# GuoYi0/alphaFive

Hardware: AMD Instinct MI355X
Metric: self-play moves/sec (11x11, 500 sims/move) (higher is better)
Workload: dtype f32 (fp16x2 split operands: 3 fp16 MFMA products per MAC, fp32 accumulate)

## Files before the change

### alphafive_amd/arena.py

```python
import ctypes

import numpy as np

from . import engine as _eng
from . import utils


def play_matches(cfg, pv0, pv1, n_games, device=0, seed0=0, seed1=1, node_cap=0, max_plies=None):
    import torch
    S, G = cfg.board_size, n_games
    C = S * S
    dev = torch.device("cuda", device)
    engines = [_eng.Engine(cfg, G, device=device, mode=_eng.MODE_EXTERNAL, training=False, seed=s, node_cap=node_cap)
               for s in (seed0, seed1)]
    pvs = [pv0, pv1]
    planes = torch.zeros((G, 3, S, S), dtype=torch.float32, device=dev)
    policy = [torch.zeros((G, C), dtype=torch.float32, device=dev) for _ in range(2)]
    value = [torch.zeros((G,), dtype=torch.float32, device=dev) for _ in range(2)]
    stream = torch.cuda.current_stream(dev).cuda_stream
    boards = [np.zeros((S, S), np.int8) for _ in range(G)]
    last = [None] * G
    over = [False] * G
    moves = [[] for _ in range(G)]
    wins, draws = [0, 0], 0
    ply = 0
    limit = max_plies or C
    while not all(over) and ply < limit:
        for p in (0, 1):
            active = [i for i in range(G) if not over[i] and (i + ply) % 2 == p]
            if not active:
                continue
            e = engines[p]
            keys = np.stack([_eng.state_to_key(utils.board_to_state(boards[i]), S) for i in active])
            lcs = [-1 if last[i] is None else last[i][0] * S + last[i][1] for i in active]
            e.set_roots(active, keys, lcs, random_a=True, reset_tree=(ply < 2), stream=stream)
            while True:
                e.tick(policy[p].data_ptr(), value[p].data_ptr(), planes.data_ptr(), stream)
                st = e.status(stream)
                if all(st[i] == _eng.STATUS_MOVE_DONE for i in active):
                    break
                pr, va = pvs[p](planes)
                policy[p].copy_(pr.reshape(G, C))
                value[p].copy_(va.reshape(G))
            cells = e.move_results(active, stream=stream)[0]
            for i, cell in zip(active, cells):
                cell = int(cell)
                a = (cell // S, cell % S)
                moves[i].append(cell)
                boards[i] = utils.step(boards[i], a)
                last[i] = a
                done, v = utils.is_game_over(boards[i], cfg.goal)
                if done:
                    over[i] = True
                    if v == 0.0:
                        draws += 1
                    else:
                        wins[p] += 1
        ply += 1
    for e in engines:
        e.close()
    return dict(wins=wins, draws=draws, moves=moves, lengths=[len(m) for m in moves])


MATCH_WIN0, MATCH_WIN1, MATCH_DRAW, MATCH_UNFINISHED = 0, 1, 2, -1
TICK_SLACK = 64


class DeviceArena:

    def __init__(self, cfg, pv0, pv1, num_games, device=0, seed0=0, seed1=1, node_cap=0, weights_versions=(None, None)):
        import torch
        if not torch.cuda.is_available():
            raise _eng.EngineError("DeviceArena needs a HIP device (torch.cuda.is_available() is False)")
        self.torch = torch
        self.cfg = cfg
        S, G = cfg.board_size, num_games
        self.S, self.C, self.G = S, S * S, G
        self.dev = torch.device("cuda", device)
        torch.cuda.set_device(self.dev)
        self.engines, self._match = [], None
        for s in (seed0, seed1):
            self.engines.append(_eng.Engine(cfg, G, device=device, mode=_eng.MODE_EXTERNAL, training=False, seed=s, node_cap=node_cap))
        h = ctypes.c_void_p()
        _eng._check(_eng.lib().af_match_create(self.engines[0]._h, self.engines[1]._h, ctypes.byref(h)), "af_match_create")
        self._match = h
        self.pvs = [pv0, pv1]
        self.planes = [torch.zeros((G, 3, S, S), dtype=torch.float32, device=self.dev) for _ in range(2)]
        self.policy = [torch.zeros((G, self.C), dtype=torch.float32, device=self.dev) for _ in range(2)]
        self.value = [torch.zeros((G,), dtype=torch.float32, device=self.dev) for _ in range(2)]
        self._versions, self._version_missing = [], False
        for p, pv in enumerate(self.pvs):
            ver, missing = _eng.resolve_weights_version(pv, weights_versions[p])
            self._versions.append(ver)
            self._version_missing = self._version_missing or missing
            if hasattr(pv, "bind_outputs"):
                pv.bind_outputs(self.policy[p], self.value[p])
        self._graph = None
        self._prog_host = torch.zeros(3, dtype=torch.int64, pin_memory=True)
        self._prog_events = [torch.cuda.Event(), torch.cuda.Event()]
        self.rounds = self.replays = self.eager_rounds = 0

    def _stream(self):
        return self.torch.cuda.current_stream(self.dev).cuda_stream

    def round(self):
        stream = self._stream()
        L = _eng.lib()
        for p in (0, 1):
            self.engines[p].tick(self.policy[p].data_ptr(), self.value[p].data_ptr(), self.planes[p].data_ptr(), stream)
            pr, va = self.pvs[p](self.planes[p])
            if pr.data_ptr() != self.policy[p].data_ptr():
                self.policy[p].copy_(pr.reshape(self.G, self.C))
            if va.data_ptr() != self.value[p].data_ptr():
                self.value[p].copy_(va.reshape(self.G))
            _eng._check(L.af_match_step(self._match, stream), "af_match_step")
        self.rounds += 1

    def _post_progress(self):
        _eng._check(_eng.lib().af_match_progress_async(self._match, self._stream(), self._prog_host.data_ptr()), "af_match_progress_async")

    def _graph_key(self, rounds_per_replay):
        return (int(rounds_per_replay), self.engines[0].params_key(), self.engines[1].params_key(),
                tuple(v() if v is not None else None for v in self._versions))

    def _raise_first_error(self, code):
        raise _eng.EngineError("device arena: a game failed: %s (code %d)" % (_eng.lib().af_strerror(code).decode(), code))

    def run(self, n_games=None, max_plies=None, rounds_per_replay=8, graph=True):
        torch = self.torch
        n_games = self.G if n_games is None else int(n_games)
        limit = int(max_plies or self.C)
        if graph and self._version_missing:
            raise _eng.EngineError("DeviceArena.run(graph=True): an evaluator takes bind_outputs but exposes no weights_version (a "
                                   "replayed graph would keep evaluating with stale weights); pass weights_versions=")
        stream = self._stream()
        _eng._check(_eng.lib().af_match_start(self._match, stream, n_games, limit), "af_match_start")
        self.rounds = self.replays = self.eager_rounds = 0
        self._prog_host.zero_()
        bound = limit * (2 * int(self.cfg.upper_simulation_per_step) + TICK_SLACK)
        n = int(rounds_per_replay)
        turn, posted = 0, 0
        if graph and (self._graph is None or self._graph[0] != self._graph_key(n)):
            self._graph = None
            self.round()
            self.eager_rounds += 1
            torch.cuda.synchronize(self.dev)
            g = torch.cuda.CUDAGraph()
            with torch.cuda.graph(g, capture_error_mode="thread_local"):
                for _ in range(n):
                    self.round()
                self._post_progress()
            self.rounds -= n
            self._graph = (self._graph_key(n), g)
        while True:
            if self.rounds > bound:
                raise _eng.EngineError("device arena: %d games not finished after %d rounds (bound %d)" % (n_games, self.rounds, bound))
            if graph:
                self._graph[1].replay()
                self.rounds += n
                self.replays += 1
            else:
                for _ in range(n):
                    self.round()
                self.eager_rounds += n
                self._post_progress()
            turn ^= 1
            self._prog_events[turn].record(torch.cuda.current_stream(self.dev))
            posted += 1
            if posted < 2:
                continue
            self._prog_events[turn ^ 1].synchronize()
            done, _, err = (int(x) for x in self._prog_host)
            if err:
                torch.cuda.synchronize(self.dev)
                self._raise_first_error(err)
            if done >= n_games:
                break
        return self.results(n_games)

    def results(self, n_games=None):
        n_games = self.G if n_games is None else int(n_games)
        res, lens = np.zeros(self.G, np.int32), np.zeros(self.G, np.int32)
        mv = np.zeros((self.G, self.C), np.int32)
        rc = _eng.lib().af_match_results(self._match, self._stream(), _eng._p(res, ctypes.c_int32), _eng._p(lens, ctypes.c_int32),
                                         _eng._p(mv, ctypes.c_int32))
        if rc < 0:
            self._raise_first_error(rc)
        res, lens = res[:n_games], lens[:n_games]
        return dict(wins=[int((res == MATCH_WIN0).sum()), int((res == MATCH_WIN1).sum())], draws=int((res == MATCH_DRAW).sum()),
                    moves=[[int(c) for c in mv[i, :lens[i]]] for i in range(n_games)], lengths=[int(x) for x in lens])

    def close(self):
        if getattr(self, "_match", None):
            _eng.lib().af_match_destroy(self._match)
            self._match = None
        for e in getattr(self, "engines", []):
            e.close()

    __del__ = close


def play_matches_device(cfg, pv0, pv1, n_games, device=0, seed0=0, seed1=1, node_cap=0, max_plies=None, **run_kw):
    a = DeviceArena(cfg, pv0, pv1, n_games, device=device, seed0=seed0, seed1=seed1, node_cap=node_cap)
    try:
        return a.run(n_games, max_plies=max_plies, **run_kw)
    finally:
        a.close()


def ladder(cfg, ckpt_paths, games, match_fn=None, result_path=None, log=print):
    paths = list(ckpt_paths)
    own = None
    if match_fn is None:
        own = match_fn = _arena_match_fn(cfg, games)
    out = []
    low, high = 0, len(paths) - 1
    try:
        while low < high:
            c0, c1 = paths[low], paths[high]
            w0, w1, draws = match_fn(c0, c1, games)
            line = "%s: %s = %d: %d" % (c0, c1, w0, w1)
            if log is not None:
                log(line)
            if result_path is not None:
                with open(result_path, "a") as f:
                    f.write(line + "\n")
            out.append((c0, c1, int(w0), int(w1), int(draws)))
            if w0 < w1:
                low += 1
            else:
                high -= 1
    finally:
        if own is not None:
            own.close()
    return out


def _arena_match_fn(cfg, games, device=0):
    state = {}

    def load(net, path):
        if str(path).endswith(".npz"):
            net.load_npz(path)
        else:
            net.restore(path)

    def match(path0, path1, n):
        from .network import ResNet
        if not state:
            state["nets"] = [ResNet(cfg.board_size, device="cuda:%d" % device) for _ in range(2)]
            state["loaded"] = [None, None]
            state["arena"] = DeviceArena(cfg, state["nets"][0].select_backend("hip"), state["nets"][1].select_backend("hip"), n,
                                         device=device)
        for p, path in enumerate((path0, path1)):
            if state["loaded"][p] != path:
                load(state["nets"][p], path)
                state["loaded"][p] = path
        r = state["arena"].run(n)
        return r["wins"][0], r["wins"][1], r["draws"]

    def close():
        if state:
            state["arena"].close()
# ... 7 lines not shown
```

### alphafive_amd/csrc/af_conv_f16s.h

```cpp
#ifndef AF_CONV_F16S_H
#define AF_CONV_F16S_H

#include <hip/hip_runtime.h>

#include <map>
#include <string>

struct f16s_net;

int f16s_supported(int board_size);
int f16s_create(f16s_net** out, int board_size, int max_batch, int device);
void f16s_destroy(f16s_net* n);
enum F16sBits : int {
    kF16sProfilingBits = 1 | 2 | 4 | 8 | 4096,
    kF16sValuStem = 16,
    kF16sOneWgPerCu = 32,
    kF16sTwoHalves15 = 64,
    kF16sWgPerPosition = 128,
    kF16sTwoLaunchBlocks = 256,
    kF16sBranchLaunchesSmall = 512,
    kF16sBranchLaunchesBig = 1024,
    kF16sLaunchSequence = 2048,
};
enum F16sForm {
    kF16sRoles,
    kF16sPaired,
    kF16sBranches,
};
struct F16sPlan {
    int batch, bits;
    bool heads;
    F16sForm form;
    bool valu_stem, two_wg_per_cu, half_classes, tile_split, fused_blocks;
};
F16sPlan f16s_plan(const f16s_net* n, int batch, int bits, bool heads);
int f16s_forward(f16s_net* n, const F16sPlan& p, hipStream_t st, const float* planes_dev, float* value, float* policy);
int f16s_trunk(f16s_net* n, const F16sPlan& p, hipStream_t st, const float* planes_dev);
int f16s_value_branch(f16s_net* n, const F16sPlan& p, hipStream_t st, float* o3_dev, int WP, int PP, float* value);
int f16s_policy_branch(f16s_net* n, const F16sPlan& p, hipStream_t st, float* o5_dev, int WP, int PP, float* policy);
int f16s_small_forward_error(f16s_net* n);
int f16s_read_activation(f16s_net* n, int which, int batch, float* host);

typedef std::map<std::string, const float*> f16s_dev_vars;
constexpr int kF16sScaleGroups = 20;
int f16s_update_absmax(f16s_net* n, hipStream_t st, const f16s_dev_vars& D, float* max_dev);
int f16s_update_pack(f16s_net* n, hipStream_t st, const f16s_dev_vars& D, const float* max_host);
int f16s_weight_buffer(const f16s_net* n, int index, const void** ptr, size_t* bytes);
int f16s_scales(const f16s_net* n, float* out, int cap);
struct UpdCopy { float* dst; const float* a; const float* b; int n_dst, n_src, sum; };
int upd_launch_copies(hipStream_t st, const UpdCopy* d, int count);

#endif
```

### alphafive_amd/csrc/af_conv_f16s.hip

```cpp
#include <hip/hip_runtime.h>
#include <stdint.h>
#include <stdio.h>
#include <stdlib.h>
#include <string.h>

#include <algorithm>
#include <atomic>
#include <cmath>
#include <map>
#include <string>
#include <vector>

#include "af_conv_f16s.h"

typedef _Float16 h8 __attribute__((ext_vector_type(8)));
typedef float f32x16 __attribute__((ext_vector_type(16)));
typedef float f32x4 __attribute__((ext_vector_type(4)));

#define FS_HIP_OK(x) do { hipError_t e_ = (x); if (e_ != hipSuccess) { fprintf(stderr, "[af_conv_f16s] %s failed: %s\n", #x, hipGetErrorString(e_)); return -2; } } while (0)

namespace {

template <int S_> struct Geo;
template <> struct Geo<11> {
// ... 12 lines not shown
    __host__ __device__ static constexpr uint32_t seg_unit(int seg) { return seg == 0 ? 0u : (seg == 1 ? 64u : 96u); }
    __host__ __device__ static constexpr uint32_t wbase(int h) { return h ? 96u : 0u; }
};
template <class G> struct Lay {
    static constexpr uint32_t kRowH = G::ROWU * 16u, kHalfH = 4u * kRowH, kSlabH = 2u * kHalfH;
    static constexpr uint32_t kRowL = G::WINU * 16u, kHalfL = 4u * kRowL, kSlotL = 2u * kHalfL;
};
constexpr uint32_t kLds0 = 256u;
#ifndef AF_F16S_DIST
#define AF_F16S_DIST 3
#endif
constexpr int kDist = AF_F16S_DIST;
template <class G, int DIST = kDist> struct Lds {
    static constexpr uint32_t kZoff = kLds0 + (DIST + 2) * Lay<G>::kSlotL;
    static constexpr uint32_t kBiasOff = kZoff + Lay<G>::kSlotL;
    static constexpr uint32_t kScrOff = kBiasOff + 512u;
};
template <class G> struct Hx {
    static constexpr int HXP = 128 * G::HALVES;
    static constexpr uint32_t kValPos = HXP * 16u, kValLo = HXP * 8u;
    static constexpr uint32_t kPolPos = HXP * 64u, kPolLo = HXP * 32u;
    static constexpr int VSTEPS = (G::NPIX + 3) / 4;
    static constexpr int NLT = (G::NPIX + 31) / 32;
};

constexpr int kS = 11, kPIX = 144, kNPIX = kS * kS;
constexpr uint32_t kRowB = kPIX * 16u, kHalfB = 4u * kRowB, kSlabB = 2u * kHalfB;

#ifndef AF_F16S_APIN
#define AF_F16S_APIN 1
#endif
#ifndef AF_F16S_VW
#define AF_F16S_VW 128
#endif
#ifndef AF_F16S_ZPAD
#define AF_F16S_ZPAD 1
#endif

__device__ __forceinline__ void st16(void* gdst, const h8& v) { *reinterpret_cast<h8*>(gdst) = v; }

template <class V16>
__device__ __forceinline__ void st16_sc1(void* gdst, const V16& v) {
    static_assert(sizeof(V16) == 16, "16-byte store");
    asm volatile("global_store_dwordx4 %0, %1, off sc1\n\ts_nop 1" : : "v"(gdst), "v"(v) : "memory");
}
template <class V8>
__device__ __forceinline__ void st8_sc1(void* gdst, const V8& v) {
    static_assert(sizeof(V8) == 8, "8-byte store");
    asm volatile("global_store_dwordx2 %0, %1, off sc1" : : "v"(gdst), "v"(v) : "memory");
}

__device__ __forceinline__ void wait_vmcnt(int n) {
#define AF_VM(k) case k: asm volatile("s_waitcnt vmcnt(" #k ")" ::: "memory"); break;
    switch (n) {
        AF_VM(0) AF_VM(1) AF_VM(2) AF_VM(3) AF_VM(4) AF_VM(5) AF_VM(6) AF_VM(7) AF_VM(8) AF_VM(9) AF_VM(10) AF_VM(11) AF_VM(12) AF_VM(13)
        AF_VM(14) AF_VM(15) AF_VM(16) AF_VM(17) AF_VM(18) AF_VM(19) AF_VM(20) AF_VM(21) AF_VM(22) AF_VM(23) AF_VM(24) AF_VM(25) AF_VM(26)
        AF_VM(27) AF_VM(28) AF_VM(29) AF_VM(30) AF_VM(31) AF_VM(32) AF_VM(33) AF_VM(34) AF_VM(35) AF_VM(36) AF_VM(37) AF_VM(38) AF_VM(39)
        AF_VM(40) AF_VM(41) AF_VM(42) AF_VM(43) AF_VM(44) AF_VM(45) AF_VM(46) AF_VM(47) AF_VM(48) AF_VM(49) AF_VM(50) AF_VM(51) AF_VM(52)
        AF_VM(53) AF_VM(54) AF_VM(55) AF_VM(56) AF_VM(57) AF_VM(58) AF_VM(59) AF_VM(60) AF_VM(61) AF_VM(62) AF_VM(63)
        default: asm volatile("s_waitcnt vmcnt(0)" ::: "memory"); break;
    }
#undef AF_VM
}

__device__ __forceinline__ void glds16(const void* gsrc, uint32_t lds_dst) {
    unsigned keep;
    asm volatile("s_mov_b32 %0, m0\n\ts_mov_b32 m0, %2\n\ts_nop 0\n\tglobal_load_lds_dwordx4 %1, off nt\n\ts_mov_b32 m0, %0"
                 : "=&s"(keep) : "v"(gsrc), "s"(lds_dst) : "memory");
}

__device__ __forceinline__ void glds16_sc1(const void* gsrc, uint32_t lds_dst) {
    unsigned keep;
    asm volatile("s_mov_b32 %0, m0\n\ts_mov_b32 m0, %2\n\ts_nop 0\n\tglobal_load_lds_dwordx4 %1, off sc1\n\ts_mov_b32 m0, %0"
                 : "=&s"(keep) : "v"(gsrc), "s"(lds_dst) : "memory");
}

typedef float f32x2 __attribute__((ext_vector_type(2)));
__device__ __forceinline__ float elu1(float x) {
    const float e = __builtin_amdgcn_exp2f(x * 1.44269504088896341f);
    return fmaxf(x, fminf(fmaxf(e, 0.0f), 1.0f) - 1.0f);
}
__device__ __forceinline__ f32x2 elu2(f32x2 x) {
    const f32x2 t = x * 1.44269504088896341f;
    f32x2 e;
    e.x = fminf(fmaxf(__builtin_amdgcn_exp2f(t.x), 0.0f), 1.0f);
    e.y = fminf(fmaxf(__builtin_amdgcn_exp2f(t.y), 0.0f), 1.0f);
    const f32x2 em1 = e - 1.0f;
    return f32x2{fmaxf(x.x, em1.x), fmaxf(x.y, em1.y)};
}

#ifndef AF_F16S_XCD_SWIZZLE
#define AF_F16S_XCD_SWIZZLE 1
#endif
#ifdef AF_F16S_TIMING
__device__ unsigned long long g_f16s_cycles[10][512][4][9];
__device__ unsigned long long g_f16s_wall[10][512][2];
#define AF_T(var) const unsigned long long var = __builtin_readcyclecounter()
#define AF_TACC(slot, a, b) tacc[slot] += (b) - (a)
#else
#define AF_T(var)
#define AF_TACC(slot, a, b)
#endif

#ifdef AF_DF_TIMING
__device__ unsigned long long g_df_wall[256][5];
#define DF_T(i) if (threadIdx.x == 0 && blockIdx.x < 256) g_df_wall[blockIdx.x][i] = wall_clock64()
#else
#define DF_T(i)
#endif
__device__ __forceinline__ void df_signal(int* ctr) {
    DF_T(2);
    asm volatile("s_waitcnt vmcnt(0)" ::: "memory");
    __syncthreads();
    if (threadIdx.x == 0) __hip_atomic_fetch_add(ctr, 1, __ATOMIC_RELAXED, __HIP_MEMORY_SCOPE_AGENT);
    DF_T(3);
}
__device__ __forceinline__ void df_poll(const int* ctr, int need, int* err) {
    int it = 0;
    while (__hip_atomic_load(ctr, __ATOMIC_RELAXED, __HIP_MEMORY_SCOPE_AGENT) < need) {
        __builtin_amdgcn_s_sleep(2);
        if (++it > (1 << 22)) { __hip_atomic_store(err, 1, __ATOMIC_RELAXED, __HIP_MEMORY_SCOPE_AGENT); break; }
    }
}
__device__ __forceinline__ void df_wait_one(const int* ctr, int need, int* err) {
    if (threadIdx.x == 0) df_poll(ctr, need, err);
    DF_T(1);
    __syncthreads();
}
__device__ __forceinline__ void df_wait_inv(const int* ctr, int need, int* err) {
    if (threadIdx.x == 0) {
        df_poll(ctr, need, err);
        __builtin_amdgcn_fence(__ATOMIC_ACQUIRE, "agent");
    }
    DF_T(1);
    __syncthreads();
}

struct F16sArgs {
    const char* in;
    const char* in2;
    const uint4* w;
    const float* bias;
    char* out;
    float* out32;
    float inv_scale;
    const uint4* pw;
    float* pbuf;
    float inv_scale_p;
    const uint4* hw;
    const float* hbias;
    char* hx;
    float inv_scale_h;
    int batch, WP, PP;
    const uint4* w2;
    const float* bias2;
    float inv_scale2;
    int gx0;
    char* stash;
    const int* df_wait;
    int df_need;
    int* df_done;
    int* df_err;
    int abl;
};

template <class G, int NSM, int NSP, int CT, int KS, int PS, bool OUT32, bool XACC, int PJ, int HD, int DIST, int WPE, int NTW, int HSEL, int FU = 0, int DF = 0>
__device__ __forceinline__ void f16s_body(const F16sArgs& A, char* smem, const int bx, const int gxw, const int tb = 0,
                                          const int by = (int)blockIdx.y, const int gy = (int)gridDim.y) {
    using L = Lay<G>;
    constexpr uint32_t kRowH = L::kRowH, kHalfH = L::kHalfH, kSlabH = L::kSlabH, kRowL = L::kRowL, kHalfL = L::kHalfL, kSlotL = L::kSlotL;
    constexpr uint32_t kZoff = Lds<G, DIST>::kZoff, kBiasOff = Lds<G, DIST>::kBiasOff, kScrOff = Lds<G, DIST>::kScrOff;
    constexpr int kDist = DIST, kRing = DIST + 2;
    constexpr int NPC = G::NPC, HV = G::HALVES;
    static_assert(FU == 0 || (G::HALVES == 1 && PJ == 1 && HD == 0 && !OUT32 && NSP == 0 && CT == 1 && HSEL < 0 &&
                              ((KS == 1 && NTW == 1) || (KS == 2 && NTW == 2))), "fused block: see above");
    constexpr uint32_t kScrBytes = KS == 2 ? (uint32_t)(CT * PS * NTW) * 4096u * (PJ == 1 ? 2u : 1u) : 0u;
    constexpr uint32_t kGOff = Lds<G, DIST>::kScrOff;
    constexpr uint32_t kW2Off = kGOff + (kScrBytes > Lay<G>::kSlotL ? kScrBytes : Lay<G>::kSlotL);
    constexpr int NT = NTW;
    static_assert(HSEL < 0 || (HV == 2 && PJ == 0 && HD == 0 && !OUT32), "half classes: plain 15x15 layers only");
    static_assert(NT % KS == 0 || PJ == 0, "an odd tile count under a k-split has no projection exchange");
    constexpr int C16 = 2 / KS;
    constexpr int ITP = C16, ITM = 9 * C16;
    constexpr int NIT = NSP * ITP + NSM * ITM;
    constexpr int SPP = NSP + NSM;
    constexpr int NFIN = NT / KS;
    static_assert(CT * KS * PS == 4 && NT >= KS, "4 waves");
    static_assert(PJ == 0 || NSP == 0, "a producer / consumer of the separate projection has no projection slabs");
    constexpr int NPW = PJ == 1 ? NSM * C16 : 0;
    static_assert(NPC * (DIST > 1 ? DIST - 1 : 1) < 64, "vmcnt is a 6-bit field");
    static_assert(DIST >= 2 || (NSP == 0 && ITM - 1 >= NPC), "distance 1: a slab's pieces must all be issued before its predecessor's last item");
    const int lane = threadIdx.x & 63, kg = lane >> 5, nn = lane & 31;
    const int wv = __builtin_amdgcn_readfirstlane((int)(threadIdx.x >> 6));
    const int ct = wv % CT, ks = (wv / CT) % KS, ps = wv / (CT * KS);
    const int rot = KS == 2 ? ks * ((NT + 1) / 2) : 0;
#define AF_OWN(jj) (KS == 1 || (jj) < NT / 2 || ((jj) < (NT + 1) / 2 && ks == 0))
    const int ctg = by * CT + ct, nso = gy * CT;
    const uint32_t lds = (uint32_t)(uintptr_t)smem;

    const int nq = HSEL >= 0 ? A.batch : A.batch * HV;
    int qpos = bx;
    if (AF_F16S_XCD_SWIZZLE && (gxw & (8 * (HSEL >= 0 ? 1 : HV) - 1)) == 0) qpos = (bx >> 3) + (gxw >> 3) * (bx & 7);
    if (qpos >= nq) return;
    const int hv = HSEL >= 0 ? HSEL : (HV == 1 ? 0 : qpos % HV);
    const uint32_t wsrc = G::wbase(hv) * 16u;
    AF_T(t_entry);
#ifdef AF_F16S_TIMING
    const unsigned long long wall_entry = wall_clock64();
#endif

    auto slab_src = [&](int qq, int j) -> const char* {
        const int p_ = (HV == 1 || HSEL >= 0) ? qq : qq / HV;
        const int p = (A.abl & 0x1000) ? (p_ & 127) : p_;
        return (j < NSM ? A.in + ((size_t)p * NSM + j) * kSlabH : A.in2 + ((size_t)p * NSP + (j - NSM)) * kSlabH) + wsrc;
    };
    auto dma_piece = [&](const char* src, uint32_t slot_off, int k) {
        const int piece = wv + 4 * k, row = piece / G::PR;
        const uint32_t su = G::seg_unit(piece % G::PR) * 16u;
        const uint32_t offh = (uint32_t)(row >> 2) * kHalfH + (uint32_t)(row & 3) * kRowH + su;
        const uint32_t offl = (uint32_t)(row >> 2) * kHalfL + (uint32_t)(row & 3) * kRowL + su;
        if (DF != 0) glds16_sc1(src + offh + lane * 16, (uint32_t)__builtin_amdgcn_readfirstlane((int)(lds + kLds0 + slot_off + offl)));
        else glds16(src + offh + lane * 16, (uint32_t)__builtin_amdgcn_readfirstlane((int)(lds + kLds0 + slot_off + offl)));
    };
    const int q0 = qpos;
    auto stream_src = [&](uint32_t idx) -> const char* {
        const int p = q0 + (int)(idx / SPP) * gxw, j = (int)(idx % SPP);
        return slab_src(p, j);
    };
    const uint32_t nslabs = (uint32_t)((nq - q0 + gxw - 1) / gxw) * SPP;

    if (DF == 0) {
#pragma unroll
        for (int d = 0; d < kDist; ++d) {
            if ((uint32_t)d < nslabs) {
#pragma unroll
                for (int k = 0; k < NPC; ++k) dma_piece(stream_src(d), (uint32_t)d * kSlotL, k);
            }
        }
    }

    h8 W[2 * NIT];
    {
        const uint4* wp = A.w + ((size_t)(ctg * KS + ks) * (2 * NIT)) * 64 + lane;
#pragma unroll
        for (int f = 0; f < 2 * NIT; ++f) {
            const uint4 v = wp[f * 64];
            __builtin_memcpy(&W[f], &v, 16);
        }
    }
    h8 PW[PJ == 1 ? 2 * NPW : 1];
    if (PJ == 1) {
        const uint4* wp = A.pw + ((size_t)(ctg * KS + ks) * (2 * NPW)) * 64 + lane;
#pragma unroll
        for (int f = 0; f < 2 * NPW; ++f) {
            const uint4 v = wp[f * 64];
            __builtin_memcpy(&PW[f], &v, 16);
        }
    }
    constexpr int HDS = HD > 0 ? HD : FU;
    h8 HA[HDS > 0 ? 4 : 1];
    float hb[HDS > 0 ? 8 : 1];
    if (FU > 0) {
        const uint4* w2 = A.w2;
#pragma unroll
        for (int i = 0; i < 9; ++i) *reinterpret_cast<uint4*>(smem + kW2Off + (uint32_t)(i * 256 + (int)threadIdx.x) * 16u) = w2[i * 256 + threadIdx.x];
        if (threadIdx.x < 32) reinterpret_cast<float*>(smem + kBiasOff + 256u)[threadIdx.x] = A.bias2[threadIdx.x];
        if (KS == 1) {
            for (uint32_t u = threadIdx.x; u < kSlotL / 16; u += 256) *reinterpret_cast<uint4*>(smem + kGOff + u * 16) = uint4{0, 0, 0, 0};
        }
    }
    if (HDS > 0) {
#pragma unroll
        for (int f = 0; f < 4; ++f) {
            const uint4 v = A.hw[f * 64 + lane];
            __builtin_memcpy(&HA[f], &v, 16);
        }
#pragma unroll
        for (int r = 0; r < 8; ++r) hb[r] = A.hbias[8 * kg + r];
    }
    if (threadIdx.x < kLds0 / 16) *reinterpret_cast<uint4*>(smem + threadIdx.x * 16) = uint4{0, 0, 0, 0};
    if (G::PADL + G::PADR > 0) {
        static_assert(G::PADL + G::PADR == 0 || (G::PADL == 8 && G::PADR == 8), "pad zeroing is written for 8 + 8 units");
        for (uint32_t u = threadIdx.x; u < (uint32_t)kRing * 128u; u += 256) {
            const uint32_t off = kLds0 + (u >> 7) * kSlotL + ((u >> 4) & 7u) * kRowL + (((u >> 3) & 1u) ? (G::WINU - 8u) * 16u : 0u) + (u & 7u) * 16u;
            *reinterpret_cast<uint4*>(smem + off) = uint4{0, 0, 0, 0};
        }
    }
    for (uint32_t u = threadIdx.x; u < kSlotL / 16; u += 256) *reinterpret_cast<uint4*>(smem + kZoff + u * 16) = uint4{0, 0, 0, 0};
    if (threadIdx.x < CT * 32) reinterpret_cast<float*>(smem + kBiasOff)[threadIdx.x] = A.bias[by * CT * 32 + threadIdx.x];
    uint32_t lb[NT], zb[NT];
    int pix[NT];
    bool ok[NT], edgeL[NT], edgeR[NT];
#pragma unroll
    for (int jj = 0; jj < NT; ++jj) {
        const int n = 128 * hv + 32 * (tb + ps * NT + ((jj + rot) % NT)) + nn;
        ok[jj] = n < G::NPIX;
        const int nc = ok[jj] ? n : 128 * hv;
        pix[jj] = nc;
        const int x = nc % G::S;
        edgeL[jj] = x == 0; edgeR[jj] = x == G::S - 1;
        lb[jj] = kLds0 + (uint32_t)((KS == 2 ? 2 * ks : 0) + kg) * kRowL + (uint32_t)((nc + G::POFF - G::S - 1 - (int)G::wbase(hv)) * 16);
        zb[jj] = kZoff + (lb[jj] & 255u);
    }
    constexpr int kAccRegs = 16 * NT * (1 + (XACC ? 1 : 0) + (PJ == 1 ? 1 : 0));
    constexpr int kWRegs = 4 * (2 * NIT + (PJ == 1 ? 2 * NPW : 0) + (HDS > 0 ? 4 : 0));
    constexpr int kNAmax = (256 - kAccRegs - 16) / 4, kNAwant = (kWRegs - AF_F16S_VW + 3) / 4;
    constexpr int NA = (AF_F16S_APIN && WPE == 1 && kNAwant > 0) ? (kNAwant < kNAmax ? kNAwant : kNAmax) : 0;
#pragma unroll
    for (int f = 0; f < 2 * NIT; ++f) {
        if (f < 2 * NIT - NA) asm volatile("" : "+v"(W[f]));
        else asm volatile("" : "+a"(W[f]));
    }
    if (PJ == 1) {
#pragma unroll
        for (int f = 0; f < 2 * NPW; ++f) asm volatile("" : "+v"(PW[f]));
    }
    if (HDS > 0) {
#pragma unroll
        for (int f = 0; f < 4; ++f) asm volatile("" : "+v"(HA[f]));
    }
    if (DF != 0) {
        df_wait_one(A.df_wait + qpos, A.df_need, A.df_err);
#pragma unroll
        for (int d = 0; d < kDist; ++d) {
            if ((uint32_t)d < nslabs) {
#pragma unroll
                for (int k = 0; k < NPC; ++k) dma_piece(stream_src(d), (uint32_t)d * kSlotL, k);
            }
        }
    }
    asm volatile("s_waitcnt vmcnt(0) lgkmcnt(0)" ::: "memory");
    __builtin_amdgcn_s_barrier();
    AF_T(t_ready);

    auto rd = [](const char* sm, bool proj, int it, int p, uint32_t c_, uint32_t l_, uint32_t r_) -> h8 {
        const int c = proj ? it : it / 9, tap = proj ? 4 : it % 9, ky = tap / 3, kx = tap % 3;
        const uint32_t base = kx == 0 ? l_ : (kx == 2 ? r_ : c_);
        const uint32_t imm = (uint32_t)p * kHalfL + (KS == 1 ? 2u * c * kRowL : 0u) + (uint32_t)(ky * G::S + kx) * 16u;
        return *reinterpret_cast<const h8*>(sm + base + imm);
    };

    auto head_tile = [&](const float (&v)[16], const int jj, const int pos) {
      if constexpr (HDS > 0) {
        h8 bh[2], bl[2];
#pragma unroll
        for (int st_ = 0; st_ < 2; ++st_)
#pragma unroll
            for (int e = 0; e < 8; ++e) {
                const float f = v[8 * st_ + e];
                const _Float16 h = (_Float16)f;
                bh[st_][e] = h;
                bl[st_][e] = (_Float16)(f - (float)h);
            }
// ... 427 lines not shown
    const int tile = (int)blockIdx.y * 4 + (int)(threadIdx.x >> 6);
    if (tile >= A.NCT) return;
    const int p = 32 * (int)blockIdx.x + nn;
    const bool valid = p < A.batch;
    const size_t pc = (size_t)(valid ? p : A.batch - 1);
    f32x16 acc[KS], acx[XACC ? KS : 1];
#pragma unroll
    for (int h = 0; h < KS; ++h)
#pragma unroll
        for (int r = 0; r < 16; ++r) { acc[h][r] = 0.0f; if (XACC) acx[h][r] = 0.0f; }
    const uint4* const wbase = A.w + (size_t)tile * KS * NIT * 2 * 64 + lane;
    constexpr int SPP = NSM + NSP;
    const char* const st0 = A.stash + (pc * SPP * 32 + (uint32_t)kg * 4u) * 16;
    struct Ops { uint4 a0, a1, b0, b1; };
    auto half_of = [](int t) constexpr -> int {
        const int k16 = t < NSM * 8 ? (t >> 2) & 1 : (t - NSM * 8) & 1;
        return KS == 2 ? k16 : 0;
    };
    auto fetch = [&](int t) -> Ops {
        int k16, item;
        const char* bsrc;
        if (t < NSM * 8) {
            const int s_ = t >> 3, tq = t & 3, ky = tq >> 1, kx = tq & 1;
            k16 = (t >> 2) & 1;
            item = NSP * C16 + s_ * 9 * C16 + (KS == 2 ? 0 : k16) * 9 + 3 * ky + kx;
            bsrc = st0 + (uint32_t)((s_ * 32 + 2 * k16 * 4 + tq) * 16);
        } else {
            const int u = t - NSM * 8, s_ = u >> 1;
            k16 = u & 1;
            item = s_ * C16 + (KS == 2 ? 0 : k16);
            bsrc = st0 + (uint32_t)(((NSM + s_) * 32 + 2 * k16 * 4 + 3) * 16);
        }
        const uint4* wp = wbase + ((size_t)((KS == 2 ? k16 : 0) * NIT + item) * 2) * 64;
        Ops o;
        o.a0 = wp[0]; o.a1 = wp[64];
        o.b0 = *reinterpret_cast<const uint4*>(bsrc); o.b1 = *reinterpret_cast<const uint4*>(bsrc + 256);
        return o;
    };
    Ops ring[D];
#pragma unroll
    for (int t = 0; t < D; ++t) ring[t] = fetch(t);
    __builtin_amdgcn_sched_barrier(0);
#pragma unroll
    for (int t = 0; t < NST; ++t) {
        const Ops o = ring[t % D];
        if (t + D < NST) ring[t % D] = fetch(t + D);
        const int h = half_of(t);
        h8 wh, wl, bh, bl;
        __builtin_memcpy(&wh, &o.a0, 16); __builtin_memcpy(&wl, &o.a1, 16); __builtin_memcpy(&bh, &o.b0, 16); __builtin_memcpy(&bl, &o.b1, 16);
        acc[h] = __builtin_amdgcn_mfma_f32_32x32x16_f16(wh, bh, acc[h], 0, 0, 0);
        if (XACC) {
            acx[h] = __builtin_amdgcn_mfma_f32_32x32x16_f16(wh, bl, acx[h], 0, 0, 0);
            acx[h] = __builtin_amdgcn_mfma_f32_32x32x16_f16(wl, bh, acx[h], 0, 0, 0);
        } else {
            acc[h] = __builtin_amdgcn_mfma_f32_32x32x16_f16(wh, bl, acc[h], 0, 0, 0);
            acc[h] = __builtin_amdgcn_mfma_f32_32x32x16_f16(wl, bh, acc[h], 0, 0, 0);
        }
        __builtin_amdgcn_sched_group_barrier(0x008, 3, 0);
        __builtin_amdgcn_sched_group_barrier(0x020, 4, 0);
    }
    if (XACC) {
#pragma unroll
        for (int h = 0; h < KS; ++h)
#pragma unroll
            for (int r = 0; r < 16; ++r) acc[h][r] += acx[h][r];
    }
    if (KS == 2) {
#pragma unroll
        for (int r = 0; r < 16; ++r) acc[0][r] = acc[KS - 1][r] + acc[0][r];
    }
    if (!valid) return;
    float v[16];
#pragma unroll
    for (int r = 0; r < 16; r += 2) {
        const f32x2 pre = f32x2{acc[0][r], acc[0][r + 1]} * A.inv_scale + f32x2{A.bias[32 * tile + 16 * kg + r], A.bias[32 * tile + 16 * kg + r + 1]};
        const f32x2 y = elu2(pre);
        v[r] = y.x; v[r + 1] = y.y;
    }
    char* o = A.out + ((size_t)p * A.NCT + tile) * L::kSlabH + (uint32_t)(2 * kg) * L::kRowH + (uint32_t)(CPIX + G::POFF) * 16u;
#pragma unroll
    for (int hf = 0; hf < 2; ++hf) {
        h8 hi, lo;
#pragma unroll
        for (int e = 0; e < 8; ++e) {
            const float f = v[8 * hf + e];
            const _Float16 h = (_Float16)f;
            hi[e] = h;
            lo[e] = (_Float16)(f - (float)h);
        }
        st16(o + hf * L::kRowH, hi);
        st16(o + hf * L::kRowH + L::kHalfH, lo);
    }
}

template <class G>
__global__ __launch_bounds__(256) void af_stem_f16s(const float* __restrict__ planes, const float* __restrict__ w,
                                                    const float* __restrict__ bias, char* __restrict__ out, int batch) {
    constexpr int S = G::S, NPIX = G::NPIX, SP = S + 4;
    constexpr uint32_t kRowH = Lay<G>::kRowH, kHalfH = Lay<G>::kHalfH, kSlabH = Lay<G>::kSlabH;
    __shared__ float sx[3 * SP * SP];
    __shared__ float sw[75 * 32];
    __shared__ float sb[32];
    const int t = threadIdx.x;
    for (int i = t; i < 75 * 32; i += 256) sw[i] = w[i];
    if (t < 32) sb[t] = bias[t];
    for (int i = t; i < 3 * SP * SP; i += 256) sx[i] = 0.0f;
    for (int b = blockIdx.x; b < batch; b += gridDim.x) {
        __syncthreads();
        for (int i = t; i < 3 * NPIX; i += 256) {
            const int c = i / NPIX, p = i - c * NPIX, y = p / S, x = p - y * S;
            sx[c * SP * SP + (y + 2) * SP + x + 2] = planes[(size_t)b * 3 * NPIX + i];
        }
        __syncthreads();
        if (t < NPIX) {
            const int y = t / S, x = t - y * S;
            float acc[32];
#pragma unroll
            for (int co = 0; co < 32; ++co) acc[co] = sb[co];
            for (int ky = 0; ky < 5; ++ky)
                for (int kx = 0; kx < 5; ++kx)
#pragma unroll
                    for (int c = 0; c < 3; ++c) {
                        const float xv = sx[c * SP * SP + (y + ky) * SP + x + kx];
                        const float* wr = sw + ((ky * 5 + kx) * 3 + c) * 32;
#pragma unroll
                        for (int co = 0; co < 32; ++co) acc[co] = fmaf(xv, wr[co], acc[co]);
                    }
            char* o = out + (size_t)b * kSlabH + (uint32_t)(t + G::POFF) * 16u;
#pragma unroll
            for (int u = 0; u < 4; ++u) {
                h8 hi, lo;
#pragma unroll
                for (int e = 0; e < 8; ++e) {
                    const float f = elu1(acc[8 * u + e]);
                    const _Float16 h = (_Float16)f;
                    hi[e] = h;
                    lo[e] = (_Float16)(f - (float)h);
                }
                *reinterpret_cast<h8*>(o + u * kRowH) = hi;
                *reinterpret_cast<h8*>(o + u * kRowH + kHalfH) = lo;
            }
        }
    }
}

template <class G> struct StemLds {
    static constexpr int SR = G::S + 4, IW = G::S + 5;
    static constexpr int kEnt = 3 * SR * G::S + 1, kImg = 3 * SR * IW;
    static constexpr uint32_t kImgOff = (uint32_t)((kEnt * 16 + 255) / 256 * 256), kBytes = kImgOff + (uint32_t)kImg * 2u;
};
template <class G, bool SC1 = false>
__device__ __forceinline__ void f16s_stem_body(const float* __restrict__ planes, const uint4* __restrict__ w ,
                                               const float* __restrict__ bias, float inv_scale, char* __restrict__ out, int batch,
                                               const int bx, const int gx, uint4* ent, _Float16* img) {
    constexpr int S = G::S, NPIX = G::NPIX, SR = S + 4, IW = S + 5;
    constexpr int NPL = 3 * NPIX, NLD = (NPL + 255) / 256;
    constexpr int NTL = (NPIX + 31) / 32, NRND = (NTL + 3) / 4;
    constexpr uint32_t kRowH = Lay<G>::kRowH, kHalfH = Lay<G>::kHalfH, kSlabH = Lay<G>::kSlabH;
    const int lane = threadIdx.x & 63, kg = lane >> 5, nn = lane & 31;
    const int wv = __builtin_amdgcn_readfirstlane((int)(threadIdx.x >> 6));
    h8 W[16];
#pragma unroll
    for (int f = 0; f < 16; ++f) {
        const uint4 v = w[f * 64 + lane];
        __builtin_memcpy(&W[f], &v, 16);
    }
    float bs[16];
#pragma unroll
    for (int r = 0; r < 16; ++r) bs[r] = bias[16 * kg + r];
    for (int i = threadIdx.x; i < 3 * SR * IW; i += 256) img[i] = (_Float16)0.0f;
    auto img_at = [](int i) -> int { const int c = i / NPIX, p = i - c * NPIX, y = p / S, x = p - y * S; return (c * SR + y + 2) * IW + x + 2; };
    int at[NLD];
    float nx[NLD];
#pragma unroll
    for (int q = 0; q < NLD; ++q) {
        const int i = (int)threadIdx.x + 256 * q;
        at[q] = img_at(i < NPL ? i : 0);
        nx[q] = 0.0f;
        if (i < NPL && bx < batch) nx[q] = planes[(size_t)bx * NPL + i];
    }
    for (int pos = bx; pos < batch; pos += gx) {
        __syncthreads();
#pragma unroll
        for (int q = 0; q < NLD; ++q)
            if ((int)threadIdx.x + 256 * q < NPL) img[at[q]] = (_Float16)nx[q];
        if (pos + gx < batch) {
            const float* pl = planes + (size_t)(pos + gx) * NPL;
#pragma unroll
            for (int q = 0; q < NLD; ++q)
                if ((int)threadIdx.x + 256 * q < NPL) nx[q] = pl[threadIdx.x + 256 * q];
        }
        __syncthreads();
        for (int en = threadIdx.x; en < 3 * SR * S; en += 256) {
            const int cin = en / (SR * S), rem = en - cin * SR * S, yy = rem / S, x = rem - yy * S;
            const _Float16* src = img + (cin * SR + yy) * IW + x;
            const h8 v = {src[0], src[1], src[2], src[3], src[4], 0, 0, 0};
            __builtin_memcpy(&ent[en], &v, 16);
        }
        __syncthreads();
#pragma unroll
        for (int rd_ = 0; rd_ < NRND; ++rd_) {
            const int n = 32 * (wv + 4 * rd_) + nn;
            const bool ok = n < NPIX;
            const int nc = ok ? n : 0;
            if (32 * (wv + 4 * rd_) >= NPIX) continue;
            f32x16 acc;
#pragma unroll
            for (int r = 0; r < 16; ++r) acc[r] = 0.0f;
#pragma unroll
            for (int s_ = 0; s_ < 8; ++s_) {
                const int ga = 2 * s_, gb = 2 * s_ + 1 < 15 ? 2 * s_ + 1 : 0;
                const uint32_t offa = (uint32_t)((ga / 5) * SR + ga % 5) * S, offb = (uint32_t)((gb / 5) * SR + gb % 5) * S;
                h8 b;
                __builtin_memcpy(&b, &ent[(uint32_t)nc + (kg ? offb : offa)], 16);
                acc = __builtin_amdgcn_mfma_f32_32x32x16_f16(W[2 * s_], b, acc, 0, 0, 0);
                acc = __builtin_amdgcn_mfma_f32_32x32x16_f16(W[2 * s_ + 1], b, acc, 0, 0, 0);
            }
            char* o = out + (size_t)pos * kSlabH + (uint32_t)(2 * kg) * kRowH + (uint32_t)(nc + G::POFF) * 16u;
#pragma unroll
            for (int hf = 0; hf < 2; ++hf) {
                h8 hi, lo;
#pragma unroll
                for (int e = 0; e < 8; ++e) {
                    const float f = elu1(acc[8 * hf + e] * inv_scale + bs[8 * hf + e]);
                    const _Float16 h = (_Float16)f;
                    hi[e] = h;
                    lo[e] = (_Float16)(f - (float)h);
                }
                if (ok) {
                    if (SC1) { st16_sc1(o + hf * kRowH, hi); st16_sc1(o + hf * kRowH + kHalfH, lo); }
                    else {
                        *reinterpret_cast<h8*>(o + hf * kRowH) = hi;
                        *reinterpret_cast<h8*>(o + hf * kRowH + kHalfH) = lo;
                    }
                }
            }
        }
    }
}

template <class G>
__global__ __launch_bounds__(256) void af_stem_mfma_f16s(const float* __restrict__ planes, const uint4* __restrict__ w, const float* __restrict__ bias,
                                                         float inv_scale, char* __restrict__ out, int batch) {
    __shared__ __attribute__((aligned(16))) uint4 ent[StemLds<G>::kEnt];
    __shared__ _Float16 img[StemLds<G>::kImg];
    f16s_stem_body<G>(planes, w, bias, inv_scale, out, batch, (int)blockIdx.x, (int)gridDim.x, ent, img);
}

template <class G>
__device__ __forceinline__ void f16s_vfc_body(const char* __restrict__ xv, const uint4* __restrict__ a, const float* __restrict__ b1,
                                              const float* __restrict__ w2, const float* __restrict__ b2, float inv_scale,
                                              float* __restrict__ value, int batch, const int bx) {
    __shared__ float red[2][32];
    constexpr int NS = Hx<G>::VSTEPS;
    const bool act = threadIdx.x < 128;
    const int lane = threadIdx.x & 63, mt = (threadIdx.x >> 6) & 1, n = lane & 31, kg = lane >> 5;
    const int pos = bx * 32 + n, posc = pos < batch ? pos : batch - 1;
    const char* xb = xv + (size_t)posc * Hx<G>::kValPos + (uint32_t)kg * 16u;
    const uint4* ap = a + (size_t)mt * 128 + lane;
    f32x16 acc;
#pragma unroll
    for (int r = 0; r < 16; ++r) acc[r] = 0.0f;
#pragma unroll
    for (int half = 0; half < (NS + 15) / 16; ++half) {
        uint4 bh[16], bl[16], ah[16], al[16];
#pragma unroll
        for (int q = 0; q < 16; ++q) {
            const int s_ = 16 * half + q;
            if (s_ < NS) {
                bh[q] = *reinterpret_cast<const uint4*>(xb + s_ * 32);
                bl[q] = *reinterpret_cast<const uint4*>(xb + Hx<G>::kValLo + s_ * 32);
                ah[q] = ap[(size_t)s_ * 256];
                al[q] = ap[(size_t)s_ * 256 + 64];
            }
        }
        typedef uint32_t u32x4 __attribute__((ext_vector_type(4)));
#pragma unroll
        for (int q = 0; q < 16; ++q) {
            if (16 * half + q < NS) {
                u32x4 t0, t1, t2, t3;
                __builtin_memcpy(&t0, &bh[q], 16); __builtin_memcpy(&t1, &bl[q], 16); __builtin_memcpy(&t2, &ah[q], 16); __builtin_memcpy(&t3, &al[q], 16);
                asm volatile("" : "+v"(t0), "+v"(t1), "+v"(t2), "+v"(t3));
                __builtin_memcpy(&bh[q], &t0, 16); __builtin_memcpy(&bl[q], &t1, 16); __builtin_memcpy(&ah[q], &t2, 16); __builtin_memcpy(&al[q], &t3, 16);
            }
        }
#pragma unroll
        for (int q = 0; q < 16; ++q) {
            if (16 * half + q < NS) {
                h8 xh, xl, wh, wl;
                __builtin_memcpy(&xh, &bh[q], 16); __builtin_memcpy(&xl, &bl[q], 16);
                __builtin_memcpy(&wh, &ah[q], 16); __builtin_memcpy(&wl, &al[q], 16);
                acc = __builtin_amdgcn_mfma_f32_32x32x16_f16(wh, xh, acc, 0, 0, 0);
                acc = __builtin_amdgcn_mfma_f32_32x32x16_f16(wh, xl, acc, 0, 0, 0);
                acc = __builtin_amdgcn_mfma_f32_32x32x16_f16(wl, xh, acc, 0, 0, 0);
            }
        }
    }
    float part = 0.0f;
#pragma unroll
    for (int r = 0; r < 16; ++r) {
        const int j = 32 * mt + 16 * kg + r;
        part += elu1(acc[r] * inv_scale + b1[j]) * w2[j];
    }
    part += __shfl_xor(part, 32);
    if (act && kg == 0) red[mt][n] = part;
    __syncthreads();
    if (act && mt == 0 && kg == 0 && pos < batch) value[pos] = tanhf((red[0][n] + red[1][n] + b2[0]) * 0.5f);
}
template <class G>
__global__ __launch_bounds__(128) __attribute__((amdgpu_waves_per_eu(1, 2))) void af_value_fc_f16s(
    const char* __restrict__ xv, const uint4* __restrict__ a , const float* __restrict__ b1, const float* __restrict__ w2,
    const float* __restrict__ b2, float inv_scale, float* __restrict__ value, int batch) {
    f16s_vfc_body<G>(xv, a, b1, w2, b2, inv_scale, value, batch, (int)blockIdx.x);
}
struct VfcArgs { const char* xv; const uint4* a; const float *b1, *w2, *b2; float inv_scale; float* value; };
template <class G>
__global__ __launch_bounds__(256, 1) __attribute__((amdgpu_waves_per_eu(1, 1))) void af_small_l7v_f16s(F16sArgs P, VfcArgs V) {
    extern __shared__ __attribute__((aligned(16))) char smem[];
    const int nb = P.batch, id = (int)blockIdx.x;
    if (id < 2 * nb) f16s_body<G, 2, 4, 2, 2, 1, false, true, 0, 0, kDist, 1, 2, -1>(P, smem, id % nb, nb, (id / nb) * 2);
    else f16s_vfc_body<G>(V.xv, V.a, V.b1, V.w2, V.b2, V.inv_scale, V.value, nb, id - 2 * nb);
}
template <class G>
__global__ __launch_bounds__(256, 1) __attribute__((amdgpu_waves_per_eu(1, 1))) void af_big_l7v_f16s(F16sArgs P, VfcArgs V) {
    extern __shared__ __attribute__((aligned(16))) char smem[];
    const int gp = P.gx0, id = (int)blockIdx.x;
    if (id < gp) f16s_body<G, 2, 4, 2, 2, 1, false, true, 0, 0, kDist, 1, 4, -1>(P, smem, id, gp);
    else f16s_vfc_body<G>(V.xv, V.a, V.b1, V.w2, V.b2, V.inv_scale, V.value, P.batch, id - gp);
}

constexpr int kDfStem = 0, kDfL0 = 8, kDfL1 = 16, kDfL2 = 24, kDfL3 = 32, kDfP = 40, kDfV = 48, kDfQ = 56, kDfB5 = 64, kDfPF = 72, kDfFin = 73, kDfErr = 74, kDfWords = 75;
struct SmallFwdArgs {
    const float* planes; const uint4* stem_w; const float* stem_b; float stem_inv; char* f0;
    F16sArgs L0, L1, L2, L3, P, V, Q, B5;
    VfcArgs F;
    const char* xp; const uint4* pfa; const float* pfb; float pf_inv; float* policy; float* pfx;
    int* df;
    int batch;
};

template <class G>
__device__ __forceinline__ void f16s_pfc_role(const SmallFwdArgs& S, const int kh, char* smem) {
    constexpr int NPIX = G::NPIX, HXP = Hx<G>::HXP, NLT = Hx<G>::NLT, LW = 32 * NLT, LWP = LW + 1, NS = HXP / 2, RD = 32;
    static_assert(NLT == 4 && NS == 64, "the role form of the policy head is written for 11x11 (one logit tile per wave)");
    const int nb = S.batch, lane = threadIdx.x & 63, n = lane & 31, kg = lane >> 5;
    const int mt = __builtin_amdgcn_readfirstlane((int)(threadIdx.x >> 6));
    int* const df = S.df;
    const int step0 = NS * kh, nstep = NPIX - step0 < NS ? NPIX - step0 : NS;
    const uint4* ap = S.pfa + ((size_t)step0 * NLT + mt) * 128 + lane;
    uint4 ring[RD][2];
#pragma unroll
    for (int q = 0; q < RD; ++q) {
        const int st_ = q < nstep ? q : nstep - 1;
        ring[q][0] = ap[(size_t)st_ * NLT * 128];
        ring[q][1] = ap[(size_t)st_ * NLT * 128 + 64];
    }
    float bj[16];
#pragma unroll
    for (int r = 0; r < 16; ++r) { const int j = 32 * mt + 16 * kg + r; bj[r] = S.pfb[j < NPIX ? j : 0]; }
    {
        unsigned sink = 0;
#pragma unroll
        for (int q = RD; q < NS; ++q) {
            const int st_ = q < nstep ? q : nstep - 1;
            sink ^= reinterpret_cast<const unsigned*>(ap + (size_t)st_ * NLT * 128)[0] ^ reinterpret_cast<const unsigned*>(ap + (size_t)st_ * NLT * 128 + 64)[0];
        }
        asm volatile("" : : "v"(sink));
    }
    if (threadIdx.x == 0) {
        for (int p = 0; p < nb; ++p) df_poll(df + kDfB5 + p, 1, df + kDfErr);
    }
    DF_T(1);
    __syncthreads();
    constexpr uint32_t kXS = 2u * NS * 32u + 16u;
    for (int c = mt; c < nb * 4; c += 4) {
        const int pp = c >> 2, hl = (c >> 1) & 1, part = c & 1;
        glds16_sc1(S.xp + (size_t)pp * Hx<G>::kPolPos + (uint32_t)hl * Hx<G>::kPolLo + (uint32_t)step0 * 32u + (uint32_t)part * 1024u + (uint32_t)lane * 16u,
                   (uint32_t)__builtin_amdgcn_readfirstlane((int)((uint32_t)(uintptr_t)smem + (uint32_t)pp * kXS + (uint32_t)hl * (NS * 32u) + (uint32_t)part * 1024u)));
    }
    asm volatile("s_waitcnt vmcnt(0)" ::: "memory");
    __syncthreads();
    const int pq = n < nb ? n : nb - 1;
    const char* xb = smem + (uint32_t)pq * kXS + (uint32_t)kg * 16u;
    f32x16 acc;
#pragma unroll
    for (int r = 0; r < 16; ++r) acc[r] = 0.0f;
    h8 bh = *reinterpret_cast<const h8*>(xb), bl = *reinterpret_cast<const h8*>(xb + NS * 32);
#pragma unroll
    for (int st_ = 0; st_ < NS; ++st_) {
        h8 ah, al, nbh = bh, nbl = bl;
        __builtin_memcpy(&ah, &ring[st_ % RD][0], 16); __builtin_memcpy(&al, &ring[st_ % RD][1], 16);
        if (st_ + 1 < NS) {
            nbh = *reinterpret_cast<const h8*>(xb + (st_ + 1) * 32);
            nbl = *reinterpret_cast<const h8*>(xb + NS * 32 + (st_ + 1) * 32);
        }
        if (st_ + RD < NS) {
            const int pf = st_ + RD < nstep ? st_ + RD : nstep - 1;
            ring[st_ % RD][0] = ap[(size_t)pf * NLT * 128];
            ring[st_ % RD][1] = ap[(size_t)pf * NLT * 128 + 64];
        }
        acc = __builtin_amdgcn_mfma_f32_32x32x16_f16(ah, bh, acc, 0, 0, 0);
        acc = __builtin_amdgcn_mfma_f32_32x32x16_f16(ah, bl, acc, 0, 0, 0);
        acc = __builtin_amdgcn_mfma_f32_32x32x16_f16(al, bh, acc, 0, 0, 0);
        if (st_ + 1 < NS) __builtin_amdgcn_sched_group_barrier(0x100, 2, 0);
        if (st_ + RD < NS) __builtin_amdgcn_sched_group_barrier(0x020, 2, 0);
        __builtin_amdgcn_sched_group_barrier(0x008, 3, 0);
        bh = nbh; bl = nbl;
    }
    __syncthreads();
    f32x4* const px = reinterpret_cast<f32x4*>(S.pfx) + (size_t)mt * 4 * 64 + lane;
    if (kh == 1) {
#pragma unroll
        for (int q = 0; q < 4; ++q) st16_sc1(px + q * 64, f32x4{acc[4 * q], acc[4 * q + 1], acc[4 * q + 2], acc[4 * q + 3]});
        df_signal(df + kDfPF);
        return;
    }
    df_wait_inv(df + kDfPF, 1, df + kDfErr);
    float* Lg = reinterpret_cast<float*>(smem);
#pragma unroll
    for (int q = 0; q < 4; ++q) {
        const f32x4 o = px[q * 64];
#pragma unroll
        for (int e = 0; e < 4; ++e) {
            const int r = 4 * q + e, j = 32 * mt + 16 * kg + r;
            Lg[n * LWP + j] = j < NPIX ? (acc[r] + o[e]) * S.pf_inv + bj[r] : -3.0e38f;
        }
    }
    __syncthreads();
    const int p = (int)threadIdx.x >> 4, sub = (int)threadIdx.x & 15;
    constexpr int NV = LW / 16;
    float v[NV], mx = -3.0e38f;
#pragma unroll
    for (int q = 0; q < NV; ++q) { v[q] = Lg[p * LWP + sub + 16 * q]; mx = fmaxf(mx, v[q]); }
#pragma unroll
    for (int off = 8; off >= 1; off >>= 1) mx = fmaxf(mx, __shfl_xor(mx, off));
    float sum = 0.0f;
#pragma unroll
    for (int q = 0; q < NV; ++q) { v[q] = (sub + 16 * q) < NPIX ? expf(v[q] - mx) : 0.0f; sum += v[q]; }
#pragma unroll
    for (int off = 8; off >= 1; off >>= 1) sum += __shfl_xor(sum, off);
    if (p < nb) {
#pragma unroll
        for (int q = 0; q < NV; ++q) {
            const int j = sub + 16 * q;
            if (j < NPIX) S.policy[(size_t)p * NPIX + j] = v[q] / sum;
        }
    }
}

template <class G>
__global__ __launch_bounds__(256, 1) __attribute__((amdgpu_waves_per_eu(1, 1))) void af_small_forward_f16s(SmallFwdArgs S) {
    extern __shared__ __attribute__((aligned(16))) char smem[];
    const int nb = S.batch;
    int id = (int)blockIdx.x;
    int* const df = S.df;
    DF_T(0);
    if (id < nb) {
        DF_T(1);
        f16s_stem_body<G, true>(S.planes, S.stem_w, S.stem_b, S.stem_inv, S.f0, nb, id, nb, reinterpret_cast<uint4*>(smem),
                          reinterpret_cast<_Float16*>(smem + StemLds<G>::kImgOff));
        df_signal(df + kDfStem + id);
    } else if ((id -= nb) < 2 * nb) {
        f16s_body<G, 1, 0, 2, 1, 2, false, false, 0, 0, 1, 1, 1, -1, 0, 1>(S.L0, smem, id % nb, nb, (id / nb) * 2, 0, 1);
    } else if ((id -= 2 * nb) < 2 * nb) {
        f16s_body<G, 2, 1, 2, 1, 2, false, true, 0, 0, kDist, 1, 1, -1, 0, 1>(S.L1, smem, id % nb, nb, (id / nb) * 2, 0, 1);
    } else if ((id -= 2 * nb) < 4 * nb) {
        f16s_body<G, 2, 0, 4, 1, 1, false, false, 0, 0, kDist, 1, 1, -1, 0, 1>(S.L2, smem, id % nb, nb, id / nb, 0, 1);
    } else if ((id -= 4 * nb) < 4 * nb) {
        const int r = id / nb;
        f16s_body<G, 4, 2, 2, 2, 1, false, false, 0, 0, kDist, 1, 2, -1, 0, 1>(S.L3, smem, id % nb, nb, (r >> 1) * 2, r & 1, 2);
    } else if ((id -= 4 * nb) < 3 * nb) {
        if (id < 2 * nb) f16s_body<G, 4, 0, 2, 2, 1, false, false, 0, 0, kDist, 1, 2, -1, 0, 1>(S.P, smem, id % nb, nb, (id / nb) * 2, 0, 1);
        else f16s_body<G, 4, 0, 1, 2, 2, false, false, 1, 0, 2, 1, 2, -1, 1, 1>(S.V, smem, id - 2 * nb, nb, 0, 0, 1);
    } else if ((id -= 3 * nb) < 2 * nb + 1) {
        if (id < 2 * nb) {
            f16s_body<G, 2, 4, 2, 2, 1, false, true, 0, 0, kDist, 1, 2, -1, 0, 1>(S.Q, smem, id % nb, nb, (id / nb) * 2, 0, 1);
        } else {
            if (threadIdx.x == 0) {
                for (int p = 0; p < nb; ++p) df_poll(df + kDfV + p, 1, df + kDfErr);
                __builtin_amdgcn_fence(__ATOMIC_ACQUIRE, "agent");
            }
            DF_T(1);
            __syncthreads();
            f16s_vfc_body<G>(S.F.xv, S.F.a, S.F.b1, S.F.w2, S.F.b2, S.F.inv_scale, S.F.value, nb, 0);
        }
    } else if ((id -= 2 * nb + 1) < nb) {
        f16s_body<G, 2, 0, 1, 1, 4, false, true, 1, 0, 2, 1, 1, -1, 2, 1>(S.B5, smem, id, nb, 0, 0, 1);
    } else {
        f16s_pfc_role<G>(S, id - nb == 0 ? 1 : 0, smem);
    }
    __syncthreads();
    DF_T(4);
    if (threadIdx.x == 0) {
        if (__hip_atomic_fetch_add(df + kDfFin, 1, __ATOMIC_RELAXED, __HIP_MEMORY_SCOPE_AGENT) == (int)gridDim.x - 1) {
            for (int i = 0; i <= kDfFin; ++i) __hip_atomic_store(df + i, 0, __ATOMIC_RELAXED, __HIP_MEMORY_SCOPE_AGENT);
        }
    }
}

constexpr uint32_t kPfRow = 528u, kPfBuf = 64u * kPfRow;
#ifndef AF_PFC_POS
#define AF_PFC_POS 32
#endif
constexpr int kPfPos = AF_PFC_POS;
constexpr uint32_t kPfLds = 4u * kPfBuf;
#ifdef AF_PFC_TIMING
__device__ unsigned long long g_pfc_wall[256][8][5];
#define PF_T(i) if ((threadIdx.x & 63) == 0 && blockIdx.x < 256) g_pfc_wall[blockIdx.x][threadIdx.x >> 6][i] = wall_clock64()
#else
#define PF_T(i)
#endif
template <class G>
__global__ __launch_bounds__(512, 1) void af_policy_fc_f16s(const char* __restrict__ xp, const uint4* __restrict__ a ,
                                                            const float* __restrict__ bf, float inv_scale, float* __restrict__ policy, int batch) {
    extern __shared__ __attribute__((aligned(16))) char psm[];
    constexpr int NPIX = G::NPIX, HXP = Hx<G>::HXP, NLT = Hx<G>::NLT, MT = NLT / 4, RD = 16 / MT, NCH = HXP / 32, LW = 32 * NLT;
    constexpr int LWP = LW + 1;
    static_assert(NLT % 4 == 0 && LWP * 32 * 4 <= (int)kPfLds, "logit tiles");
    const int t = threadIdx.x & 255, lane = t & 63, n = lane & 31, kg = lane >> 5;
    const int kh = __builtin_amdgcn_readfirstlane((int)(threadIdx.x >> 8)), mt = __builtin_amdgcn_readfirstlane(t >> 6);
    PF_T(0);
    const int b0 = (int)blockIdx.x * kPfPos;
    char* const sm = psm + (uint32_t)kh * 2u * kPfBuf;
    const char* src[8];
    uint32_t dst[8];
#pragma unroll
    for (int i = 0; i < 8; ++i) {
        const int u = 256 * i + t, seg = u >> 5, pl = seg >> 1, hl = seg & 1, wi = u & 31, px = wi >> 1, oc = wi & 1;
        const int pq = b0 + (pl & (kPfPos - 1));
        const int p = pq < batch ? pq : batch - 1;
        src[i] = xp + (size_t)p * Hx<G>::kPolPos + (uint32_t)hl * Hx<G>::kPolLo + (uint32_t)((HXP / 2) * kh + px) * 32u + (uint32_t)oc * 16u;
        dst[i] = (uint32_t)((hl * 16 + px) * 2 + oc) * kPfRow + (uint32_t)pl * 16u;
    }
    uint4 stg[8];
#pragma unroll
    for (int i = 0; i < 8; ++i) stg[i] = *reinterpret_cast<const uint4*>(src[i]);
    uint4 ring[RD][MT][2];
    const int step0 = (HXP / 2) * kh, nstep = NPIX - step0 < HXP / 2 ? NPIX - step0 : HXP / 2;
    const uint4* ap = a + ((size_t)step0 * NLT + mt) * 128 + lane;
#pragma unroll
    for (int q = 0; q < RD; ++q)
#pragma unroll
        for (int m = 0; m < MT; ++m) {
            ring[q][m][0] = ap[((size_t)q * NLT + 4 * m) * 128];
            ring[q][m][1] = ap[((size_t)q * NLT + 4 * m) * 128 + 64];
        }
#pragma unroll
    for (int i = 0; i < 8; ++i) *reinterpret_cast<uint4*>(sm + dst[i]) = stg[i];
    f32x16 acc[MT];
#pragma unroll
    for (int m = 0; m < MT; ++m)
#pragma unroll
        for (int r = 0; r < 16; ++r) acc[m][r] = 0.0f;
    __syncthreads();
    PF_T(1);
    for (int c = 0; c < NCH; ++c) {
        const uint32_t cur = (uint32_t)(c & 1) * kPfBuf, nxt = kPfBuf - cur;
        if (c < NCH - 1) {
#pragma unroll
            for (int i = 0; i < 8; ++i) stg[i] = *reinterpret_cast<const uint4*>(src[i] + (size_t)(c + 1) * 512u);
        }
        const char* bb = sm + cur + (uint32_t)kg * kPfRow + (uint32_t)n * 16u;
#pragma unroll
        for (int q = 0; q < 16; ++q) {
            const int step = 16 * c + q;
            {
                const h8 bh = *reinterpret_cast<const h8*>(bb + (uint32_t)(2 * q) * kPfRow);
                const h8 bl = *reinterpret_cast<const h8*>(bb + (uint32_t)(2 * (16 + q)) * kPfRow);
#pragma unroll
                for (int m = 0; m < MT; ++m) {
                    h8 ah, al;
                    __builtin_memcpy(&ah, &ring[q % RD][m][0], 16);
                    __builtin_memcpy(&al, &ring[q % RD][m][1], 16);
                    {
                        const int pf = step + RD < nstep ? step + RD : nstep - 1;
                        ring[q % RD][m][0] = ap[((size_t)pf * NLT + 4 * m) * 128];
                        ring[q % RD][m][1] = ap[((size_t)pf * NLT + 4 * m) * 128 + 64];
                    }
                    acc[m] = __builtin_amdgcn_mfma_f32_32x32x16_f16(ah, bh, acc[m], 0, 0, 0);
                    acc[m] = __builtin_amdgcn_mfma_f32_32x32x16_f16(ah, bl, acc[m], 0, 0, 0);
                    acc[m] = __builtin_amdgcn_mfma_f32_32x32x16_f16(al, bh, acc[m], 0, 0, 0);
                }
            }
        }
        if (c < NCH - 1) {
#pragma unroll
            for (int i = 0; i < 8; ++i) *reinterpret_cast<uint4*>(sm + nxt + dst[i]) = stg[i];
        }
        __syncthreads();
    }
    PF_T(2);
    float* Lg = reinterpret_cast<float*>(psm);
    if (kh == 1) {
#pragma unroll
        for (int m = 0; m < MT; ++m)
#pragma unroll
            for (int r = 0; r < 16; ++r) Lg[n * LWP + 32 * (mt + 4 * m) + 16 * kg + r] = acc[m][r];
    }
    __syncthreads();
    if (kh == 0) {
#pragma unroll
        for (int m = 0; m < MT; ++m)
#pragma unroll
            for (int r = 0; r < 16; ++r) {
                const int j = 32 * (mt + 4 * m) + 16 * kg + r;
                Lg[n * LWP + j] = j < NPIX ? (acc[m][r] + Lg[n * LWP + j]) * inv_scale + bf[j] : -3.0e38f;
            }
    }
    __syncthreads();
    PF_T(3);
    const int p = (int)threadIdx.x >> 4, sub = (int)threadIdx.x & 15;
    constexpr int NV = LW / 16;
    float v[NV], mx = -3.0e38f;
#pragma unroll
    for (int q = 0; q < NV; ++q) { v[q] = Lg[p * LWP + sub + 16 * q]; mx = fmaxf(mx, v[q]); }
#pragma unroll
    for (int off = 8; off >= 1; off >>= 1) mx = fmaxf(mx, __shfl_xor(mx, off));
    float sum = 0.0f;
#pragma unroll
    for (int q = 0; q < NV; ++q) { v[q] = (sub + 16 * q) < NPIX ? expf(v[q] - mx) : 0.0f; sum += v[q]; }
#pragma unroll
    for (int off = 8; off >= 1; off >>= 1) sum += __shfl_xor(sum, off);
    if (p < kPfPos && b0 + p < batch) {
#pragma unroll
        for (int q = 0; q < NV; ++q) {
            const int j = sub + 16 * q;
            if (j < NPIX) policy[(size_t)(b0 + p) * NPIX + j] = v[q] / sum;
        }
    }
    PF_T(4);
}
#ifdef AF_PFC_TIMING
extern "C" int af_pfc_debug_wall(unsigned long long* host) {
    FS_HIP_OK(hipDeviceSynchronize());
    FS_HIP_OK(hipMemcpyFromSymbol(host, HIP_SYMBOL(g_pfc_wall), sizeof(unsigned long long) * 256 * 8 * 5));
    return 0;
}
#endif

struct LayerCfg { int cin, cout, pcin, CT, KS, PS, gy, pj; bool xacc; };
constexpr LayerCfg kLayers[10] = {
    {32, 64, 0, 2, 1, 2, 1, 0, true},    {64, 64, 32, 2, 1, 2, 1, 0, true},
    {64, 128, 0, 4, 1, 1, 1, 0, false},  {128, 128, 64, 2, 2, 1, 2, 0, false},
    {128, 32, 0, 1, 2, 2, 1, 1, false},  {32, 32, 0, 1, 1, 4, 1, 2, true},
    {128, 64, 0, 2, 2, 1, 1, 0, false},  {64, 64, 128, 2, 2, 1, 1, 0, true},
    {64, 32, 0, 1, 1, 4, 1, 1, true},    {32, 32, 0, 1, 1, 4, 1, 2, true},
};
const char* const kBlockNames[5] = {"bone/block1", "bone/block2", "value/block3", "policy/block4", "policy/block5"};
template <int LI> constexpr int kHeadOf = LI == 4 || LI == 5 ? 1 : LI == 8 || LI == 9 ? 2 : 0;

int device_bit(uint64_t* bit) {
    int dev = 0;
    FS_HIP_OK(hipGetDevice(&dev));
    *bit = 1ull << (dev & 63);
    return 0;
}
template <auto K>
int dyn_lds(uint64_t bit, int bytes) {
    static std::atomic<uint64_t> devs{0};
    if (!(devs.load(std::memory_order_relaxed) & bit)) {
        FS_HIP_OK(hipFuncSetAttribute(reinterpret_cast<const void*>(K), hipFuncAttributeMaxDynamicSharedMemorySize, bytes));
        devs.fetch_or(bit, std::memory_order_relaxed);
    }
    return 0;
}

template <class G, int NSM, int NSP, int CT, int KS, int PS, bool OUT32, bool XACC, int PJ = 0, int HD = 0, int DIST = kDist, int WPE = 1>
int launch_cfg(hipStream_t st, const F16sArgs& a, int gy, int ncu, bool tile_split) {
    constexpr int NT = 4 / PS;
    constexpr size_t lds = Lds<G, DIST>::kScrOff + (KS == 2 ? (size_t)CT * PS * NT * 4096 * (PJ == 1 ? 2 : 1) : 0);
    static_assert(WPE * lds <= 160 * 1024, "LDS budget of the workgroups sharing a CU");
#ifndef AF_F16S_NO_LDS_ASSERT
    static_assert(lds <= 160 * 1024, "LDS budget");
#endif
    uint64_t bit;
    if (device_bit(&bit) || dyn_lds<af_conv_f16s<G, NSM, NSP, CT, KS, PS, OUT32, XACC, PJ, HD, DIST, WPE>>(bit, 160 * 1024)) return -2;
    constexpr int NTS = KS == 2 ? 2 : 1;
    if constexpr (NTS < NT && HD == 0) {
        if (tile_split) {
            if (dyn_lds<af_conv_f16s_sb<G, NSM, NSP, CT, KS, PS, OUT32, XACC, PJ, HD, DIST, WPE, NTS>>(bit, 160 * 1024)) return -2;
            hipLaunchKernelGGL((af_conv_f16s_sb<G, NSM, NSP, CT, KS, PS, OUT32, XACC, PJ, HD, DIST, WPE, NTS>),
                               dim3(a.batch * G::HALVES, gy, NT / NTS), dim3(256), lds, st, a);
            FS_HIP_OK(hipGetLastError());
            return 0;
        }
    }
    int gx = std::max(1, std::min(a.batch * G::HALVES, WPE * ncu / gy));
    gx = std::max(G::HALVES, gx / G::HALVES * G::HALVES);
    hipLaunchKernelGGL((af_conv_f16s<G, NSM, NSP, CT, KS, PS, OUT32, XACC, PJ, HD, DIST, WPE>), dim3(gx, gy), dim3(256), lds, st, a);
    FS_HIP_OK(hipGetLastError());
    return 0;
}

template <class G, int LI>
int launch_block(hipStream_t st, const F16sArgs& a, int ncu) {
    constexpr LayerCfg L = kLayers[LI];
    constexpr int NSM = L.cin / 32, KS = L.KS, PS = L.PS, FU = kHeadOf<LI>;
    constexpr int DIST = 2;
    constexpr size_t scr = KS == 2 ? (size_t)PS * (4 / PS) * 4096 * 2 : 0;
    constexpr size_t lds = Lds<G, DIST>::kScrOff + (scr > Lay<G>::kSlotL ? scr : Lay<G>::kSlotL) + 36864;
    static_assert(lds <= 160 * 1024, "LDS budget of the fused block");
    uint64_t bit;
    if (device_bit(&bit) || dyn_lds<af_block_f16s<G, NSM, KS, PS, L.xacc, FU, DIST>>(bit, 160 * 1024)) return -2;
    const int gx = std::max(1, std::min(a.batch, ncu));
    hipLaunchKernelGGL((af_block_f16s<G, NSM, KS, PS, L.xacc, FU, DIST>), dim3(gx), dim3(256), lds, st, a);
    FS_HIP_OK(hipGetLastError());
    return 0;
}

template <class G, int NSM, int NSP, int CT, int KS, bool XACC>
int launch_h15(hipStream_t st, F16sArgs a, int gy, int ncu) {
    constexpr size_t lds = Lds<G, kDist>::kScrOff + (KS == 2 ? (size_t)CT * 4 * 4096 : 0);
    static_assert(lds <= 160 * 1024, "LDS budget");
    uint64_t bit;
    if (device_bit(&bit) || dyn_lds<af_conv_f16s_h15<G, NSM, NSP, CT, KS, XACC>>(bit, 160 * 1024)) return -2;
    const int gx = std::max(16, ncu / gy / 16 * 16);
    static const int num1 = [] { const char* e = getenv("AF_F16S_H15_NUM1"); const int v = e ? atoi(e) : 0; return v > 0 && v < 32 ? v : 18; }();
    static const int num2 = [] { const char* e = getenv("AF_F16S_H15_NUM2"); const int v = e ? atoi(e) : 0; return v > 0 && v < 32 ? v : 17; }();
    static const int rnd = [] { const char* e = getenv("AF_F16S_H15_ROUND"); return e ? atoi(e) : 1; }();
    const int num = KS == 1 ? num1 : num2;
    a.gx0 = rnd ? std::max(8, (gx * num / 32 + 4) / 8 * 8) : std::max(1, gx * num / 32);
    if (a.gx0 >= gx) a.gx0 = gx - 8;
    hipLaunchKernelGGL((af_conv_f16s_h15<G, NSM, NSP, CT, KS, XACC>), dim3(gx, gy), dim3(256), lds, st, a);
    FS_HIP_OK(hipGetLastError());
    CornerArgs c;
    c.stash = a.stash; c.w = a.w; c.bias = a.bias; c.out = a.out; c.inv_scale = a.inv_scale;
    c.batch = a.batch; c.NCT = gy * CT;
    hipLaunchKernelGGL((af_corner_f16s<G, KS, XACC, NSM, NSP>), dim3((a.batch + 31) / 32, (c.NCT + 3) / 4), dim3(256), 0, st, c);
    FS_HIP_OK(hipGetLastError());
    return 0;
}

}

struct f16s_net {
    int S = 11;
    int max_batch = 0, device = 0, ncu = 256;
    std::vector<void*> allocs;
    float *stem_w = nullptr, *stem_b = nullptr;
    uint4* stem_wm = nullptr;
    float stem_inv_scale = 1.0f;
    uint4* w[10] = {};
    uint4* pw[10] = {};
    float* pbuf[5] = {};
    float* bias[10] = {};
    float inv_scale[10] = {}, inv_scale_p[10] = {};
    char *f0 = nullptr, *g[5] = {}, *o[5] = {};
    uint4 *hcw[2] = {}, *hfw[2] = {};
    float *hcb[2] = {}, *hfb[2] = {}, *v2w = nullptr, *v2b = nullptr;
    float hc_inv[2] = {}, hf_inv[2] = {};
    char* hx[2] = {};
    int* df = nullptr;
    float* pfx = nullptr;
    char* stash = nullptr;
    std::vector<std::pair<const void*, size_t>> wreg;
};

static int layer_frags(const LayerCfg& L) { return (L.cout / 32) * L.KS * ((L.pcin / 32) * (2 / L.KS) + (L.cin / 32) * 9 * (2 / L.KS)); }
static int proj_frags(const LayerCfg& L, int cout) { return (cout / 32) * L.KS * (L.cin / 32) * (2 / L.KS); }
constexpr int kStemFrags = 8, kHconvFrags = 2;
static int vfc_frags(int npix) { return (npix + 3) / 4 * 2; }
static int pfc_frags(int npix) { return npix * ((npix + 31) / 32); }
constexpr size_t kFragBytes = 2 * 64 * 16;

int f16s_supported(int board_size) { return board_size == 11 || board_size == 15; }

template <class T>
static int dev_alloc(f16s_net* n, T** dst, size_t bytes, bool zero) {
    void* q = nullptr;
    FS_HIP_OK(hipMalloc(&q, bytes));
    n->allocs.push_back(q);
    if (zero) FS_HIP_OK(hipMemset(q, 0, bytes));
    *dst = (T*)q;
    return 0;
}

int f16s_create(f16s_net** out, int board_size, int max_batch, int device) {
    if (!f16s_supported(board_size)) return -1;
    FS_HIP_OK(hipSetDevice(device));
    f16s_net* n = new f16s_net();
// ... 122 lines not shown
            return j < D.npix ? D.w3[(size_t)(c16 * D.npix + px) * D.npix + j] * D.scale : 0.0f;
        }
    }
}

constexpr int kFragBlocks = 64;
__global__ __launch_bounds__(256) void af_update_frags(FragTable T) {
#pragma clang fp contract(off)
    const FragDesc& D = T.d[blockIdx.y];
    for (int row = blockIdx.x * 256 + threadIdx.x; row < D.frags * 64; row += kFragBlocks * 256) {
        const int f = row >> 6, lane = row & 63;
        h8 hi, lo;
#pragma unroll
        for (int e = 0; e < 8; ++e) {
            const float v = frag_value(D, f, lane, e);
            const _Float16 h = (_Float16)v;
            hi[e] = h;
            lo[e] = (_Float16)(v - (float)h);
        }
        h8* dst = reinterpret_cast<h8*>(D.dst);
        dst[(size_t)(2 * f) * 64 + lane] = hi;
        dst[(size_t)(2 * f + 1) * 64 + lane] = lo;
    }
}

constexpr int kMaxCopies = 48, kCopyBlocks = 32;
struct CopyTable { UpdCopy d[kMaxCopies]; };
__global__ __launch_bounds__(256) void af_update_copy(CopyTable T) {
    const UpdCopy& D = T.d[blockIdx.y];
    for (int i = blockIdx.x * 256 + threadIdx.x; i < D.n_dst; i += kCopyBlocks * 256) {
        float v = 0.0f;
        if (i < D.n_src) v = D.sum ? D.a[i] + (D.b ? D.b[i] : 0.0f) : D.a[i];
        D.dst[i] = v;
    }
}

}

int upd_launch_copies(hipStream_t st, const UpdCopy* d, int count) {
    if (count < 1 || count > kMaxCopies) return -1;
    CopyTable T = {};
    for (int i = 0; i < count; ++i) T.d[i] = d[i];
    hipLaunchKernelGGL(af_update_copy, dim3(kCopyBlocks, count), dim3(256), 0, st, T);
    FS_HIP_OK(hipGetLastError());
    return 0;
}

int f16s_update_absmax(f16s_net* n, hipStream_t st, const f16s_dev_vars& D, float* max_dev) {
    const int npix = n->S * n->S;
    MaxTable T = {};
    T.g[0] = {D.at("bone/conv1/kernel"), nullptr, 75 * 32, 0};
    for (int b = 0; b < 5; ++b) {
        const std::string s = kBlockNames[b];
        const LayerCfg &L1 = kLayers[2 * b], &L2 = kLayers[2 * b + 1];
        const float* kr = D.at(s + "_res/kernel");
        const int nr = L1.cin * L2.cout;
        T.g[1 + 3 * b] = {D.at(s + "_conv1/kernel"), nullptr, 9 * L1.cin * L1.cout, 0};
        T.g[2 + 3 * b] = {D.at(s + "_conv2/kernel"), kr, 9 * L2.cin * L2.cout, L1.pj == 1 ? 0 : nr};
        T.g[3 + 3 * b] = {kr, nullptr, nr, 0};
    }
    T.g[16] = {D.at("value/conv/kernel"), nullptr, 32 * 4, 0};
    T.g[17] = {D.at("policy/conv/kernel"), nullptr, 32 * 16, 0};
    T.g[18] = {D.at("value/fc1/kernel"), nullptr, 4 * npix * 64, 0};
    T.g[19] = {D.at("policy/fc/kernel"), nullptr, 16 * npix * npix, 0};
    FS_HIP_OK(hipMemsetAsync(max_dev, 0, kF16sScaleGroups * sizeof(float), st));
    hipLaunchKernelGGL(af_update_absmax, dim3(kMaxBlocks, kF16sScaleGroups), dim3(256), 0, st, T, max_dev);
    FS_HIP_OK(hipGetLastError());
    return 0;
}

int f16s_update_pack(f16s_net* n, hipStream_t st, const f16s_dev_vars& D, const float* max_host) {
    const int npix = n->S * n->S;
    float sc[kF16sScaleGroups];
    for (int g = 0; g < kF16sScaleGroups; ++g) sc[g] = pick_scale(max_host[g]);
    FragTable T = {};
    int nb = 0;
    auto frag = [&](uint4* dst, const float* w3, const float* w1, float scale, int kind, int frags, int cin, int cout, int pcin, int KS, int nc) {
        T.d[nb++] = FragDesc{dst, w3, w1, scale, kind, frags, cin, cout, pcin, KS, nc, npix};
    };
    UpdCopy C[kMaxCopies];
    int ncp = 0;
    auto copy = [&](float* dst, const float* a, const float* b, int n_dst, int n_src, int sum) { C[ncp++] = UpdCopy{dst, a, b, n_dst, n_src, sum}; };
    frag(n->stem_wm, D.at("bone/conv1/kernel"), nullptr, sc[0], FK_STEM, kStemFrags, 0, 0, 0, 1, 0);
    copy(n->stem_w, D.at("bone/conv1/kernel"), nullptr, 75 * 32, 75 * 32, 0);
    copy(n->stem_b, D.at("bone/conv1/bias"), nullptr, 32, 32, 0);
    for (int b = 0; b < 5; ++b) {
        const std::string s = kBlockNames[b];
        const LayerCfg &L1 = kLayers[2 * b], &L2 = kLayers[2 * b + 1];
        const float *k1 = D.at(s + "_conv1/kernel"), *k2 = D.at(s + "_conv2/kernel"), *kr = D.at(s + "_res/kernel");
        frag(n->w[2 * b], k1, nullptr, sc[1 + 3 * b], FK_LAYER, layer_frags(L1), L1.cin, L1.cout, L1.pcin, L1.KS, 0);
        frag(n->w[2 * b + 1], k2, kr, sc[2 + 3 * b], FK_LAYER, layer_frags(L2), L2.cin, L2.cout, L2.pcin, L2.KS, 0);
        if (L1.pj == 1) frag(n->pw[2 * b], nullptr, kr, sc[3 + 3 * b], FK_LAYER, proj_frags(L1, L2.cout), 0, L2.cout, L1.cin, L1.KS, 0);
        copy(n->bias[2 * b], D.at(s + "_conv1/bias"), nullptr, L1.cout, L1.cout, 0);
        copy(n->bias[2 * b + 1], D.at(s + "_conv2/bias"), D.at(s + "_res/bias"), L2.cout, L2.cout, 1);
    }
    frag(n->hcw[0], D.at("value/conv/kernel"), nullptr, sc[16], FK_HCONV, kHconvFrags, 0, 0, 0, 1, 4);
    frag(n->hcw[1], D.at("policy/conv/kernel"), nullptr, sc[17], FK_HCONV, kHconvFrags, 0, 0, 0, 1, 16);
    frag(n->hfw[0], D.at("value/fc1/kernel"), nullptr, sc[18], FK_VFC, vfc_frags(npix), 0, 0, 0, 1, 0);
    frag(n->hfw[1], D.at("policy/fc/kernel"), nullptr, sc[19], FK_PFC, pfc_frags(npix), 0, 0, 0, 1, 0);
    copy(n->hcb[0], D.at("value/conv/bias"), nullptr, 16, 4, 0);
    copy(n->hcb[1], D.at("policy/conv/bias"), nullptr, 16, 16, 0);
    copy(n->hfb[0], D.at("value/fc1/bias"), nullptr, 64, 64, 0);
    copy(n->hfb[1], D.at("policy/fc/bias"), nullptr, npix, npix, 0);
    copy(n->v2w, D.at("value/fc2/kernel"), nullptr, 64, 64, 0);
    copy(n->v2b, D.at("value/fc2/bias"), nullptr, 1, 1, 0);
    hipLaunchKernelGGL(af_update_frags, dim3(kFragBlocks, nb), dim3(256), 0, st, T);
    FS_HIP_OK(hipGetLastError());
    if (upd_launch_copies(st, C, ncp)) return -2;
    n->stem_inv_scale = 1.0f / sc[0];
    for (int b = 0; b < 5; ++b) {
        n->inv_scale[2 * b] = 1.0f / sc[1 + 3 * b]; n->inv_scale[2 * b + 1] = 1.0f / sc[2 + 3 * b];
        if (kLayers[2 * b].pj == 1) n->inv_scale_p[2 * b] = 1.0f / sc[3 + 3 * b];
    }
    n->hc_inv[0] = 1.0f / sc[16]; n->hc_inv[1] = 1.0f / sc[17];
    n->hf_inv[0] = 1.0f / sc[18]; n->hf_inv[1] = 1.0f / sc[19];
    return 0;
}

int f16s_weight_buffer(const f16s_net* n, int index, const void** ptr, size_t* bytes) {
    if (!n || index < 0 || index >= (int)n->wreg.size()) return -1;
    *ptr = n->wreg[index].first; *bytes = n->wreg[index].second;
    return 0;
}

int f16s_scales(const f16s_net* n, float* out, int cap) {
    float v[25];
    v[0] = n->stem_inv_scale;
    for (int i = 0; i < 10; ++i) { v[1 + i] = n->inv_scale[i]; v[11 + i] = n->inv_scale_p[i]; }
    v[21] = n->hc_inv[0]; v[22] = n->hc_inv[1]; v[23] = n->hf_inv[0]; v[24] = n->hf_inv[1];
    for (int i = 0; i < 25 && i < cap; ++i) out[i] = v[i];
    return 25;
}

constexpr int kSmallBatch = 8;

F16sPlan f16s_plan(const f16s_net* n, int batch, int bits, bool heads) {
    const bool s11 = n->S == 11, small = batch <= kSmallBatch;
    F16sPlan p = {};
    p.batch = batch; p.bits = bits; p.heads = heads;
    p.valu_stem = bits & kF16sValuStem;
    p.two_wg_per_cu = s11 && !(bits & kF16sOneWgPerCu);
    p.half_classes = !s11 && batch >= 128 && !(bits & kF16sTwoHalves15);
    p.tile_split = small && !(bits & kF16sWgPerPosition);
    p.fused_blocks = s11 && heads && !(bits & kF16sTwoLaunchBlocks);
    if (p.fused_blocks && p.tile_split && p.two_wg_per_cu && !p.valu_stem && !(bits & (kF16sBranchLaunchesSmall | kF16sLaunchSequence)))
        p.form = kF16sRoles;
    else if (p.fused_blocks && (small ? p.tile_split && !(bits & kF16sBranchLaunchesSmall) : !(bits & kF16sBranchLaunchesBig)))
        p.form = kF16sPaired;
    else
        p.form = kF16sBranches;
    return p;
}

static F16sArgs layer_args(const f16s_net* n, const F16sPlan& p, int li, const char* in, const char* in2, char* out) {
    F16sArgs a = {};
    a.in = in; a.in2 = in2; a.out = out;
    a.w = n->w[li]; a.bias = n->bias[li]; a.inv_scale = n->inv_scale[li];
    a.pw = n->pw[li]; a.pbuf = n->pbuf[li / 2]; a.inv_scale_p = n->inv_scale_p[li];
    a.inv_scale2 = a.inv_scale_h = 1.0f;
    a.batch = p.batch; a.stash = n->stash;
    a.abl = (p.bits & 0xf0ff) | (li << 8);
    static const int mask = [] { const char* e = getenv("AF_F16S_ABL_LAYERS"); return e ? (int)strtol(e, nullptr, 0) : 0x3ff; }();
    if (!((mask >> li) & 1)) a.abl &= ~kF16sProfilingBits;
    return a;
}
static void add_conv2(F16sArgs& a, const f16s_net* n, int li) { a.w2 = n->w[li]; a.bias2 = n->bias[li]; a.inv_scale2 = n->inv_scale[li]; }
static void add_head(F16sArgs& a, const f16s_net* n, int h) { a.hw = n->hcw[h]; a.hbias = n->hcb[h]; a.hx = n->hx[h]; a.inv_scale_h = n->hc_inv[h]; }
template <int LI>
static F16sArgs block_args(const f16s_net* n, const F16sPlan& p, const char* in) {
    F16sArgs a = layer_args(n, p, LI, in, nullptr, nullptr);
    add_conv2(a, n, LI + 1);
    add_head(a, n, kHeadOf<LI> - 1);
    return a;
}

template <class F>
static int with_geo(const f16s_net* n, F&& f) { return n->S == 11 ? f(Geo<11>{}) : f(Geo<15>{}); }

template <class G, int LI>
static int launch_one(const f16s_net* n, const F16sPlan& p, hipStream_t st, const F16sArgs& a) {
    constexpr LayerCfg L = kLayers[LI];
    constexpr int NSM = L.cin / 32, NSP = L.pcin / 32, CT = L.CT, KS = L.KS, PS = L.PS, PJ = L.pj, HD = kHeadOf<LI>;
    constexpr bool OUT32 = PJ == 2, XACC = L.xacc;
    const bool head = OUT32 && p.heads;
    if constexpr (G::S == 11 && (LI == 0 || LI == 5 || LI == 9)) {
        if (p.two_wg_per_cu && (head || !OUT32))
            return launch_cfg<G, NSM, NSP, CT, KS, PS, OUT32, XACC && LI != 0, PJ, HD, 1, 2>(st, a, L.gy, n->ncu, p.tile_split);
    }
    if constexpr (G::S == 15 && (LI == 2 || LI == 3 || LI == 6 || LI == 7)) {
        if (p.half_classes) return launch_h15<G, NSM, NSP, CT, KS, XACC>(st, a, L.gy, n->ncu);
    }
    if constexpr (OUT32) {
        if (head) return launch_cfg<G, NSM, NSP, CT, KS, PS, OUT32, XACC, PJ, HD>(st, a, L.gy, n->ncu, p.tile_split);
    }
    return launch_cfg<G, NSM, NSP, CT, KS, PS, OUT32, XACC, PJ>(st, a, L.gy, n->ncu, p.tile_split);
}
template <int LI>
static int launch_layer(const f16s_net* n, const F16sPlan& p, hipStream_t st, const char* in, const char* in2, char* out,
                        float* out32 = nullptr, int WP = 0, int PP = 0) {
    F16sArgs a = layer_args(n, p, LI, in, in2, out);
    a.out32 = out32; a.WP = WP; a.PP = PP;
    if constexpr (kLayers[LI].pj == 2) {
        if (p.heads) add_head(a, n, kHeadOf<LI> - 1);
    }
    return with_geo(n, [&](auto g) { return launch_one<decltype(g), LI>(n, p, st, a); });
}
static int launch_policy_fc(const f16s_net* n, hipStream_t st, int batch, float* policy) {
    return with_geo(n, [&](auto g) {
        hipLaunchKernelGGL(af_policy_fc_f16s<decltype(g)>, dim3((batch + kPfPos - 1) / kPfPos), dim3(512), kPfLds, st, n->hx[1], n->hfw[1], n->hfb[1],
                           n->hf_inv[1], policy, batch);
        return 0;
    });
}

int f16s_trunk(f16s_net* n, const F16sPlan& p, hipStream_t st, const float* planes) {
    const int batch = p.batch;
    if (!n || batch < 1 || batch > n->max_batch) return -1;
    with_geo(n, [&](auto g) {
        using G = decltype(g);
        if (p.valu_stem) hipLaunchKernelGGL(af_stem_f16s<G>, dim3(std::min(batch, 2048)), dim3(256), 0, st, planes, n->stem_w, n->stem_b, n->f0, batch);
        else hipLaunchKernelGGL(af_stem_mfma_f16s<G>, dim3(std::min(batch, 1024)), dim3(256), 0, st, planes, n->stem_wm, n->stem_b, n->stem_inv_scale, n->f0, batch);
        return 0;
    });
    int rc = launch_layer<0>(n, p, st, n->f0, nullptr, n->g[0]);
    if (!rc) rc = launch_layer<1>(n, p, st, n->g[0], n->f0, n->o[0]);
    if (!rc) rc = launch_layer<2>(n, p, st, n->o[0], nullptr, n->g[1]);
    if (!rc) rc = launch_layer<3>(n, p, st, n->g[1], n->o[0], n->o[1]);
    return rc;
}

int f16s_value_branch(f16s_net* n, const F16sPlan& p, hipStream_t st, float* o3, int WP, int PP, float* value) {
    int rc;
    if (p.fused_blocks) {
        rc = launch_block<Geo<11>, 4>(st, block_args<4>(n, p, n->o[1]), n->ncu);
    } else {
        rc = launch_layer<4>(n, p, st, n->o[1], nullptr, n->g[2]);
        if (!rc) rc = launch_layer<5>(n, p, st, n->g[2], n->o[1], nullptr, o3, WP, PP);
    }
    if (!rc && p.heads)
        with_geo(n, [&](auto g) {
            hipLaunchKernelGGL(af_value_fc_f16s<decltype(g)>, dim3((p.batch + 31) / 32), dim3(128), 0, st, n->hx[0], n->hfw[0], n->hfb[0], n->v2w, n->v2b,
                               n->hf_inv[0], value, p.batch);
            return 0;
        });
    return rc;
}

int f16s_policy_branch(f16s_net* n, const F16sPlan& p, hipStream_t st, float* o5, int WP, int PP, float* policy) {
    int rc = launch_layer<6>(n, p, st, n->o[1], nullptr, n->g[3]);
    if (!rc) rc = launch_layer<7>(n, p, st, n->g[3], n->o[1], n->o[3]);
    if (!rc && p.fused_blocks) {
        rc = launch_block<Geo<11>, 8>(st, block_args<8>(n, p, n->o[3]), n->ncu);
    } else {
        if (!rc) rc = launch_layer<8>(n, p, st, n->o[3], nullptr, n->g[4]);
        if (!rc) rc = launch_layer<9>(n, p, st, n->g[4], n->o[3], nullptr, o5, WP, PP);
    }
    if (!rc && p.heads) launch_policy_fc(n, st, p.batch, policy);
    return rc;
}

static int paired_branches(f16s_net* n, const F16sPlan& p, hipStream_t st, float* value, float* policy) {
    using G = Geo<11>;
    const int batch = p.batch;
    F16sArgs P = layer_args(n, p, 6, n->o[1], nullptr, n->g[3]);
    const F16sArgs V = block_args<4>(n, p, n->o[1]);
    constexpr size_t ldsP = Lds<G, kDist>::kScrOff + (size_t)2 * 1 * 4 * 4096;
    constexpr size_t ldsV = Lds<G, 2>::kScrOff + (size_t)2 * 2 * 4096 * 2 + 36864;
    constexpr size_t lds = ldsP > ldsV ? ldsP : ldsV;
    static_assert(lds <= 160 * 1024, "LDS budget");
    uint64_t bit;
    if (device_bit(&bit)) return -2;
    const int gp = std::max(1, std::min(batch, n->ncu));
    if (p.tile_split) {
        if (dyn_lds<af_small_pair_f16s<G>>(bit, 160 * 1024)) return -2;
        hipLaunchKernelGGL(af_small_pair_f16s<G>, dim3(3 * batch), dim3(256), lds, st, P, V);
    } else {
        if (dyn_lds<af_big_pair_f16s<G>>(bit, 160 * 1024)) return -2;
        P.gx0 = gp;
        hipLaunchKernelGGL(af_big_pair_f16s<G>, dim3(2 * gp), dim3(256), lds, st, P, V);
    }
    FS_HIP_OK(hipGetLastError());
    F16sArgs Q = layer_args(n, p, 7, n->g[3], n->o[1], n->o[3]);
    const VfcArgs F = {n->hx[0], n->hfw[0], n->hfb[0], n->v2w, n->v2b, n->hf_inv[0], value};
    constexpr size_t lds7 = Lds<G, kDist>::kScrOff + (size_t)2 * 1 * 4 * 4096;
    if (p.tile_split) {
        if (dyn_lds<af_small_l7v_f16s<G>>(bit, (int)lds7)) return -2;
        hipLaunchKernelGGL(af_small_l7v_f16s<G>, dim3(2 * batch + 1), dim3(256), lds7, st, Q, F);
    } else {
        if (dyn_lds<af_big_l7v_f16s<G>>(bit, (int)lds7)) return -2;
        Q.gx0 = gp;
        hipLaunchKernelGGL(af_big_l7v_f16s<G>, dim3(gp + (batch + 31) / 32), dim3(256), lds7, st, Q, F);
    }
    FS_HIP_OK(hipGetLastError());
    const int rc = launch_block<G, 8>(st, block_args<8>(n, p, n->o[3]), n->ncu);
    if (!rc) launch_policy_fc(n, st, batch, policy);
    FS_HIP_OK(hipGetLastError());
    return rc;
}

static int roles_forward(f16s_net* n, const F16sPlan& p, hipStream_t st, const float* planes, float* value, float* policy) {
    using G = Geo<11>;
    const int batch = p.batch;
    SmallFwdArgs S = {};
    S.planes = planes; S.stem_w = n->stem_wm; S.stem_b = n->stem_b; S.stem_inv = n->stem_inv_scale; S.f0 = n->f0;
    S.df = n->df; S.batch = batch;
    auto role = [&](F16sArgs a, int wait, int need, int done) { a.df_wait = n->df + wait; a.df_need = need; a.df_done = n->df + done; a.df_err = n->df + kDfErr; return a; };
    S.L0 = role(layer_args(n, p, 0, n->f0, nullptr, n->g[0]), kDfStem, 1, kDfL0);
    S.L1 = role(layer_args(n, p, 1, n->g[0], n->f0, n->o[0]), kDfL0, 2, kDfL1);
    S.L2 = role(layer_args(n, p, 2, n->o[0], nullptr, n->g[1]), kDfL1, 2, kDfL2);
    S.L3 = role(layer_args(n, p, 3, n->g[1], n->o[0], n->o[1]), kDfL2, 4, kDfL3);
    S.P = role(layer_args(n, p, 6, n->o[1], nullptr, n->g[3]), kDfL3, 4, kDfP);
    S.V = role(block_args<4>(n, p, n->o[1]), kDfL3, 4, kDfV);
    S.Q = role(layer_args(n, p, 7, n->g[3], n->o[1], n->o[3]), kDfP, 2, kDfQ);
    S.B5 = role(block_args<8>(n, p, n->o[3]), kDfQ, 2, kDfB5);
    S.F = VfcArgs{n->hx[0], n->hfw[0], n->hfb[0], n->v2w, n->v2b, n->hf_inv[0], value};
    constexpr size_t ldsC = Lds<G, kDist>::kScrOff + (size_t)2 * 1 * 4 * 4096;
    constexpr size_t ldsV = Lds<G, 2>::kScrOff + (size_t)2 * 2 * 4096 * 2 + 36864;
    constexpr size_t ldsB = Lds<G, 2>::kScrOff + Lay<G>::kSlotL + 36864;
    constexpr size_t lds = std::max(std::max(ldsC, ldsV), std::max(ldsB, (size_t)StemLds<G>::kBytes));
    static_assert(lds + 256 <= 160 * 1024, "LDS budget (dynamic + the value head's static reduction buffer)");
    uint64_t bit;
    if (device_bit(&bit) || dyn_lds<af_small_forward_f16s<G>>(bit, (int)lds)) return -2;
    S.xp = n->hx[1]; S.pfa = n->hfw[1]; S.pfb = n->hfb[1]; S.pf_inv = n->hf_inv[1]; S.policy = policy; S.pfx = n->pfx;
    hipLaunchKernelGGL(af_small_forward_f16s<G>, dim3(19 * batch + 3), dim3(256), lds, st, S);
    FS_HIP_OK(hipGetLastError());
    return 0;
}

int f16s_forward(f16s_net* n, const F16sPlan& p, hipStream_t st, const float* planes, float* value, float* policy) {
    if (!n || p.form == kF16sBranches || p.batch < 1 || p.batch > n->max_batch || !planes || !value || !policy) return -1;
    if (p.form == kF16sRoles) return roles_forward(n, p, st, planes, value, policy);
    const int rc = f16s_trunk(n, p, st, planes);
    return rc ? rc : paired_branches(n, p, st, value, policy);
}
int f16s_small_forward_error(f16s_net* n) {
    if (!n || !n->df) return -1;
    int e = 0;
    FS_HIP_OK(hipDeviceSynchronize());
    FS_HIP_OK(hipMemcpy(&e, n->df + kDfErr, sizeof(int), hipMemcpyDeviceToHost));
    return e;
}

int f16s_read_activation(f16s_net* n, int which, int batch, float* host) {
    if (!n || batch < 1 || batch > n->max_batch) return -1;
    const char* bufs[9] = {n->f0, n->g[0], n->o[0], n->g[1], n->o[1], n->g[2], n->g[3], n->o[3], n->g[4]};
    const int chans[9] = {32, 64, 64, 128, 128, 32, 64, 64, 32};
    if (which < 0 || which > 8) return -1;
    const int C = chans[which];
    const bool s11 = n->S == 11;
    const size_t slab_h = (s11 ? Lay<Geo<11>>::kSlabH : Lay<Geo<15>>::kSlabH) / 2, half_h = slab_h / 2;
    const int rowu = s11 ? (int)Geo<11>::ROWU : (int)Geo<15>::ROWU, poff = s11 ? Geo<11>::POFF : Geo<15>::POFF, npix = n->S * n->S;
    std::vector<_Float16> h((size_t)batch * (C / 32) * slab_h);
    FS_HIP_OK(hipDeviceSynchronize());
    FS_HIP_OK(hipMemcpy(h.data(), bufs[which], h.size() * 2, hipMemcpyDeviceToHost));
    for (int b = 0; b < batch; ++b)
        for (int c = 0; c < C; ++c)
            for (int p = 0; p < npix; ++p) {
                const size_t slab = ((size_t)b * (C / 32) + c / 32) * slab_h;
                const size_t idx = slab + ((size_t)((c % 32) / 8) * rowu + p + poff) * 8 + c % 8;
                host[((size_t)b * C + c) * npix + p] = (float)h[idx] + (float)h[idx + half_h];
            }
    return C;
}

#ifdef AF_DF_TIMING
extern "C" int af_df_debug_wall(unsigned long long* host) {
    FS_HIP_OK(hipDeviceSynchronize());
    FS_HIP_OK(hipMemcpyFromSymbol(host, HIP_SYMBOL(g_df_wall), sizeof(unsigned long long) * 256 * 5));
    return 0;
}
#endif
#ifdef AF_F16S_TIMING
extern "C" int af_f16s_debug_cycles(unsigned long long* host) {
    FS_HIP_OK(hipDeviceSynchronize());
    FS_HIP_OK(hipMemcpyFromSymbol(host, HIP_SYMBOL(g_f16s_cycles), sizeof(unsigned long long) * 10 * 512 * 4 * 9));
    return 0;
}
extern "C" int af_f16s_debug_wall(unsigned long long* host) {
    FS_HIP_OK(hipDeviceSynchronize());
    FS_HIP_OK(hipMemcpyFromSymbol(host, HIP_SYMBOL(g_f16s_wall), sizeof(unsigned long long) * 10 * 512 * 2));
    return 0;
}
#endif
```

### alphafive_amd/csrc/af_engine.hip

```cpp

#include <hip/hip_runtime.h>
#include <stdint.h>
#include <stdio.h>
#include <stdlib.h>
#include <string.h>

#include <type_traits>
#include <vector>

#include "af_engine.h"
#include "af_noise.h"

typedef unsigned long long u64;

enum { PH_IDLE = 0, PH_MOVE_START = 1, PH_SEARCH = 2, PH_MOVE_DONE = 3, PH_ERROR = 4, PH_DESCENT = 5  };
enum { CT_SIMS = 0, CT_SELECTS, CT_EXPANDS, CT_TERMINALS, CT_PLIES, CT_EPISODES, CT_LSUM, CT_LEXP,
       CT_GC, CT_GC_SCANNED, CT_YIELDS, CT_STALLS, CT_N };
enum { HIST_WORK = 0, HIST_TIME = 64, HIST_MAXTIME = 96, HIST_N = 97 };

struct EngineParams {
    int G, S, C, goal, sims, upper, training, mode, node_cap, max_ply, budget, budget_hard;
    uint32_t hash_mask;
    double init_temp, tau_decay, tau_decay_r, alpha, c_puct;
    float c_puct32;
// ... 1141 lines not shown
        const int ph = P.phase[g];
        o[0] = P.action[g]; o[1] = P.has_policy[g];
        o[2] = ph == PH_MOVE_DONE ? 0 : (ph == PH_ERROR ? P.status[g] : AF_ERR_STATE);
        const u64 tb = (u64)__double_as_longlong(P.tau[g]);
        o[3] = (int32_t)(uint32_t)tb; o[4] = (int32_t)(uint32_t)(tb >> 32);
    }
    for (int c = lane; c < C; c += 64) {
        o[8 + c] = __float_as_int(P.policy[(size_t)g * CP + c]);
        o[8 + C + c] = P.visits[(size_t)g * CP + c];
    }
}

enum { MT_RUNNING = 0, MT_OVER = 1, MT_STOPPED = 2, MT_FAILED = 3, MT_UNUSED = 4 };
enum { MC_DONE = 0, MC_PLIES = 1, MC_ERROR = 2, MC_N = 3 };
struct MatchParams {
    int32_t* hdr;
    int32_t *ply, *ended, *result, *error;
    int32_t* moves;
    u64* counters;
};

__global__ __launch_bounds__(64) void af_match_start_kernel(EngineParams P0, EngineParams P1, MatchParams M, int n_games, int max_plies, int KW2) {
    const int g = blockIdx.x, lane = threadIdx.x, C = P0.C;
    if (g >= P0.G) return;
    if (g == 0 && lane == 0) {
        M.hdr[0] = n_games; M.hdr[1] = max_plies;
        for (int i = 0; i < MC_N; ++i) M.counters[i] = 0ull;
    }
    for (int c = lane; c < C; c += 64) M.moves[(size_t)g * C + c] = -1;
    if (lane == 0) {
        M.ply[g] = 0; M.ended[g] = g < n_games ? MT_RUNNING : MT_UNUSED; M.result[g] = AF_MATCH_UNFINISHED; M.error[g] = 0;
        P0.phase[g] = PH_IDLE; P0.pending[g] = 0; P0.status[g] = 0; P0.episode[g] = 0;
        P1.phase[g] = PH_IDLE; P1.pending[g] = 0; P1.status[g] = 0; P1.episode[g] = 0;
    }
    if (g < n_games) {
        if (g & 1) install_root(P1, g, lane, KW2, 0ull, -1, 1, 1);
        else install_root(P0, g, lane, KW2, 0ull, -1, 1, 1);
    }
}

template <int KW>
__device__ __forceinline__ void match_step_game(const EngineParams& P, const EngineParams& Q, const MatchParams& M, int g, int lane, int p, int ply,
                                                int max_plies) {
    const int phase = rfli(P.phase[g]);
    if (phase == PH_ERROR) {
        if (lane == 0) {
            const int code = P.status[g];
            M.error[g] = code; M.ended[g] = MT_FAILED;
            atomicCAS(reinterpret_cast<unsigned long long*>(&M.counters[MC_ERROR]), 0ull, (unsigned long long)(long long)code);
            atomicAdd(reinterpret_cast<unsigned long long*>(&M.counters[MC_DONE]), 1ull);
        }
        return;
    }
    if (phase != PH_MOVE_DONE) return;
    const int action = rfli(P.action[g]);
    u64 rm[KW], rt[KW];
#pragma unroll
    for (int k = 0; k < KW; ++k) {
        rm[k] = rfl64(P.root[(size_t)g * 2 * KW + k]);
        rt[k] = rfl64(P.root[(size_t)g * 2 * KW + KW + k]);
    }
    bool legal = action >= 0 && action < P.C && ply < P.C;
    if (legal) legal = !bb_test<KW>(rm, action) && !bb_test<KW>(rt, action);
    if (!legal) {
        if (lane == 0) {
            P.phase[g] = PH_IDLE; M.error[g] = AF_ERR_STATE; M.ended[g] = MT_FAILED;
            atomicCAS(reinterpret_cast<unsigned long long*>(&M.counters[MC_ERROR]), 0ull, (unsigned long long)(long long)AF_ERR_STATE);
            atomicAdd(reinterpret_cast<unsigned long long*>(&M.counters[MC_DONE]), 1ull);
        }
        return;
    }
    u64 nm[KW], nt[KW];
#pragma unroll
    for (int k = 0; k < KW; ++k) { nm[k] = rt[k]; nt[k] = rm[k]; }
    bb_set<KW>(nt, action);
    float fv;
    const int over = terminal_test<KW>(P, nm, nt, &fv);
    const int nply = ply + 1;
    if (lane == 0) {
        M.moves[(size_t)g * P.C + ply] = action;
        M.ply[g] = nply;
        P.phase[g] = PH_IDLE;
        atomicAdd(reinterpret_cast<unsigned long long*>(&M.counters[MC_PLIES]), 1ull);
        if (over) {
            M.result[g] = fv == 0.0f ? AF_MATCH_DRAW : p;
            M.ended[g] = MT_OVER;
        } else if (nply >= max_plies) {
            M.ended[g] = MT_STOPPED;
        }
        if (over || nply >= max_plies) atomicAdd(reinterpret_cast<unsigned long long*>(&M.counters[MC_DONE]), 1ull);
    }
    if (over || nply >= max_plies) return;
    install_root(Q, g, lane, 2 * KW, key_word<KW>(nm, nt, lane), action, 1, nply < 2 ? 1 : 0);
}

template <int KW>
__global__ __launch_bounds__(64) void af_match_step_kernel(EngineParams P0, EngineParams P1, MatchParams M) {
    const int g = blockIdx.x, lane = threadIdx.x;
    if (g >= rfli(M.hdr[0])) return;
    if (rfli(M.ended[g]) != MT_RUNNING) return;
    const int max_plies = rfli(M.hdr[1]);
    const int ply = rfli(M.ply[g]);
    const int p = (g + ply) & 1;
    if (p) match_step_game<KW>(P1, P0, M, g, lane, 1, ply, max_plies);
    else match_step_game<KW>(P0, P1, M, g, lane, 0, ply, max_plies);
}

template <int KW>
__global__ __launch_bounds__(64) void af_memo_insert_kernel(EngineParams P, const float* __restrict__ policy, const float* __restrict__ value) {
    constexpr int CP = 64 * KW, MK = 4 * KW;
    const int g = blockIdx.x, lane = threadIdx.x;
    if (!rfli(P.pending[g])) return;
    u64 lm[KW], lt[KW];
#pragma unroll
    for (int k = 0; k < KW; ++k) {
        lm[k] = rfl64(P.leaf[(size_t)g * 2 * KW + k]);
        lt[k] = rfl64(P.leaf[(size_t)g * 2 * KW + KW + k]);
    }
    if (bb_count<KW>(lm) + bb_count<KW>(lt) > P.memo_max_stones) return;
    const int last = rfli(P.leaf_last[g]);
    const uint32_t bucket = memo_bucket<KW>(P, lm, lt, last);
    uint32_t empty_ways;
    if (memo_probe<KW>(P, bucket, lm, lt, last, lane, &empty_ways) >= 0) return;
    const u64 serial = rfl64(P.memo_stats[MEMO_SERIAL]);
    const int way = empty_ways ? __builtin_ctz(empty_ways) : (int)((key_hash<KW>(lm, lt) >> 24) + (uint32_t)serial) & 3;
    const size_t e = (size_t)bucket * 4 + way;
    int own = 0;
    if (lane == 0) own = atomicMax(reinterpret_cast<unsigned long long*>(&P.memo_lock[e]), (unsigned long long)serial) < serial ? 1 : 0;
    if (!rfli(own)) return;
    if (lane < MK) P.memo_key[e * MK + lane] = memo_word<KW>(P, lm, lt, last, lane);
#pragma unroll
    for (int k = 0; k < KW; ++k) {
        const int c = lane + 64 * k;
        P.memo_pv[e * CP + c] = c < P.C ? policy[(size_t)g * P.C + c] : 0.0f;
    }
    if (lane == 0) {
        P.memo_val[e] = value[g];
        atomicAdd(reinterpret_cast<unsigned long long*>(&P.memo_stats[MEMO_INSERTS]), 1ull);
        if (!empty_ways) atomicAdd(reinterpret_cast<unsigned long long*>(&P.memo_stats[MEMO_REPLACED]), 1ull);
    }
}

struct af_engine {
    EngineParams P;
    int device;
    int KW;
    std::vector<void*> allocs;
    std::vector<int32_t> h_i32, h_i32b;
    char* stage_dev = nullptr;
    size_t stage_cap = 0;
    std::vector<int32_t> pack_host;
    std::vector<u64> h_ct;
    unsigned long long* stamps = nullptr;
    bool memo = false;
    bool memo_budget_fixed = false;
    size_t memo_entries = 0;
};

struct af_match {
    af_engine *e0, *e1;
    MatchParams M;
    int device, G, C;
    int32_t* block = nullptr;
    void* small = nullptr;
    std::vector<int32_t> host;
    bool started = false;
};

#define HIP_OK(x) do { hipError_t e_ = (x); if (e_ != hipSuccess) { fprintf(stderr, "[af_engine] %s failed: %s\n", #x, hipGetErrorString(e_)); return AF_ERR_HIP; } } while (0)

template <typename T>
static int dalloc(af_engine* e, T** p, size_t n) {
    void* q = nullptr;
    if (hipMalloc(&q, n * sizeof(T)) != hipSuccess) {
        fprintf(stderr, "[af_engine] hipMalloc of %zu bytes failed (node_cap / num_games too large for the device?)\n", n * sizeof(T));
        (void)hipGetLastError();
        return AF_ERR_HIP;
    }
    HIP_OK(hipMemset(q, 0, n * sizeof(T)));
    e->allocs.push_back(q);
    *p = (T*)q;
    return AF_OK;
}

static int stage_reserve(af_engine* e, size_t bytes) {
    if (e->stage_cap >= bytes) return AF_OK;
    if (e->stage_dev) (void)hipFree(e->stage_dev);
    e->stage_dev = nullptr; e->stage_cap = 0;
    HIP_OK(hipMalloc((void**)&e->stage_dev, bytes * 2));
    e->stage_cap = bytes * 2;
    return AF_OK;
}

static bool valid_position(const EngineParams& P, int KW, const uint64_t* key) {
    for (int k = 0; k < KW; ++k)
        if (((key[k] | key[KW + k]) & ~P.boardmask[k]) || (key[k] & key[KW + k])) return false;
    return true;
}

#define WITH_KW(kw, ...) do { if ((kw) == 2) { constexpr int KW_ = 2; __VA_ARGS__; } else { constexpr int KW_ = 4; __VA_ARGS__; } } while (0)
#define WITH_FLAG(flag, NAME, ...) do { if (flag) { constexpr bool NAME = true; __VA_ARGS__; } else { constexpr bool NAME = false; __VA_ARGS__; } } while (0)

static int live_nodes(af_engine* e, int game, std::vector<int32_t>& bs, int* live) {
    const EngineParams& P = e->P;
    HIP_OK(hipDeviceSynchronize());
    int32_t hw;
    HIP_OK(hipMemcpy(&hw, P.nodes + game, 4, hipMemcpyDeviceToHost));
    bs.resize((size_t)(hw > 0 ? hw : 0));
    if (hw > 0) HIP_OK(hipMemcpy(bs.data(), P.node_sum + (size_t)game * P.node_cap, (size_t)hw * 4, hipMemcpyDeviceToHost));
    *live = 0;
    for (int32_t v : bs) *live += v >= 0;
    return AF_OK;
}

template <typename D, typename S>
static void rows_out(D* dst, const std::vector<S>& src, const std::vector<int32_t>& bs, int W, int C) {
    size_t o = 0;
    for (size_t i = 0; i < bs.size(); ++i) {
        if (bs[i] < 0) continue;
        for (int c = 0; c < C; ++c) dst[o * C + c] = (D)src[i * W + c];
        ++o;
    }
}
template <typename D, typename S>
static std::vector<D> rows_in(const S* src, int count, int W, int C) {
    std::vector<D> dst((size_t)count * W, D(0));
    for (size_t i = 0; i < (size_t)count; ++i)
        for (int c = 0; c < C; ++c) dst[i * W + c] = (D)src[i * C + c];
    return dst;
}

extern "C" {

int af_abi_version(void) { return AF_ABI_VERSION; }

const char* af_strerror(int code) {
    switch (code) {
        case AF_OK: return "ok";
        case AF_ERR_ARG: return "bad argument";
        case AF_ERR_HIP: return "HIP runtime error";
        case AF_ERR_NODE_CAP: return "transposition store full (raise node_cap)";
        case AF_ERR_NO_ROOT: return "get_action on a finished position";
        case AF_ERR_EP_OVERRUN: return "finished episodes not popped in time";
        case AF_ERR_STATE: return "engine state error";
        default: return "unknown error";
    }
}

int af_engine_create(const af_config* cfg, int32_t num_games, int32_t device, int32_t mode, int32_t training,
                     uint64_t seed, uint32_t first_game_id, int32_t node_cap, af_engine** out) {
    if (!cfg || !out || num_games < 1) return AF_ERR_ARG;
    const int S = cfg->board_size, C = S * S;
    if (S < 2 || C > 256 || cfg->goal < 2 || cfg->goal > S || cfg->simulation_per_step < 1) return AF_ERR_ARG;
    const int value_f64 = (mode & AF_MODE_VALUE_F64) ? 1 : 0;
    mode &= ~AF_MODE_VALUE_F64;
    if (mode != AF_MODE_SELFPLAY && mode != AF_MODE_EXTERNAL) return AF_ERR_ARG;
    if (!(cfg->dirichlet_alpha > 0.0 && cfg->dirichlet_alpha < 1.0)) return AF_ERR_ARG;
    if (cfg->upper_simulation_per_step < 1 || !(cfg->c_puct >= 0.0)) return AF_ERR_ARG;
    HIP_OK(hipSetDevice(device));
    af_engine* e = new af_engine();
    e->device = device;
    e->KW = C <= 128 ? 2 : 4;
    const int KW = e->KW, CP = 64 * KW;
    EngineParams& P = e->P;
    memset(&P, 0, sizeof(P));
    P.G = num_games; P.S = S; P.C = C; P.goal = cfg->goal;
    P.sims = cfg->simulation_per_step; P.upper = cfg->upper_simulation_per_step;
    P.training = training ? 1 : 0; P.mode = mode; P.max_ply = C; P.w64 = value_f64;
    P.budget = AF_DEFAULT_TICK_BUDGET; P.budget_hard = AF_DEFAULT_TICK_BUDGET_HARD;
    if (const char* b = getenv("AF_TICK_BUDGET")) { const int v = atoi(b); if (v > 0) P.budget = v; }
    if (const char* b = getenv("AF_TICK_BUDGET_HARD")) { const int v = atoi(b); if (v > 0) P.budget_hard = v; }
    if (P.budget_hard < P.budget) P.budget_hard = P.budget;
    if (node_cap <= 0) node_cap = mode == AF_MODE_SELFPLAY ? 4 * P.sims + 64 : 32768;
    if (node_cap < P.sims + 8) node_cap = P.sims + 8;
    P.node_cap = node_cap;
    uint32_t hcap = 64;
    while (hcap < 2u * (uint32_t)node_cap) hcap <<= 1;
    P.hash_mask = hcap - 1;
    P.init_temp = cfg->init_temp; P.tau_decay = cfg->tau_decay_rate; P.tau_decay_r = cfg->tau_decay_rate_r;
    P.alpha = cfg->dirichlet_alpha; P.c_puct = cfg->c_puct; P.c_puct32 = (float)cfg->c_puct;
    P.k0 = af_key0(seed); P.seed_hi = (uint32_t)(seed >> 32); P.first_game_id = first_game_id;
    for (int c = 0; c < C; ++c) {
        P.boardmask[c >> 6] |= 1ull << (c & 63);
        if (c % S <= S - cfg->goal) P.colmask[c >> 6] |= 1ull << (c & 63);
    }
    const size_t G = num_games;
    int rc = AF_OK;
#define A(p, n) if (rc == AF_OK) rc = dalloc(e, &P.p, (n))
    A(phase, G); A(pending, G); A(sims_left, G); A(ply, G); A(root_last, G); A(nodes, G); A(nfree, G); A(depth, G);
    A(leaf_last, G); A(leaf_slot, G); A(status, G); A(random_a, G); A(action, G); A(has_policy, G);
    A(visits, G * CP); A(policy, G * CP); A(root, G * 2 * KW); A(leaf, G * 2 * KW); A(tau, G);
    A(episode, G); A(sel, G); A(plyctr, G); A(path_node, G * CP); A(path_cell, G * CP);
    A(hash, G * hcap); A(node_key, G * node_cap * 2 * KW); A(node_sum, G * node_cap); A(free_idx, G * node_cap);
    A(edge_n, G * node_cap * CP); A(edge_p, G * node_cap * CP); A(edge_c, G * node_cap * CP);
    if (value_f64) { A(edge_w64, G * node_cap * CP); A(edge_w, 64); } else { A(edge_w, G * node_cap * CP); A(edge_w64, 8); }
    A(ep_seq, G); A(ep_popped, G); A(counters, G * CT_N); A(progress, 2); A(hist, HIST_N);
    if (mode == AF_MODE_SELFPLAY) {
        const size_t R = G * 2 * P.max_ply;
        A(ep_len, G * 2); A(ep_final, G * 2); A(rec_key, R * 2 * KW); A(rec_policy, R * C); A(rec_visits, R * C);
        A(rec_last, R); A(rec_action, R);
    }
#undef A
    if (rc == AF_OK) rc = dalloc(e, &e->stamps, (size_t)AF_STAMP_SLOTS);
    if (rc != AF_OK) { af_engine_destroy(e); return rc; }
    std::vector<int32_t> ph(G, mode == AF_MODE_SELFPLAY ? PH_MOVE_START : PH_IDLE), rl(G, -1);
    std::vector<double> tau(G, cfg->init_temp);
    HIP_OK(hipMemcpy(P.phase, ph.data(), G * 4, hipMemcpyHostToDevice));
    HIP_OK(hipMemcpy(P.root_last, rl.data(), G * 4, hipMemcpyHostToDevice));
    HIP_OK(hipMemcpy(P.tau, tau.data(), G * 8, hipMemcpyHostToDevice));
    e->h_i32.resize(G); e->h_i32b.resize(G); e->h_ct.resize(G * CT_N);
    *out = e;
    return AF_OK;
}

void af_engine_destroy(af_engine* e) {
    if (!e) return;
    (void)hipSetDevice(e->device);
    for (void* p : e->allocs) (void)hipFree(p);
    if (e->stage_dev) (void)hipFree(e->stage_dev);
    delete e;
}

int32_t af_engine_num_games(const af_engine* e) { return e->P.G; }
int32_t af_engine_cells(const af_engine* e) { return e->P.C; }
int32_t af_engine_key_words(const af_engine* e) { return 2 * e->KW; }
int32_t af_engine_max_plies(const af_engine* e) { return e->P.max_ply; }

int af_engine_tick(af_engine* e, void* stream, const float* policy_dev, const float* value_dev, float* planes_dev) {
    if (!e || !planes_dev) return AF_ERR_ARG;
    hipStream_t st = (hipStream_t)stream;
    WITH_FLAG(e->memo, MEMO_, WITH_KW(e->KW, WITH_FLAG(e->P.w64, W64_,
        hipLaunchKernelGGL((af_tick_kernel<KW_, W64_, MEMO_>), dim3(e->P.G), dim3(64), 0, st, e->P, policy_dev, value_dev, planes_dev))));
    HIP_OK(hipGetLastError());
    return AF_OK;
}

int af_engine_memo_enable(af_engine* e, int32_t log2_buckets, int32_t max_stones) {
    if (!e || e->memo || log2_buckets < 4 || log2_buckets > 28 || max_stones < 0) return AF_ERR_ARG;
    HIP_OK(hipSetDevice(e->device));
    EngineParams& P = e->P;
    const size_t NE = (size_t)4 << log2_buckets, CP = 64 * (size_t)e->KW, MK = 4 * (size_t)e->KW;
    int rc = AF_OK;
    if (rc == AF_OK) rc = dalloc(e, &P.memo_key, NE * MK);
    if (rc == AF_OK) rc = dalloc(e, &P.memo_pv, NE * CP);
    if (rc == AF_OK) rc = dalloc(e, &P.memo_val, NE);
    if (rc == AF_OK) rc = dalloc(e, &P.memo_lock, NE);
    if (rc == AF_OK) rc = dalloc(e, &P.memo_stats, (size_t)MEMO_N);
    if (rc != AF_OK) return rc;
    P.memo_bucket_mask = (uint32_t)((1ull << log2_buckets) - 1ull);
    P.memo_max_stones = max_stones;
    P.memo_epoch = 1;
    P.memo_budget = P.budget < 6 ? P.budget : 6;
    if (const char* b = getenv("AF_MEMO_BUDGET")) { const int v = atoi(b); if (v > 0) { P.memo_budget = v; e->memo_budget_fixed = true; } }
    e->memo_entries = NE;
    e->memo = true;
    return AF_OK;
}

int af_engine_memo_insert(af_engine* e, void* stream, const float* policy_dev, const float* value_dev) {
    if (!e || !e->memo || !policy_dev || !value_dev) return AF_ERR_ARG;
    hipStream_t st = (hipStream_t)stream;
    WITH_KW(e->KW, hipLaunchKernelGGL((af_memo_insert_kernel<KW_>), dim3(e->P.G), dim3(64), 0, st, e->P, policy_dev, value_dev));
    HIP_OK(hipGetLastError());
    return AF_OK;
}

int af_engine_memo_clear(af_engine* e, void* stream) {
    if (!e || !e->memo) return AF_ERR_ARG;
    hipStream_t st = (hipStream_t)stream;
    if (e->P.memo_epoch == 0xffffffffu) {
        HIP_OK(hipMemsetAsync(e->P.memo_key, 0, e->memo_entries * 4 * (size_t)e->KW * 8, st));
        e->P.memo_epoch = 1;
    } else {
        ++e->P.memo_epoch;
    }
    return AF_OK;
}

int64_t af_engine_memo_epoch(af_engine* e) { return (e && e->memo) ? (int64_t)e->P.memo_epoch : 0; }

int af_engine_memo_stats(af_engine* e, void* stream, uint64_t* out) {
    if (!e || !e->memo || !out) return AF_ERR_ARG;
    hipStream_t st = (hipStream_t)stream;
    HIP_OK(hipMemcpyAsync(out, e->P.memo_stats, (size_t)MEMO_N * 8, hipMemcpyDeviceToHost, st));
    HIP_OK(hipStreamSynchronize(st));
    out[MEMO_N] = (uint64_t)e->memo_entries;
    return AF_OK;
}

int af_engine_status(af_engine* e, void* stream, int32_t* status_host) {
    if (!e || !status_host) return AF_ERR_ARG;
    hipStream_t st = (hipStream_t)stream;
    HIP_OK(hipMemcpyAsync(status_host, e->P.status, (size_t)e->P.G * 4, hipMemcpyDeviceToHost, st));
    HIP_OK(hipStreamSynchronize(st));
    for (int g = 0; g < e->P.G; ++g) if (status_host[g] < 0) return status_host[g];
    return AF_OK;
}

int af_engine_set_training(af_engine* e, int32_t training) {
    if (!e) return AF_ERR_ARG;
    e->P.training = training ? 1 : 0;
    return AF_OK;
}

int af_engine_set_simulations(af_engine* e, int32_t sims, int32_t upper) {
    if (!e || sims < 1 || upper < 1 || sims + 8 > e->P.node_cap) return AF_ERR_ARG;
    e->P.sims = sims;
    e->P.upper = upper;
    return AF_OK;
}

int af_engine_set_root(af_engine* e, int32_t game, const uint64_t* key, int32_t last_cell, int32_t random_a,
                       int32_t reset_tree) {
    if (!e || !key || game < 0 || game >= e->P.G || e->P.mode != AF_MODE_EXTERNAL) return AF_ERR_ARG;
    if (last_cell < -1 || last_cell >= e->P.C) return AF_ERR_ARG;
    HIP_OK(hipDeviceSynchronize());
    return af_engine_set_roots(e, nullptr, 1, &game, key, &last_cell, &random_a, &reset_tree);
}

int af_engine_set_roots(af_engine* e, void* stream, int32_t n, const int32_t* games, const uint64_t* keys, const int32_t* last_cells,
                        const int32_t* random_a, const int32_t* reset_tree) {
    if (!e || e->P.mode != AF_MODE_EXTERNAL || n < 0 || (n > 0 && (!games || !keys || !last_cells))) return AF_ERR_ARG;
    if (n == 0) return AF_OK;
    EngineParams& P = e->P;
    const int KW = e->KW, KW2 = 2 * KW;
    std::vector<int32_t> req((size_t)4 * n);
    for (int i = 0; i < n; ++i) {
        if (games[i] < 0 || games[i] >= P.G || last_cells[i] < -1 || last_cells[i] >= P.C) return AF_ERR_ARG;
        if (!valid_position(P, KW, keys + (size_t)i * KW2)) return AF_ERR_ARG;
        req[4 * i] = games[i]; req[4 * i + 1] = last_cells[i]; req[4 * i + 2] = random_a ? random_a[i] : 0; req[4 * i + 3] = reset_tree ? reset_tree[i] : 0;
    }
    hipStream_t st = (hipStream_t)stream;
    const size_t rb = (size_t)4 * n * 4, kb = (size_t)n * KW2 * 8;
    if (int rc = stage_reserve(e, rb + kb)) return rc;
    HIP_OK(hipMemcpyAsync(e->stage_dev, req.data(), rb, hipMemcpyHostToDevice, st));
    HIP_OK(hipMemcpyAsync(e->stage_dev + rb, keys, kb, hipMemcpyHostToDevice, st));
    hipLaunchKernelGGL(af_set_roots_kernel, dim3(n), dim3(64), 0, st, P, n, (const int32_t*)e->stage_dev, (const u64*)(e->stage_dev + rb), KW2);
    HIP_OK(hipGetLastError());
    HIP_OK(hipStreamSynchronize(st));
    return AF_OK;
}

int af_engine_move_results(af_engine* e, void* stream, int32_t n, const int32_t* games, int32_t* action_cells, int32_t* has_policy,
                           float* policies, int32_t* visits, double* taus) {
    if (!e || n < 0 || (n > 0 && (!games || !action_cells))) return AF_ERR_ARG;
    if (n == 0) return AF_OK;
    EngineParams& P = e->P;
    for (int i = 0; i < n; ++i) if (games[i] < 0 || games[i] >= P.G) return AF_ERR_ARG;
    hipStream_t st = (hipStream_t)stream;
    const int C = P.C, R = 8 + 2 * C, CP = 64 * e->KW;
    const size_t gb = (size_t)n * 4, ob = (size_t)n * R * 4;
    if (int rc = stage_reserve(e, gb + ob)) return rc;
    HIP_OK(hipMemcpyAsync(e->stage_dev, games, gb, hipMemcpyHostToDevice, st));
    hipLaunchKernelGGL(af_move_results_kernel, dim3(n), dim3(64), 0, st, P, n, (const int32_t*)e->stage_dev, (int32_t*)(e->stage_dev + gb), CP);
    HIP_OK(hipGetLastError());
    std::vector<int32_t> out((size_t)n * R);
    HIP_OK(hipMemcpyAsync(out.data(), e->stage_dev + gb, ob, hipMemcpyDeviceToHost, st));
    HIP_OK(hipStreamSynchronize(st));
    for (int i = 0; i < n; ++i) {
        const int32_t* o = out.data() + (size_t)i * R;
        if (o[2] != 0) return o[2];
        action_cells[i] = o[0];
        if (has_policy) has_policy[i] = o[1];
        if (policies) memcpy(policies + (size_t)i * C, o + 8, (size_t)C * 4);
        if (visits) memcpy(visits + (size_t)i * C, o + 8 + C, (size_t)C * 4);
        if (taus) { const uint64_t tb = (uint64_t)(uint32_t)o[3] | ((uint64_t)(uint32_t)o[4] << 32); memcpy(taus + i, &tb, 8); }
    }
    return AF_OK;
}

int af_engine_move_result(af_engine* e, int32_t game, int32_t* action_cell, int32_t* has_policy, float* policy,
                          int32_t* visits, double* tau) {
    if (!e || game < 0 || game >= e->P.G) return AF_ERR_ARG;
    HIP_OK(hipDeviceSynchronize());
    int32_t cell;
    const int rc = af_engine_move_results(e, nullptr, 1, &game, &cell, has_policy, policy, visits, tau);
    if (rc == AF_OK && action_cell) *action_cell = cell;
    return rc;
}

int64_t af_engine_pack_ints(const af_engine* e, int32_t max_episodes, int32_t max_plies) {
    if (!e || max_episodes < 0 || max_plies < 0) return AF_ERR_ARG;
    const int64_t R = 4 * e->KW + 2 * e->P.C + 2;
    return 4 + (int64_t)max_episodes * 5 + (int64_t)max_plies * R;
}

// ... 354 lines not shown
```

### alphafive_amd/csrc/af_net.hip

```cpp

#include <hip/hip_runtime.h>
#include <stdint.h>
#include <stdio.h>
#include <string.h>

#include <map>
#include <string>
#include <vector>

#include "af_net.h"
#include "af_conv_f16s.h"

typedef float f32x16 __attribute__((ext_vector_type(16)));
typedef float f4u __attribute__((ext_vector_type(4), aligned(4)));
typedef float f2u __attribute__((ext_vector_type(2), aligned(4)));
typedef float f2a __attribute__((ext_vector_type(2)));

__device__ __forceinline__ float elu1(float x) { return x > 0.0f ? x : __expf(x) - 1.0f; }

struct WinoArgs {
    const float* in;
    const float* u;
    const float* in2;
    const float* u2;
// ... 704 lines not shown
    float* stage = nullptr;
    NET_HIP_OK(hipMalloc((void**)&stage, image.size() * sizeof(float)));
    f16s_dev_vars D;
    size_t off = 0;
    for (auto& kv : n->vars) { D[kv.first] = stage + off; off += kv.second.size(); }
    rc = hipMemcpy(stage, image.data(), image.size() * sizeof(float), hipMemcpyHostToDevice) == hipSuccess ? AF_NET_OK : AF_NET_ERR_HIP;
    if (!rc) rc = pack_from_device(n, nullptr, D);
    if (!rc && hipStreamSynchronize(nullptr) != hipSuccess) rc = AF_NET_ERR_HIP;
    (void)hipFree(stage);
    n->ready = rc == AF_NET_OK;
    return rc;
}

int af_net_update_device(af_net* n, void* stream, const char* const* tf_names, const float* const* dev_ptrs, const int64_t* counts,
                         int32_t nvars) {
    if (!n || !tf_names || !dev_ptrs || !counts) return AF_NET_ERR_ARG;
    if (n->allocs.empty()) return AF_NET_ERR_STATE;
    if (nvars != (int32_t)n->expect.size()) return AF_NET_ERR_ARG;
    f16s_dev_vars D;
    for (int i = 0; i < nvars; ++i) {
        if (!tf_names[i] || !dev_ptrs[i]) return AF_NET_ERR_ARG;
        auto it = n->expect.find(tf_names[i]);
        if (it == n->expect.end() || (int64_t)it->second != counts[i]) return AF_NET_ERR_NAME;
        if (!D.emplace(it->first, dev_ptrs[i]).second) return AF_NET_ERR_ARG;
    }
    hipStream_t st = (hipStream_t)stream;
    hipStreamCaptureStatus cap = hipStreamCaptureStatusNone;
    NET_HIP_OK(hipStreamIsCapturing(st, &cap));
    if (cap != hipStreamCaptureStatusNone) return AF_NET_ERR_STATE;
    NET_HIP_OK(hipSetDevice(n->device));
    const int rc = pack_from_device(n, st, D);
    if (rc) return rc;
    n->vars.clear();
    n->ready = true;
    return AF_NET_OK;
}

int64_t af_net_debug_weights(af_net* n, int32_t index, void* host_out, int64_t cap_bytes) {
    if (!n || index < 0 || n->allocs.empty()) return AF_NET_ERR_ARG;
    const void* p = nullptr;
    size_t bytes = 0;
    const int n32 = (int)n->wreg.size();
    if (index < n32) { p = n->wreg[index].first; bytes = n->wreg[index].second; }
    else if (!n->f16s || f16s_weight_buffer(n->f16s, index - n32, &p, &bytes)) return AF_NET_ERR_ARG;
    if (!host_out) return (int64_t)bytes;
    if (cap_bytes < (int64_t)bytes) return AF_NET_ERR_ARG;
    NET_HIP_OK(hipSetDevice(n->device));
    NET_HIP_OK(hipDeviceSynchronize());
    NET_HIP_OK(hipMemcpy(host_out, p, bytes, hipMemcpyDeviceToHost));
    return (int64_t)bytes;
}

int32_t af_net_debug_scales(af_net* n, float* host_out, int32_t cap) {
    if (!n || !host_out || cap < 0) return AF_NET_ERR_ARG;
    return n->f16s ? f16s_scales(n->f16s, host_out, cap) : 0;
}

}

static int g_f16s_abl = 0;
static int g_wino = 5;

static void launch_wino(hipStream_t st, const af_net* n, int batch, const float* in, const float* u, int cin,
                        const float* in2, const float* u2, int cin2, const float* bias, float* out, int cout) {
    WinoArgs a;
    a.in = in; a.u = u; a.in2 = in2; a.u2 = u2; a.bias = bias; a.out = out;
    a.cin = cin; a.cin2 = cin2; a.cout = cout; a.T = n->T; a.S = n->S; a.WP = n->WP; a.PP = n->PP;
    a.ntiles = batch * n->T * n->T;
    const int ntb = (a.ntiles + 31) / 32;
    const int ngrp8 = (((ntb + 3) / 4) + 7) / 8 * 8;
    hipLaunchKernelGGL(af_conv_wino, dim3(ngrp8 * (cout / 32)), dim3(256), 0, st, a);
}


static int g_phead = 1;
static int g_branch = 1;
static int g_fhead = 1;

static int forward_range(af_net* n, hipStream_t st, const float* planes_all, int b0, int batch, float* policy_all, float* value_all) {
    const int S = n->S, HW = n->HW, WP = n->WP, PP = n->PP;
    const float* planes = planes_all + (size_t)b0 * 3 * HW;
    float* policy = policy_all + (size_t)b0 * HW;
    float* value = value_all + b0;
    const size_t po = (size_t)b0 * PP;
    float* f0 = n->f0 + po * 32;
    float* g[5];
    float* o[5];
    for (int i = 0; i < 5; ++i) { g[i] = n->g[i] + po * kBlocks[i].cout; o[i] = n->o[i] + po * kBlocks[i].cout; }
    const bool split16 = g_wino == 5 && n->f16s != nullptr;
    const bool fhead = split16 && g_fhead;
    F16sPlan plan = {};
    if (split16) {
        plan = f16s_plan(n->f16s, batch, g_f16s_abl, fhead);
        if (plan.form != kF16sBranches) return f16s_forward(n->f16s, plan, st, planes, value, policy) ? AF_NET_ERR_HIP : AF_NET_OK;
        if (f16s_trunk(n->f16s, plan, st, planes)) return AF_NET_ERR_HIP;
    } else {
        hipLaunchKernelGGL(af_stem_conv, dim3(batch), dim3(256), 0, st, planes, n->stem_w, n->stem_b, f0, S, WP, PP);
    }
    const float* block_in[5] = {f0, o[0], o[1], o[1], o[3]};
    hipStream_t vs = st;
    if (g_branch && n->branch_stream && (!split16 || g_branch == 2)) {
        vs = n->branch_stream;
    }
    for (int i = split16 ? 2 : 0; i < 5; ++i) {
        const Block& b = kBlocks[i];
        hipStream_t st_main = st;
        if (i == 2 && vs != st_main) {
            NET_HIP_OK(hipEventRecord(n->ev_trunk, st_main));
            NET_HIP_OK(hipStreamWaitEvent(vs, n->ev_trunk, 0));
        }
        hipStream_t st = (i == 2) ? vs : st_main;
        if (split16) {
            if (i == 2 && f16s_value_branch(n->f16s, plan, st, o[2], WP, PP, value)) return AF_NET_ERR_HIP;
            if (i == 4 && f16s_policy_branch(n->f16s, plan, st, o[4], WP, PP, policy)) return AF_NET_ERR_HIP;
        } else {
            launch_wino(st, n, batch, block_in[i], n->wino1_u[i], b.cin, nullptr, nullptr, 0, n->conv1_b[i], g[i], b.cout);
            launch_wino(st, n, batch, g[i], n->wino2_u[i], b.cout, block_in[i], n->winor_u[i], b.cin, n->sum_b[i], o[i], b.cout);
        }
        if (i == 2) {
            if (!fhead)
            hipLaunchKernelGGL(af_value_head, dim3((batch + VPB - 1) / VPB), dim3(256), 0, st, o[2], n->vc_w, n->vc_b, n->v1_w, n->v1_b,
                               n->v2_w, n->v2_b, value, batch, S, WP, PP);
            if (vs != st_main) NET_HIP_OK(hipEventRecord(n->ev_value, vs));
        }
    }
    if (fhead) {
    } else if (HW <= 128 && g_phead) {
        const int K = 16 * HW, KS = K + ((2 - K % 32) + 32) % 32;
        const size_t lds = (size_t)16 * KS * 4;
        hipLaunchKernelGGL(af_policy_head_mfma, dim3((batch + 15) / 16), dim3(256), lds, st, o[4], n->pc_w, n->pc_b, n->pf_w,
                           n->pf_b, policy, batch, S, WP, PP);
    } else if (HW <= 128) {
        const size_t lds = ((size_t)16 * HW * 8 + 512 + 32) * 4;
        hipLaunchKernelGGL((af_policy_head<8>), dim3((batch + 7) / 8), dim3(256), lds, st, o[4], n->pc_w, n->pc_b, n->pf_w,
                           n->pf_b, policy, batch, S, WP, PP);
    } else {
        const size_t lds = ((size_t)16 * HW * 4 + 512 + 16) * 4;
        hipLaunchKernelGGL((af_policy_head<4>), dim3((batch + 3) / 4), dim3(256), lds, st, o[4], n->pc_w, n->pc_b, n->pf_w,
                           n->pf_b, policy, batch, S, WP, PP);
    }
    if (vs != st) NET_HIP_OK(hipStreamWaitEvent(st, n->ev_value, 0));
    NET_HIP_OK(hipGetLastError());
    return AF_NET_OK;
}

extern "C" {

int af_net_forward(af_net* n, void* stream, const float* planes, int32_t batch, float* policy, float* value) {
    if (!n || !planes || !policy || !value || batch < 1 || batch > n->max_batch) return AF_NET_ERR_ARG;
    if (!n->ready) return AF_NET_ERR_STATE;
    return forward_range(n, (hipStream_t)stream, planes, 0, batch, policy, value);
}

int af_net_tune(int32_t key, int32_t value) {
    if (key == 0) { if (value != 1 && value != 5) return AF_NET_ERR_ARG; g_wino = value; return AF_NET_OK; }
    if (key == 5) { g_phead = value; return AF_NET_OK; }
    if (key == 4) { g_branch = value; return AF_NET_OK; }
    if (key == 9) { g_fhead = value ? 1 : 0; return AF_NET_OK; }
    if (key == 7) { g_f16s_abl = value; return AF_NET_OK; }
    return AF_NET_ERR_ARG;
}

int af_net_debug_activation(af_net* n, int32_t which, int32_t batch, float* host_out) {
    if (!n || !host_out || !n->f16s) return AF_NET_ERR_ARG;
    const int c = f16s_read_activation(n->f16s, which, batch, host_out);
    return c < 0 ? AF_NET_ERR_ARG : c;
}

int af_net_small_forward_error(af_net* n) {
    if (!n || !n->f16s) return AF_NET_ERR_ARG;
    return f16s_small_forward_error(n->f16s);
}

int64_t af_net_flops_per_position(const af_net* n) {
    const int64_t HW = n->HW;
    int64_t mac = 75 * 32 * HW;
    for (const Block& b : kBlocks) mac += ((int64_t)9 * b.cin * b.cout + (int64_t)9 * b.cout * b.cout + (int64_t)b.cin * b.cout) * HW;
    mac += 32 * 4 * HW + 4 * HW * 64 + 64 + 32 * 16 * HW + 16 * HW * HW;
    return 2 * mac;
}

}
```

### alphafive_amd/engine.py

```python
import ctypes as C
import os

import numpy as np

_PKG = os.path.dirname(os.path.abspath(__file__))
_LIBPATH = os.environ.get("AF_HIP_LIB") or os.path.join(_PKG, "_lib", "libaf_hip.so")

MODE_SELFPLAY, MODE_EXTERNAL = 0, 1
MODE_VALUE_F64 = 0x100
STATUS_IDLE, STATUS_NEED_EVAL, STATUS_MOVE_DONE, STATUS_YIELD = 0, 1, 2, 3
STAMP_SLOTS = 64
BLACK_WIN, WHITE_WIN, DRAW = 1, -1, 0

CFG_ATTRS = ("board_size", "goal", "simulation_per_step", "upper_simulation_per_step", "init_temp", "gamma",
             "tau_decay_rate", "tau_decay_rate_r", "dirichlet_alpha", "c_puct")


class AfConfig(C.Structure):
    _fields_ = [("board_size", C.c_int32), ("goal", C.c_int32), ("simulation_per_step", C.c_int32),
                ("upper_simulation_per_step", C.c_int32), ("init_temp", C.c_double), ("gamma", C.c_double),
                ("tau_decay_rate", C.c_double), ("tau_decay_rate_r", C.c_double), ("dirichlet_alpha", C.c_double),
                ("c_puct", C.c_double)]

    @classmethod
    def from_cfg(cls, cfg):
        return cls(*[getattr(cfg, a) for a in CFG_ATTRS])


class EngineError(RuntimeError):
    pass


_lib = None


def lib():
    global _lib
    if _lib is None:
        if not os.path.exists(_LIBPATH):
            raise EngineError(f"{_LIBPATH} not found: build the HIP engine first "
                              f"(python -m alphafive_amd.build). There is no CPU fallback.")
        import torch
        L = C.CDLL(_LIBPATH)
        vp = C.c_void_p
        i32p, f32p, u64p, u8p = (C.POINTER(C.c_int32), C.POINTER(C.c_float), C.POINTER(C.c_uint64),
                                 C.POINTER(C.c_uint8))
        L.af_abi_version.restype = C.c_int
        L.af_strerror.restype = C.c_char_p
        L.af_strerror.argtypes = [C.c_int]
        L.af_engine_create.argtypes = [C.POINTER(AfConfig), C.c_int32, C.c_int32, C.c_int32, C.c_int32, C.c_uint64,
                                       C.c_uint32, C.c_int32, C.POINTER(vp)]
        L.af_engine_destroy.argtypes = [vp]
        L.af_engine_destroy.restype = None
        for fn in ("af_engine_num_games", "af_engine_cells", "af_engine_key_words", "af_engine_max_plies"):
            getattr(L, fn).argtypes = [vp]
            getattr(L, fn).restype = C.c_int32
        L.af_engine_tick.argtypes = [vp, vp, vp, vp, vp]
        L.af_engine_status.argtypes = [vp, vp, i32p]
        L.af_engine_set_root.argtypes = [vp, C.c_int32, u64p, C.c_int32, C.c_int32, C.c_int32]
        L.af_engine_move_result.argtypes = [vp, C.c_int32, i32p, i32p, f32p, i32p, C.POINTER(C.c_double)]
        L.af_engine_set_training.argtypes = [vp, C.c_int32]
        L.af_engine_set_simulations.argtypes = [vp, C.c_int32, C.c_int32]
        L.af_engine_set_roots.argtypes = [vp, vp, C.c_int32, i32p, u64p, i32p, i32p, i32p]
        L.af_engine_move_results.argtypes = [vp, vp, C.c_int32, i32p, i32p, i32p, f32p, i32p, C.POINTER(C.c_double)]
        L.af_engine_pop_episodes.argtypes = [vp, vp, C.c_int32, i32p, f32p, u64p, f32p, i32p, i32p, i32p]
        L.af_engine_pack_ints.argtypes = [vp, C.c_int32, C.c_int32]
        L.af_engine_pack_ints.restype = C.c_int64
        L.af_engine_pack_episodes.argtypes = [vp, vp, C.c_int32, C.c_int32, vp]
        L.af_engine_counters.argtypes = [vp, vp, u64p]
        L.af_engine_tree_w64.argtypes = [vp, C.c_int32, C.c_int32, C.POINTER(C.c_double)]
        L.af_engine_set_tree_w64.argtypes = [vp, C.c_int32, C.c_int32, C.POINTER(C.c_double)]
        L.af_engine_progress.argtypes = [vp, vp, u64p]
        L.af_engine_progress_async.argtypes = [vp, vp, vp]
        L.af_engine_stamp.argtypes = [vp, vp, C.c_int32]
        L.af_engine_stamps_async.argtypes = [vp, vp, vp]
        L.af_engine_tick_histogram.argtypes = [vp, vp, u64p, C.c_int32]
        L.af_engine_set_tick_budget.argtypes = [vp, C.c_int32]
        L.af_engine_memo_enable.argtypes = [vp, C.c_int32, C.c_int32]
        L.af_engine_memo_insert.argtypes = [vp, vp, vp, vp]
        L.af_engine_memo_clear.argtypes = [vp, vp]
        L.af_engine_memo_stats.argtypes = [vp, vp, u64p]
        L.af_engine_memo_epoch.argtypes = [vp]
        L.af_engine_memo_epoch.restype = C.c_int64
        L.af_match_create.argtypes = [vp, vp, C.POINTER(vp)]
        L.af_match_destroy.argtypes = [vp]
        L.af_match_destroy.restype = None
        L.af_match_start.argtypes = [vp, vp, C.c_int32, C.c_int32]
        L.af_match_step.argtypes = [vp, vp]
        L.af_match_progress_async.argtypes = [vp, vp, vp]
        L.af_match_results.argtypes = [vp, vp, i32p, i32p, i32p]
        L.af_engine_tree_dump.argtypes = [vp, C.c_int32, C.c_int32, u64p, i32p, i32p, f32p, f32p, u8p]
        L.af_engine_load_tree.argtypes = [vp, C.c_int32, C.c_int32, u64p, i32p, i32p, f32p, f32p, u8p]
        L.af_state_to_key.argtypes = [C.c_char_p, C.c_int32, u64p]
        L.af_key_to_state.argtypes = [u64p, C.c_int32, C.c_char_p, C.c_int32]
        _lib = L
    return _lib


def _check(rc, what):
    if rc < 0:
        raise EngineError(f"{what}: {lib().af_strerror(rc).decode()} (code {rc})")
    return rc


def _p(a, ct):
    return a.ctypes.data_as(C.POINTER(ct))


def key_words(S):
    return 4 if S * S <= 128 else 8


def state_to_key(state, S):
    key = np.zeros(key_words(S), np.uint64)
    _check(lib().af_state_to_key(state.encode(), S, _p(key, C.c_uint64)), "af_state_to_key")
    return key


def key_to_state(key, S):
    key = np.ascontiguousarray(key, np.uint64)
    out = C.create_string_buffer(288)
    _check(lib().af_key_to_state(_p(key, C.c_uint64), S, out, 288), "af_key_to_state")
    return out.value.decode()


COUNTER_NAMES = ("sims", "selects", "expands", "terminals", "plies", "episodes", "legal_sum", "legal_sum_expand",
                 "nodes", "collector_runs", "collector_scanned", "yields", "stalls")


class Engine:

    def __init__(self, cfg, num_games, device=0, mode=MODE_SELFPLAY, training=True, seed=0, first_game_id=0,
                 node_cap=0, value_f64=False):
        self._h = C.c_void_p()
        self.cfg = AfConfig.from_cfg(cfg) if not isinstance(cfg, AfConfig) else cfg
        self.value_f64 = bool(value_f64) or bool(mode & MODE_VALUE_F64)
        mode = (mode & ~MODE_VALUE_F64) | (MODE_VALUE_F64 if self.value_f64 else 0)
        _check(lib().af_engine_create(C.byref(self.cfg), num_games, device, mode, int(training), seed, first_game_id,
                                      node_cap, C.byref(self._h)), "af_engine_create")
        self.G = num_games
        self.S = self.cfg.board_size
        self.C = self.S * self.S
        self.KW2 = lib().af_engine_key_words(self._h)
        self.max_plies = lib().af_engine_max_plies(self._h)
        self.mode = mode & ~MODE_VALUE_F64
        self.device = device
        self._status = np.zeros(num_games, np.int32)
        self._params = {"training": int(bool(training)), "sims": int(self.cfg.simulation_per_step),
                        "upper": int(self.cfg.upper_simulation_per_step), "tick_budget": None}

    def close(self):
        if getattr(self, "_h", None):
            lib().af_engine_destroy(self._h)
            self._h = None

    __del__ = close

    def tick(self, policy_ptr, value_ptr, planes_ptr, stream=None):
        _check(lib().af_engine_tick(self._h, stream, policy_ptr, value_ptr, planes_ptr), "af_engine_tick")

    def status(self, stream=None):
        rc = lib().af_engine_status(self._h, stream, _p(self._status, C.c_int32))
        _check(rc, "engine status")
        return self._status

    def params_key(self):
        p = self._params
        return (p["training"], p["sims"], p["upper"], p["tick_budget"], p.get("memo_epoch"), p.get("memo"))

    def set_training(self, training):
        _check(lib().af_engine_set_training(self._h, int(training)), "af_engine_set_training")
        self._params["training"] = int(bool(training))

    def set_simulations(self, sims, upper):
        _check(lib().af_engine_set_simulations(self._h, int(sims), int(upper)), "af_engine_set_simulations")
        self._params["sims"], self._params["upper"] = int(sims), int(upper)

    def set_root(self, game, key, last_cell=-1, random_a=False, reset_tree=False):
        key = np.ascontiguousarray(key, np.uint64)
        _check(lib().af_engine_set_root(self._h, game, _p(key, C.c_uint64), last_cell, int(random_a), int(reset_tree)),
               "af_engine_set_root")

    def move_result(self, game):
        a, hp, tau = C.c_int32(-1), C.c_int32(0), C.c_double(0)
        pol = np.zeros(self.C, np.float32)
        vis = np.zeros(self.C, np.int32)
        _check(lib().af_engine_move_result(self._h, game, C.byref(a), C.byref(hp), _p(pol, C.c_float),
                                           _p(vis, C.c_int32), C.byref(tau)), "af_engine_move_result")
        return a.value, (pol if hp.value else None), vis, tau.value

    def set_roots(self, games, keys, last_cells, random_a=False, reset_tree=False, stream=None):
        n = len(games)
        g = np.ascontiguousarray(games, np.int32)
        k = np.ascontiguousarray(keys, np.uint64).reshape(n, self.KW2)
        lc = np.ascontiguousarray(last_cells, np.int32)
        ra = np.ascontiguousarray(np.broadcast_to(np.asarray(random_a, np.int32), (n,)))
        rt = np.ascontiguousarray(np.broadcast_to(np.asarray(reset_tree, np.int32), (n,)))
        _check(lib().af_engine_set_roots(self._h, stream, n, _p(g, C.c_int32), _p(k, C.c_uint64), _p(lc, C.c_int32),
                                         _p(ra, C.c_int32), _p(rt, C.c_int32)), "af_engine_set_roots")

    def move_results(self, games, stream=None):
        n = len(games)
        g = np.ascontiguousarray(games, np.int32)
        act, hp = np.zeros(n, np.int32), np.zeros(n, np.int32)
        pol, vis, tau = np.zeros((n, self.C), np.float32), np.zeros((n, self.C), np.int32), np.zeros(n, np.float64)
        _check(lib().af_engine_move_results(self._h, stream, n, _p(g, C.c_int32), _p(act, C.c_int32), _p(hp, C.c_int32),
                                            _p(pol, C.c_float), _p(vis, C.c_int32), _p(tau, C.c_double)), "af_engine_move_results")
        return act, hp, pol, vis, tau

    def counters(self, stream=None):
        out = np.zeros(len(COUNTER_NAMES), np.uint64)
        _check(lib().af_engine_counters(self._h, stream, _p(out, C.c_uint64)), "af_engine_counters")
        return {k: int(v) for k, v in zip(COUNTER_NAMES, out)}

    def tick_histogram(self, stream=None, reset=False):
        out = np.zeros(97, np.uint64)
        _check(lib().af_engine_tick_histogram(self._h, stream, _p(out, C.c_uint64), int(reset)), "tick_histogram")
        return dict(selects=out[:64].astype(np.int64), wave_us=out[64:96].astype(np.int64),
                    max_wave_us=float(out[96]) * 0.01)

    def memo_enable(self, log2_buckets=18, max_stones=5):
        _check(lib().af_engine_memo_enable(self._h, int(log2_buckets), int(max_stones)), "af_engine_memo_enable")
        kw = self.KW2 // 2
        self.memo_bytes = (4 << int(log2_buckets)) * (32 * kw + 256 * kw + 12)
        self._params["memo"] = (int(log2_buckets), int(max_stones))
        self._params["memo_epoch"] = int(lib().af_engine_memo_epoch(self._h))

    @property
    def memo(self):
        return self._params.get("memo")

    def memo_insert(self, policy_ptr, value_ptr, stream=None):
        _check(lib().af_engine_memo_insert(self._h, stream, policy_ptr, value_ptr), "af_engine_memo_insert")

    def memo_clear(self, stream=None):
        _check(lib().af_engine_memo_clear(self._h, stream), "af_engine_memo_clear")
        self._params["memo_epoch"] = int(lib().af_engine_memo_epoch(self._h))

    def memo_stats(self, stream=None):
        out = np.zeros(6, np.uint64)
        _check(lib().af_engine_memo_stats(self._h, stream, _p(out, C.c_uint64)), "af_engine_memo_stats")
        return {k: int(v) for k, v in zip(("launches", "probes", "hits", "inserts", "replaced", "entries"), out)}

    def set_tick_budget(self, selects_per_launch):
        _check(lib().af_engine_set_tick_budget(self._h, int(selects_per_launch)), "af_engine_set_tick_budget")
        self._params["tick_budget"] = int(selects_per_launch)

    def progress(self, stream=None):
        out = np.zeros(2, np.uint64)
        _check(lib().af_engine_progress(self._h, stream, _p(out, C.c_uint64)), "af_engine_progress")
        return int(out[0]), int(out[1])

    def progress_async(self, out_ptr, stream=None):
        _check(lib().af_engine_progress_async(self._h, stream, out_ptr), "af_engine_progress_async")

    def stamp(self, slot, stream=None):
        _check(lib().af_engine_stamp(self._h, stream, int(slot)), "af_engine_stamp")

    def stamps_async(self, out_ptr, stream=None):
        _check(lib().af_engine_stamps_async(self._h, stream, out_ptr), "af_engine_stamps_async")

    def tree_dump(self, game):
        cnt = _check(lib().af_engine_tree_dump(self._h, game, 0, None, None, None, None, None, None), "tree_dump")
        keys = np.zeros((cnt, self.KW2), np.uint64)
        sum_n = np.zeros(cnt, np.int32)
        n = np.zeros((cnt, self.C), np.int32)
        w = np.zeros((cnt, self.C), np.float32)
        p = np.zeros((cnt, self.C), np.float32)
        f = np.zeros((cnt, self.C), np.uint8)
        if cnt:
            _check(lib().af_engine_tree_dump(self._h, game, cnt, _p(keys, C.c_uint64), _p(sum_n, C.c_int32),
                                             _p(n, C.c_int32), _p(w, C.c_float), _p(p, C.c_float), _p(f, C.c_uint8)),
                   "tree_dump")
            if self.value_f64:
                w = np.zeros((cnt, self.C), np.float64)
                _check(lib().af_engine_tree_w64(self._h, game, cnt, _p(w, C.c_double)), "af_engine_tree_w64")
        return dict(keys=keys, sum_n=sum_n, n=n, w=w, p=p, f32=f)

    def load_tree(self, game, dump):
        cnt = len(dump["sum_n"])
        arr = {k: np.ascontiguousarray(dump[k], t) for k, t in (("keys", np.uint64), ("sum_n", np.int32), ("n", np.int32),
                                                                 ("w", np.float32), ("p", np.float32), ("f32", np.uint8))}
        _check(lib().af_engine_load_tree(self._h, game, cnt, _p(arr["keys"], C.c_uint64), _p(arr["sum_n"], C.c_int32),
                                         _p(arr["n"], C.c_int32), _p(arr["w"], C.c_float), _p(arr["p"], C.c_float),
                                         _p(arr["f32"], C.c_uint8)), "af_engine_load_tree")
        if self.value_f64:
            w64 = np.ascontiguousarray(dump["w"], np.float64)
            _check(lib().af_engine_set_tree_w64(self._h, game, cnt, _p(w64, C.c_double)), "af_engine_set_tree_w64")

    def pack_ints(self, max_eps, max_plies):
        return int(_check(lib().af_engine_pack_ints(self._h, max_eps, max_plies), "af_engine_pack_ints"))

    def pack_episodes(self, out_ptr, max_eps, max_plies, stream=None):
        _check(lib().af_engine_pack_episodes(self._h, stream, max_eps, max_plies, out_ptr), "af_engine_pack_episodes")


def unpack_episodes(buf, max_eps):
    buf = np.ascontiguousarray(buf, np.int32)
    n, _, K, Cc = (int(x) for x in buf[:4])
    R = 2 * K + 2 * Cc + 2
    head = 4 + 5 * max_eps
    out = []
    for i in range(n):
        g, seq, T, p0 = (int(x) for x in buf[4 + 4 * i:8 + 4 * i])
        rec = buf[head + p0 * R:head + (p0 + T) * R].reshape(T, R)
        out.append(dict(game=g, seq=seq, T=T, final_value=float(buf[4 + 4 * max_eps + i:5 + 4 * max_eps + i].view(np.float32)[0]),
                        keys=np.ascontiguousarray(rec[:, :2 * K]).view(np.uint64).reshape(T, K).copy(),
                        policies=np.ascontiguousarray(rec[:, 2 * K:2 * K + Cc]).view(np.float32).copy(),
                        visits=rec[:, 2 * K + Cc:2 * K + 2 * Cc].copy(),
                        lasts=rec[:, 2 * K + 2 * Cc].copy(), actions=rec[:, 2 * K + 2 * Cc + 1].copy()))
    return out


def packed_used_ints(hdr, max_eps):
    n_plies, K, Cc = int(hdr[1]), int(hdr[2]), int(hdr[3])
    return 4 + 5 * max_eps + n_plies * (2 * K + 2 * Cc + 2)


def assemble_episode(raw, S, gamma):
    from . import utils
    T = raw["T"]
    value = float(raw["final_value"])
    if T % 2 == 1:
        value = -value
    weights = utils.construct_weights(T, gamma=gamma)
    rec = []
    for t in range(T):
        la = None if raw["lasts"][t] < 0 else (int(raw["lasts"][t]) // S, int(raw["lasts"][t]) % S)
        rec.append((key_to_state(raw["keys"][t], S), raw["policies"][t].reshape(S, S).copy(), la, value, weights[t]))
        value = -value
    last_value = rec[-1][-2]
    if last_value == 0.0:
        result = DRAW
    elif T % 2 == 1:
        result = BLACK_WIN
    else:
        result = WHITE_WIN
    return rec, result


def resolve_weights_version(pv, explicit=None):
    if explicit is not None:
        return (explicit if callable(explicit) else (lambda: explicit)), False
    ver = getattr(pv, "weights_version", None)
    if callable(ver):
        return ver, False
    owner = getattr(pv, "__self__", None)
    if owner is not None and hasattr(owner, "version"):
        return (lambda: owner.version), False
    return None, hasattr(pv, "bind_outputs")


class SelfPlayEngine:

    def __init__(self, cfg, num_games, pv_device, device=0, seed=0, first_game_id=0, training=True, node_cap=0,
                 value_f64=False, weights_version=None, eval_memo=None):
        import torch
        if not torch.cuda.is_available():
            raise EngineError("SelfPlayEngine needs a HIP device (torch.cuda.is_available() is False)")
        self.torch = torch
        self.cfg = cfg
        self.dev = torch.device("cuda", device)
        torch.cuda.set_device(self.dev)
        self.engine = Engine(cfg, num_games, device=device, mode=MODE_SELFPLAY, training=training, seed=seed,
                             first_game_id=first_game_id, node_cap=node_cap, value_f64=value_f64)
        S = cfg.board_size
        self.G, self.S, self.C = num_games, S, S * S
        self.planes = torch.zeros((num_games, 3, S, S), dtype=torch.float32, device=self.dev)
        self.policy = torch.zeros((num_games, S * S), dtype=torch.float32, device=self.dev)
        self.value = torch.zeros((num_games,), dtype=torch.float32, device=self.dev)
        self.pv_device = pv_device
        self._weights_version = self._resolve_weights_version(weights_version)
        if hasattr(pv_device, "bind_outputs"):
            pv_device.bind_outputs(self.policy, self.value)
        self._memo_version = None
        if eval_memo:
            if self._weights_version is None:
                raise EngineError("eval_memo: the evaluator exposes no weights_version (the memo could not tell when to forget); "
                                  "pass SelfPlayEngine(..., weights_version=lambda: net.version)")
            self.engine.memo_enable(**({} if eval_memo is True else dict(eval_memo)))
            self._memo_version = self._weights_version()
        self.ticks = 0
        self._boxes = {}
        self._graph = None
        self._prog_host, self._prog_events, self._prog_turn, self._prog_replays = None, None, 0, 0
        self.replay_events = []
        self._graph_stamped, self._stamp_host, self._stamp_event, self._stamp_pending, self.stamp_samples = None, None, None, False, []

    def tick(self, stamp_base=None):
        torch = self.torch
        stream = torch.cuda.current_stream(self.dev).cuda_stream
        if stamp_base is not None:
            self.engine.stamp(stamp_base, stream)
        memo = self.engine.memo is not None
        if memo:
            ver = self._weights_version()
            if ver != self._memo_version:
                self.engine.memo_clear(stream)
                self._memo_version = ver
        self.engine.tick(self.policy.data_ptr(), self.value.data_ptr(), self.planes.data_ptr(), stream)
        if stamp_base is not None:
            self.engine.stamp(stamp_base + 1, stream)
        p, v = self.pv_device(self.planes)
        if p.data_ptr() != self.policy.data_ptr():
            self.policy.copy_(p.reshape(self.G, self.C))
        if v.data_ptr() != self.value.data_ptr():
            self.value.copy_(v.reshape(self.G))
        if memo:
            self.engine.memo_insert(self.policy.data_ptr(), self.value.data_ptr(), stream)
        if stamp_base is not None:
            self.engine.stamp(stamp_base + 2, stream)
        self.ticks += 1

    def run_ticks(self, n, check_every=0):
        for i in range(n):
            self.tick()
            if check_every and (i + 1) % check_every == 0:
                self.check()

    def _resolve_weights_version(self, explicit):
        ver, missing = resolve_weights_version(self.pv_device, explicit)
        if missing:
            self._weights_version_missing = True
        return ver

    def _graph_key(self, n):
        ver = self._weights_version
        return (int(n), self.engine.params_key(), ver() if ver is not None else None)

    def run_ticks_graph(self, n=16, timed=False, stamped=False):
        torch = self.torch
        if getattr(self, "_weights_version_missing", False):
            raise EngineError("run_ticks_graph: pv_device takes bind_outputs but exposes no weights_version (a replayed graph "
                              "would keep evaluating with stale weights); pass SelfPlayEngine(..., weights_version=lambda: net.version)")
        key = self._graph_key(n)
        if stamped:
            if 3 * n > STAMP_SLOTS:
                raise EngineError("run_ticks_graph(stamped=True): at most %d ticks per replay" % (STAMP_SLOTS // 3))
            if self._graph_stamped is None or self._graph_stamped[0] != key:
                self._graph_stamped = None
                if self._graph is None or self._graph[0] != key:
                    self.run_ticks_graph(n)
                if self._stamp_host is None:
                    self._stamp_host = torch.zeros(STAMP_SLOTS, dtype=torch.int64, pin_memory=True)
                    self._stamp_event = torch.cuda.Event()
                torch.cuda.synchronize(self.dev)
                g = torch.cuda.CUDAGraph()
                with torch.cuda.graph(g, capture_error_mode="thread_local"):
                    for i in range(n):
                        self.tick(stamp_base=3 * i)
                    st = torch.cuda.current_stream(self.dev).cuda_stream
                    self.engine.stamps_async(self._stamp_host.data_ptr(), st)
                    self.engine.progress_async(self._prog_host.data_ptr(), st)
                self.ticks -= n
                self._graph_stamped = (self._graph_key(n), g, n)
            if self._stamp_pending:
                self._collect_stamps()
            self._graph_stamped[1].replay()
            self._stamp_event.record(torch.cuda.current_stream(self.dev))
            self._stamp_pending = True
            self.ticks += n
            self._prog_turn ^= 1
            self._prog_events[self._prog_turn].record(torch.cuda.current_stream(self.dev))
            self._prog_replays += 1
            return
        if self._graph is None or self._graph[0] != key:
            self._graph = None
            if self._prog_host is None:
                self._prog_host = torch.zeros(2, dtype=torch.int64, pin_memory=True)
                self._prog_events = [torch.cuda.Event(), torch.cuda.Event()]
            self.tick()
            torch.cuda.synchronize(self.dev)
            g = torch.cuda.CUDAGraph()
            with torch.cuda.graph(g, capture_error_mode="thread_local"):
                for _ in range(n):
                    self.tick()
                st = torch.cuda.current_stream(self.dev).cuda_stream
                self.engine.progress_async(self._prog_host.data_ptr(), st)
            self.ticks -= n
            self._graph = (self._graph_key(n), g)
        if timed:
            e0, e1 = torch.cuda.Event(enable_timing=True), torch.cuda.Event(enable_timing=True)
            e0.record(torch.cuda.current_stream(self.dev))
        self._graph[1].replay()
        if timed:
            e1.record(torch.cuda.current_stream(self.dev))
            self.replay_events.append((n, e0, e1))
        self.ticks += n
        self._prog_turn ^= 1
        self._prog_events[self._prog_turn].record(torch.cuda.current_stream(self.dev))
        self._prog_replays += 1

    def _collect_stamps(self):
        self._stamp_event.synchronize()
        t = self._stamp_host.numpy().astype(np.int64)[:3 * self._graph_stamped[2]].reshape(-1, 3)
        self.stamp_samples.append(np.stack([(t[:, 1] - t[:, 0]) * 1e-5, (t[:, 2] - t[:, 1]) * 1e-5], axis=1))
        self._stamp_pending = False

    def read_stamps(self):
        if self._stamp_pending:
            self._collect_stamps()
        return np.concatenate(self.stamp_samples) if self.stamp_samples else np.zeros((0, 2))

    def progress_lagged(self):
        if self._prog_replays < 2:
            return 0, 0
        self._prog_events[self._prog_turn ^ 1].synchronize()
        return int(self._prog_host[0]), int(self._prog_host[1])

    def check(self):
        stream = self.torch.cuda.current_stream(self.dev).cuda_stream
        return self.engine.status(stream)

    def counters(self):
        return self.engine.counters(self.torch.cuda.current_stream(self.dev).cuda_stream)

    def progress(self):
        return self.engine.progress(self.torch.cuda.current_stream(self.dev).cuda_stream)

    def _pack_plies(self, cap):
        return max(cap * 40, int(self.engine.max_plies))

    def _outbox(self, cap):
        box = self._boxes.get(cap)
        if box is None:
            torch = self.torch
            max_plies = self._pack_plies(cap)
            ints = self.engine.pack_ints(cap, max_plies)
            box = dict(cap=cap, max_plies=max_plies, buf=torch.zeros(ints, dtype=torch.int32, pin_memory=True),
                       event=torch.cuda.Event(), posted=False)
            self._boxes[cap] = box
        return box

    def post_episodes(self, cap=256):
        box = self._outbox(cap)
        if box["posted"]:
            raise EngineError("post_episodes: the previous post has not been collected")
        stream = self.torch.cuda.current_stream(self.dev)
        self.engine.pack_episodes(box["buf"].data_ptr(), cap, box["max_plies"], stream.cuda_stream)
        box["event"].record(stream)
        box["posted"] = True
        return box

    def collect_episodes(self, cap=256, unpack=True):
        box = self._outbox(cap)
        if not box["posted"]:
            return [] if unpack else None
        box["event"].synchronize()
        box["posted"] = False
        return unpack_episodes(box["buf"].numpy(), cap) if unpack else box["buf"].numpy()

    def pop_raw(self, cap=256):
        self.post_episodes(cap)
        return self.collect_episodes(cap)

    def post_episodes_device(self, cap=256):
# ... 14 lines not shown
```

### alphafive_amd/net_hip.py

```python
import ctypes as C
import os

import numpy as np
import torch

_PKG = os.path.dirname(os.path.abspath(__file__))
_LIBPATH = os.environ.get("AF_NET_LIB") or os.path.join(_PKG, "_lib", "libaf_net.so")
_lib = None


class NetError(RuntimeError):
    pass


def lib():
    global _lib
    if _lib is None:
        if not os.path.exists(_LIBPATH):
            raise ImportError(f"{_LIBPATH} not built (python -m alphafive_amd.build)")
        import torch
        L = C.CDLL(_LIBPATH)
        vp = C.c_void_p
        L.af_net_create.argtypes = [C.c_int32, C.c_int32, C.c_int32, C.POINTER(vp)]
        L.af_net_destroy.argtypes = [vp]
        L.af_net_destroy.restype = None
        L.af_net_set_variable.argtypes = [vp, C.c_char_p, C.POINTER(C.c_float), C.c_int64]
        L.af_net_finalize.argtypes = [vp]
        L.af_net_forward.argtypes = [vp, vp, vp, C.c_int32, vp, vp]
        L.af_net_update_device.argtypes = [vp, vp, C.POINTER(C.c_char_p), C.POINTER(vp), C.POINTER(C.c_int64), C.c_int32]
        L.af_net_debug_weights.argtypes = [vp, C.c_int32, vp, C.c_int64]
        L.af_net_debug_weights.restype = C.c_int64
        L.af_net_debug_scales.argtypes = [vp, C.POINTER(C.c_float), C.c_int32]
        L.af_net_debug_scales.restype = C.c_int32
        L.af_net_flops_per_position.argtypes = [vp]
        L.af_net_flops_per_position.restype = C.c_int64
        L.af_net_small_forward_error.argtypes = [vp]
        L.af_net_strerror.argtypes = [C.c_int]
        L.af_net_strerror.restype = C.c_char_p
        _lib = L
    return _lib


def _check(rc, what):
    if rc < 0:
        raise NetError(f"{what}: {lib().af_net_strerror(rc).decode()} (code {rc})")


class HipNet(object):

    def __init__(self, variables, board_size, max_batch, device):
        self.S, self.max_batch, self.device = board_size, max_batch, torch.device(device)
        self._h = C.c_void_p()
        self._version = 0
        idx = self.device.index if self.device.index is not None else torch.cuda.current_device()
        _check(lib().af_net_create(board_size, max_batch, idx, C.byref(self._h)), "af_net_create")
        self.load(variables)
        self.flops_per_position = int(lib().af_net_flops_per_position(self._h))
        self.policy = torch.empty((max_batch, board_size * board_size), dtype=torch.float32, device=self.device)
        self.value = torch.empty((max_batch,), dtype=torch.float32, device=self.device)

    def load(self, variables):
        torch.cuda.synchronize(self.device)
        for name, arr in variables.items():
            a = np.ascontiguousarray(arr, np.float32)
            _check(lib().af_net_set_variable(self._h, name.encode(), a.ctypes.data_as(C.POINTER(C.c_float)), a.size),
                   f"af_net_set_variable({name})")
        _check(lib().af_net_finalize(self._h), "af_net_finalize")
        self._version += 1

    def load_device(self, tensors):
        names, ptrs, counts = [], [], []
        for name, t in tensors.items():
            if not (torch.is_tensor(t) and t.is_cuda and t.dtype == torch.float32 and t.is_contiguous()):
                raise NetError(f"load_device({name}): a contiguous float32 tensor on {self.device} is required")
            if t.device.index != (self.device.index if self.device.index is not None else torch.cuda.current_device()):
                raise NetError(f"load_device({name}): tensor on {t.device}, handle on {self.device}")
            names.append(name.encode())
            ptrs.append(t.data_ptr())
            counts.append(t.numel())
        n = len(names)
        stream = torch.cuda.current_stream(self.device).cuda_stream
        _check(lib().af_net_update_device(self._h, stream, (C.c_char_p * n)(*names), (C.c_void_p * n)(*ptrs), (C.c_int64 * n)(*counts), n),
               "af_net_update_device")
        self._version += 1

    def debug_weights(self):
        out = []
        while True:
            size = lib().af_net_debug_weights(self._h, len(out), None, 0)
            if size < 0:
                return out
            buf = np.empty(size, np.uint8)
            _check(lib().af_net_debug_weights(self._h, len(out), buf.ctypes.data_as(C.c_void_p), size), "af_net_debug_weights")
            out.append(buf)

    def debug_scales(self):
        buf = np.zeros(64, np.float32)
        n = lib().af_net_debug_scales(self._h, buf.ctypes.data_as(C.POINTER(C.c_float)), buf.size)
        _check(n, "af_net_debug_scales")
        return buf[:n].copy()

    def weights_version(self):
        return self._version

    def bind_outputs(self, policy, value):
        assert policy.is_contiguous() and value.is_contiguous() and policy.dtype == torch.float32
        assert policy.shape[0] >= self.max_batch or policy.shape[0] == value.shape[0]
        self.policy, self.value = policy, value

    def __call__(self, planes):
        B = planes.shape[0]
        assert B <= self.max_batch and planes.is_contiguous() and planes.dtype == torch.float32
        stream = torch.cuda.current_stream(self.device).cuda_stream
        _check(lib().af_net_forward(self._h, stream, planes.data_ptr(), B, self.policy.data_ptr(), self.value.data_ptr()),
               "af_net_forward")
        return self.policy[:B], self.value[:B]

    def small_forward_error(self):
        return int(lib().af_net_small_forward_error(self._h))

    def close(self):
        if getattr(self, "_h", None):
            try:
                lib().af_net_destroy(self._h)
            except Exception:
                pass
            self._h = None

    __del__ = close


def make_eval(resnet):
    if resnet.device.type != "cuda" or not (3 <= resnet.board_size <= 15):
        return None
    lib()
    state = {"net": None, "out": None, "version": None}

    def pv(planes):
        B = planes.shape[0]
        if state["net"] is None or state["net"].max_batch < B:
            if state["net"] is not None:
                state["net"].close()
            state["net"] = HipNet(resnet.variables, resnet.board_size, B, resnet.device)
            state["version"] = getattr(resnet, "version", None)
            if state["out"] is not None and state["out"][0].shape[0] >= B:
                state["net"].bind_outputs(*state["out"])
        elif state["version"] != getattr(resnet, "version", None):
            version = getattr(resnet, "version", None)
            snap = resnet.device_snapshot() if hasattr(resnet, "device_snapshot") else None
            if snap is not None:
                tensors, event = snap
                stream = torch.cuda.current_stream(resnet.device)
                stream.wait_event(event)
                state["net"].load_device(tensors)
                for t in tensors.values():
                    t.record_stream(stream)
            else:
                state["net"].load(resnet.variables)
            state["version"] = version
        return state["net"](planes)

    def bind_outputs(policy, value):
        state["out"] = (policy, value)
        if state["net"] is not None and policy.shape[0] >= state["net"].max_batch:
            state["net"].bind_outputs(policy, value)

    def close():
        if state["net"] is not None:
            state["net"].close()
            state["net"] = None

    pv.bind_outputs = bind_outputs
    pv.close = close
    pv.weights_version = lambda: getattr(resnet, "version", None)
    return pv


_SPLIT_MAC_PER_PIXEL = sum(9 * ci * co + 9 * co * co + ci * co for ci, co in ((32, 64), (64, 128), (128, 32), (128, 64), (64, 32)))
_SPLIT_BYTES_PER_POSITION = (28 * 16384 + 17 * 15488 + 2 * (4 + 16) * 121 * 2 * 2 + 3 * 121 * 4 + 122 * 4)


_conv_mode = 5


def roofline_info(board_size=11):
    if board_size == 15 and _conv_mode == 5:
        return {"backend": "hip (af_conv_f16s.hip on 15x15: two half-board pseudo-positions per board, fp16 split operands, fp32 "
                           "accumulation; MFMA stem and fused heads as on 11x11)",
                "kernel": "af_net_forward = af_stem_mfma_f16s<Geo<15>> + 10x af_conv_f16s<Geo<15>> (the last conv of each branch also "
                          "applies the head's 1x1 convolution) + af_value_fc_f16s<Geo<15>> + af_policy_fc_f16s<Geo<15>> (whole "
                          "forward timed)",
                "peak_tflops": 2500.0, "issued_flop_per_position": 2 * 3 * _SPLIT_MAC_PER_PIXEL * 256,
                "algorithmic_bytes_per_position": (30 * 2 * 20480 + 19 * 30720 + 2 * 2 * 2 * 16384 + 2 * (4 + 16) * 225 * 2 * 2 + 3 * 225 * 4 + 226 * 4)}
    if board_size == 11 and _conv_mode == 5:
        return {"backend": "hip (af_conv_f16s.hip: stem, convs and heads on v_mfma_f32_32x32x16_f16 with fp16 split operands and "
                           "fp32 accumulation; convs weight-stationary with an LDS-DMA slab ring)",
                "kernel": "af_net_forward = af_stem_mfma_f16s + 6x af_conv_f16s + 2x af_block_f16s (blocks 3 and 5: both convolutions "
                          "and the head's 1x1 convolution in one kernel, the intermediate in LDS) + af_value_fc_f16s + af_policy_fc_f16s "
                          "(whole forward timed; the convolution kernels carry 99 % of the algorithmic FLOPs, each MAC issued as 3 fp16 MFMA MACs)",
                "peak_tflops": 2500.0, "issued_flop_per_position": 2 * 3 * _SPLIT_MAC_PER_PIXEL * 121,
                "algorithmic_bytes_per_position": _SPLIT_BYTES_PER_POSITION}
    return {"backend": "hip (af_net.hip: fp32 MFMA Winograd F(2x2,3x3) convs, fused transforms/bias/ELU/residual)",
            "kernel": "af_net_forward = af_stem_conv + 10x af_conv_wino + af_value_head + af_policy_head "
                      "(whole forward timed; af_conv_wino carries 97 % of the algorithmic FLOPs; achieved = "
                      "direct-convolution FLOPs / time, the MFMAs issued are 2.25x fewer on the 3x3 layers)",
            "peak_tflops": 157.3}


def tune(key, value):
    global _conv_mode
    lib().af_net_tune.argtypes = [C.c_int32, C.c_int32]
    _check(lib().af_net_tune(key, value), "af_net_tune")
    if key == 0:
        _conv_mode = int(value)
```

### include/af_engine.h

```cpp
#ifndef AF_ENGINE_H
#define AF_ENGINE_H

#include <stdint.h>

#ifdef __cplusplus
extern "C" {
#endif

#define AF_ABI_VERSION 6

#define AF_MODE_SELFPLAY 0
#define AF_MODE_EXTERNAL 1
#define AF_MODE_VALUE_F64 0x100

#define AF_STATUS_IDLE      0
#define AF_STATUS_NEED_EVAL 1
#define AF_STATUS_MOVE_DONE 2
#define AF_STATUS_YIELD     3

#define AF_DEFAULT_TICK_BUDGET 8
#define AF_DEFAULT_TICK_BUDGET_HARD 12

#define AF_OK 0
#define AF_ERR_ARG        (-1)
#define AF_ERR_HIP        (-2)
#define AF_ERR_NODE_CAP   (-3)
#define AF_ERR_NO_ROOT    (-4)
#define AF_ERR_EP_OVERRUN (-5)
#define AF_ERR_STATE      (-6)

typedef struct {
    int32_t board_size;
    int32_t goal;
    int32_t simulation_per_step;
    int32_t upper_simulation_per_step;
    double init_temp;
    double gamma;
    double tau_decay_rate;
    double tau_decay_rate_r;
    double dirichlet_alpha;
    double c_puct;
} af_config;

typedef struct af_engine af_engine;

int af_engine_create(const af_config* cfg, int32_t num_games, int32_t device, int32_t mode, int32_t training,
                     uint64_t seed, uint32_t first_game_id, int32_t node_cap, af_engine** out);
void af_engine_destroy(af_engine* e);

int32_t af_engine_num_games(const af_engine* e);
int32_t af_engine_cells(const af_engine* e);
int32_t af_engine_key_words(const af_engine* e);
int32_t af_engine_max_plies(const af_engine* e);

int af_engine_tick(af_engine* e, void* stream, const float* policy_dev, const float* value_dev, float* planes_dev);

int af_engine_status(af_engine* e, void* stream, int32_t* status_host);

int af_engine_set_root(af_engine* e, int32_t game, const uint64_t* key, int32_t last_cell, int32_t random_a,
                       int32_t reset_tree);
int af_engine_move_result(af_engine* e, int32_t game, int32_t* action_cell, int32_t* has_policy, float* policy,
                          int32_t* visits, double* tau);
int af_engine_set_training(af_engine* e, int32_t training);
int af_engine_set_simulations(af_engine* e, int32_t simulation_per_step, int32_t upper_simulation_per_step);

int af_engine_set_roots(af_engine* e, void* stream, int32_t n, const int32_t* games, const uint64_t* keys, const int32_t* last_cells,
                        const int32_t* random_a, const int32_t* reset_tree);
int af_engine_move_results(af_engine* e, void* stream, int32_t n, const int32_t* games, int32_t* action_cells, int32_t* has_policy,
                           float* policies, int32_t* visits, double* taus);

int64_t af_engine_pack_ints(const af_engine* e, int32_t max_episodes, int32_t max_plies);
int af_engine_pack_episodes(af_engine* e, void* stream, int32_t max_episodes, int32_t max_plies, int32_t* out);

int af_engine_pop_episodes(af_engine* e, void* stream, int32_t cap, int32_t* meta, float* final_value,
                           uint64_t* keys, float* policies, int32_t* visits, int32_t* lasts, int32_t* actions);

#define AF_NUM_COUNTERS 13
int af_engine_counters(af_engine* e, void* stream, uint64_t* out);

#define AF_MEMO_STATS 6
int af_engine_memo_enable(af_engine* e, int32_t log2_buckets, int32_t max_stones);
int af_engine_memo_insert(af_engine* e, void* stream, const float* policy_dev, const float* value_dev);
int af_engine_memo_clear(af_engine* e, void* stream);
int af_engine_memo_stats(af_engine* e, void* stream, uint64_t* out);
int64_t af_engine_memo_epoch(af_engine* e);

#define AF_HIST_WORDS 97
int af_engine_tick_histogram(af_engine* e, void* stream, uint64_t* out, int32_t reset);

int af_engine_set_tick_budget(af_engine* e, int32_t selects_per_launch);

int af_engine_progress(af_engine* e, void* stream, uint64_t* out);
int af_engine_progress_async(af_engine* e, void* stream, uint64_t* out_pinned);

#define AF_STAMP_SLOTS 64
int af_engine_stamp(af_engine* e, void* stream, int32_t slot);
int af_engine_stamps_async(af_engine* e, void* stream, uint64_t* out_pinned);

#define AF_MATCH_UNFINISHED (-1)
#define AF_MATCH_WIN0 0
#define AF_MATCH_WIN1 1
#define AF_MATCH_DRAW 2
typedef struct af_match af_match;
int af_match_create(af_engine* e0, af_engine* e1, af_match** out);
void af_match_destroy(af_match* m);
int af_match_start(af_match* m, void* stream, int32_t n_games, int32_t max_plies);
int af_match_step(af_match* m, void* stream);
int af_match_progress_async(af_match* m, void* stream, uint64_t* out_pinned);
int af_match_results(af_match* m, void* stream, int32_t* result, int32_t* lengths, int32_t* moves);

int af_engine_tree_dump(af_engine* e, int32_t game, int32_t cap, uint64_t* keys, int32_t* sum_n, int32_t* n,
                        float* w, float* p, uint8_t* f32);

int af_engine_load_tree(af_engine* e, int32_t game, int32_t count, const uint64_t* keys, const int32_t* sum_n,
                        const int32_t* n, const float* w, const float* p, const uint8_t* f32);

int af_engine_tree_w64(af_engine* e, int32_t game, int32_t cap, double* w);
int af_engine_set_tree_w64(af_engine* e, int32_t game, int32_t count, const double* w);

int af_state_to_key(const char* state, int32_t board_size, uint64_t* key);
int af_key_to_state(const uint64_t* key, int32_t board_size, char* out, int32_t cap);

const char* af_strerror(int code);
int af_abi_version(void);

#ifdef __cplusplus
}
#endif
#endif
```

### include/af_net.h

```cpp
#ifndef AF_NET_H
#define AF_NET_H

#include <stdint.h>

#ifdef __cplusplus
extern "C" {
#endif

typedef struct af_net af_net;

#define AF_NET_OK 0
#define AF_NET_ERR_ARG   (-1)
#define AF_NET_ERR_HIP   (-2)
#define AF_NET_ERR_NAME  (-3)
#define AF_NET_ERR_STATE (-4)

int af_net_create(int32_t board_size, int32_t max_batch, int32_t device, af_net** out);
void af_net_destroy(af_net* n);

int af_net_set_variable(af_net* n, const char* tf_name, const float* host_data, int64_t count);
int af_net_finalize(af_net* n);

int af_net_update_device(af_net* n, void* stream, const char* const* tf_names, const float* const* dev_ptrs, const int64_t* counts,
                         int32_t nvars);

int af_net_forward(af_net* n, void* stream, const float* planes_dev, int32_t batch, float* policy_dev, float* value_dev);

int af_net_tune(int32_t key, int32_t value);

int af_net_debug_activation(af_net* n, int32_t which, int32_t batch, float* host_out);

int64_t af_net_debug_weights(af_net* n, int32_t index, void* host_out, int64_t cap_bytes);
int32_t af_net_debug_scales(af_net* n, float* host_out, int32_t cap);

int af_net_small_forward_error(af_net* n);

int64_t af_net_flops_per_position(const af_net* n);
const char* af_net_strerror(int code);

#ifdef __cplusplus
}
#endif
#endif
```

Before: 6047.

## Evaluate only live (pending) game rows in the network forward via device-side compaction

Adds a device kernel that scans the per-game pending flags and writes a compacted list of live game indices plus a count. The f16s network forward path (stem, trunk layers, value and policy FC) reads that count and row map on the device, so it skips blocks past the live count and gathers planes and scatters outputs by row index. Self-play and arena default to this path, which avoids running the network on games that have no leaf waiting in a given tick. The cost is an extra scan launch, indirect addressing, and a dependence on the paired form being selected, otherwise it falls back to the full batch.

```diff
diff --git a/alphafive_amd/arena.py b/alphafive_amd/arena.py
--- a/alphafive_amd/arena.py
+++ b/alphafive_amd/arena.py
@@ -68,7 +68,7 @@
 
 class DeviceArena:
 
-    def __init__(self, cfg, pv0, pv1, num_games, device=0, seed0=0, seed1=1, node_cap=0, weights_versions=(None, None)):
+    def __init__(self, cfg, pv0, pv1, num_games, device=0, seed0=0, seed1=1, node_cap=0, weights_versions=(None, None), live_rows=True):
         import torch
         if not torch.cuda.is_available():
             raise _eng.EngineError("DeviceArena needs a HIP device (torch.cuda.is_available() is False)")
@@ -95,6 +95,7 @@
             self._version_missing = self._version_missing or missing
             if hasattr(pv, "bind_outputs"):
                 pv.bind_outputs(self.policy[p], self.value[p])
+        self._live_rows = [bool(live_rows) and hasattr(pv, "forward_rows") and hasattr(pv, "bind_outputs") for pv in self.pvs]
         self._graph = None
         self._prog_host = torch.zeros(3, dtype=torch.int64, pin_memory=True)
         self._prog_events = [torch.cuda.Event(), torch.cuda.Event()]
@@ -108,7 +109,14 @@
         L = _eng.lib()
         for p in (0, 1):
             self.engines[p].tick(self.policy[p].data_ptr(), self.value[p].data_ptr(), self.planes[p].data_ptr(), stream)
-            pr, va = self.pvs[p](self.planes[p])
+            if self._live_rows[p]:
+                count_ptr, rows_ptr = self.engines[p].live_rows()
+                self.pvs[p].bind_outputs(self.policy[p], self.value[p])
+                pr, va = self.pvs[p].forward_rows(self.planes[p], rows_ptr, count_ptr)
+                if pr.data_ptr() != self.policy[p].data_ptr() or va.data_ptr() != self.value[p].data_ptr():
+                    raise _eng.EngineError("forward_rows did not write into the arena's policy / value tensors; use DeviceArena(..., live_rows=False)")
+            else:
+                pr, va = self.pvs[p](self.planes[p])
             if pr.data_ptr() != self.policy[p].data_ptr():
                 self.policy[p].copy_(pr.reshape(self.G, self.C))
             if va.data_ptr() != self.value[p].data_ptr():
diff --git a/alphafive_amd/csrc/af_conv_f16s.h b/alphafive_amd/csrc/af_conv_f16s.h
--- a/alphafive_amd/csrc/af_conv_f16s.h
+++ b/alphafive_amd/csrc/af_conv_f16s.h
@@ -32,8 +32,11 @@
     bool heads;
     F16sForm form;
     bool valu_stem, two_wg_per_cu, half_classes, tile_split, fused_blocks;
+    const int* rows;
+    const int* count;
 };
 F16sPlan f16s_plan(const f16s_net* n, int batch, int bits, bool heads);
+bool f16s_plan_rows(const f16s_net* n, int max_rows, int bits, bool heads, const int* rows_dev, const int* count_dev, F16sPlan* out);
 int f16s_forward(f16s_net* n, const F16sPlan& p, hipStream_t st, const float* planes_dev, float* value, float* policy);
 int f16s_trunk(f16s_net* n, const F16sPlan& p, hipStream_t st, const float* planes_dev);
 int f16s_value_branch(f16s_net* n, const F16sPlan& p, hipStream_t st, float* o3_dev, int WP, int PP, float* value);
diff --git a/alphafive_amd/csrc/af_conv_f16s.hip b/alphafive_amd/csrc/af_conv_f16s.hip
--- a/alphafive_amd/csrc/af_conv_f16s.hip
+++ b/alphafive_amd/csrc/af_conv_f16s.hip
@@ -188,6 +188,7 @@
     char* hx;
     float inv_scale_h;
     int batch, WP, PP;
+    const int* cnt;
     const uint4* w2;
     const float* bias2;
     float inv_scale2;
@@ -199,6 +200,17 @@
     int* df_err;
     int abl;
 };
+
+__device__ __forceinline__ int f16s_count(const int* cnt, int batch) {
+    if (!cnt) return batch;
+    const int c = *cnt;
+    return c < 0 ? 0 : c < batch ? c : batch;
+}
+__device__ __forceinline__ size_t f16s_row(const int* rows, int pos, int cap) {
+    if (!rows) return (size_t)pos;
+    const unsigned r = (unsigned)rows[pos];
+    return r < (unsigned)cap ? r : (unsigned)cap - 1u;
+}
 
 template <class G, int NSM, int NSP, int CT, int KS, int PS, bool OUT32, bool XACC, int PJ, int HD, int DIST, int WPE, int NTW, int HSEL, int FU = 0, int DF = 0>
 __device__ __forceinline__ void f16s_body(const F16sArgs& A, char* smem, const int bx, const int gxw, const int tb = 0,
@@ -234,7 +246,8 @@
     const int ctg = by * CT + ct, nso = gy * CT;
     const uint32_t lds = (uint32_t)(uintptr_t)smem;
 
-    const int nq = HSEL >= 0 ? A.batch : A.batch * HV;
+    const int nb = f16s_count(A.cnt, A.batch);
+    const int nq = HSEL >= 0 ? nb : nb * HV;
     int qpos = bx;
     if (AF_F16S_XCD_SWIZZLE && (gxw & (8 * (HSEL >= 0 ? 1 : HV) - 1)) == 0) qpos = (bx >> 3) + (gxw >> 3) * (bx & 7);
     if (qpos >= nq) return;
@@ -968,7 +981,8 @@
 template <class G, bool SC1 = false>
 __device__ __forceinline__ void f16s_stem_body(const float* __restrict__ planes, const uint4* __restrict__ w ,
                                                const float* __restrict__ bias, float inv_scale, char* __restrict__ out, int batch,
-                                               const int bx, const int gx, uint4* ent, _Float16* img) {
+                                               const int bx, const int gx, uint4* ent, _Float16* img,
+                                               const int* __restrict__ rows = nullptr, const int cap = 0) {
     constexpr int S = G::S, NPIX = G::NPIX, SR = S + 4, IW = S + 5;
     constexpr int NPL = 3 * NPIX, NLD = (NPL + 255) / 256;
     constexpr int NTL = (NPIX + 31) / 32, NRND = (NTL + 3) / 4;
@@ -993,7 +1007,7 @@
         const int i = (int)threadIdx.x + 256 * q;
         at[q] = img_at(i < NPL ? i : 0);
         nx[q] = 0.0f;
-        if (i < NPL && bx < batch) nx[q] = planes[(size_t)bx * NPL + i];
+        if (i < NPL && bx < batch) nx[q] = planes[f16s_row(rows, bx, cap) * NPL + i];
     }
     for (int pos = bx; pos < batch; pos += gx) {
         __syncthreads();
@@ -1001,7 +1015,7 @@
         for (int q = 0; q < NLD; ++q)
             if ((int)threadIdx.x + 256 * q < NPL) img[at[q]] = (_Float16)nx[q];
         if (pos + gx < batch) {
-            const float* pl = planes + (size_t)(pos + gx) * NPL;
+            const float* pl = planes + f16s_row(rows, pos + gx, cap) * NPL;
 #pragma unroll
             for (int q = 0; q < NLD; ++q)
                 if ((int)threadIdx.x + 256 * q < NPL) nx[q] = pl[threadIdx.x + 256 * q];
@@ -1057,17 +1071,22 @@
 
 template <class G>
 __global__ __launch_bounds__(256) void af_stem_mfma_f16s(const float* __restrict__ planes, const uint4* __restrict__ w, const float* __restrict__ bias,
-                                                         float inv_scale, char* __restrict__ out, int batch) {
+                                                         float inv_scale, char* __restrict__ out, int batch,
+                                                         const int* __restrict__ rows, const int* __restrict__ cnt) {
     __shared__ __attribute__((aligned(16))) uint4 ent[StemLds<G>::kEnt];
     __shared__ _Float16 img[StemLds<G>::kImg];
-    f16s_stem_body<G>(planes, w, bias, inv_scale, out, batch, (int)blockIdx.x, (int)gridDim.x, ent, img);
+    const int nb = f16s_count(cnt, batch);
+    if ((int)blockIdx.x >= nb) return;
+    f16s_stem_body<G>(planes, w, bias, inv_scale, out, nb, (int)blockIdx.x, (int)gridDim.x, ent, img, rows, batch);
 }
 
 template <class G>
 __device__ __forceinline__ void f16s_vfc_body(const char* __restrict__ xv, const uint4* __restrict__ a, const float* __restrict__ b1,
                                               const float* __restrict__ w2, const float* __restrict__ b2, float inv_scale,
-                                              float* __restrict__ value, int batch, const int bx) {
+                                              float* __restrict__ value, int batch, const int bx,
+                                              const int* __restrict__ rows = nullptr, const int cap = 0) {
     __shared__ float red[2][32];
+    if (bx * 32 >= batch) return;
     constexpr int NS = Hx<G>::VSTEPS;
     const bool act = threadIdx.x < 128;
     const int lane = threadIdx.x & 63, mt = (threadIdx.x >> 6) & 1, n = lane & 31, kg = lane >> 5;
@@ -1121,7 +1140,7 @@
     part += __shfl_xor(part, 32);
     if (act && kg == 0) red[mt][n] = part;
     __syncthreads();
-    if (act && mt == 0 && kg == 0 && pos < batch) value[pos] = tanhf((red[0][n] + red[1][n] + b2[0]) * 0.5f);
+    if (act && mt == 0 && kg == 0 && pos < batch) value[f16s_row(rows, pos, cap)] = tanhf((red[0][n] + red[1][n] + b2[0]) * 0.5f);
 }
 template <class G>
 __global__ __launch_bounds__(128) __attribute__((amdgpu_waves_per_eu(1, 2))) void af_value_fc_f16s(
@@ -1129,7 +1148,7 @@
     const float* __restrict__ b2, float inv_scale, float* __restrict__ value, int batch) {
     f16s_vfc_body<G>(xv, a, b1, w2, b2, inv_scale, value, batch, (int)blockIdx.x);
 }
-struct VfcArgs { const char* xv; const uint4* a; const float *b1, *w2, *b2; float inv_scale; float* value; };
+struct VfcArgs { const char* xv; const uint4* a; const float *b1, *w2, *b2; float inv_scale; float* value; const int* rows; };
 template <class G>
 __global__ __launch_bounds__(256, 1) __attribute__((amdgpu_waves_per_eu(1, 1))) void af_small_l7v_f16s(F16sArgs P, VfcArgs V) {
     extern __shared__ __attribute__((aligned(16))) char smem[];
@@ -1142,7 +1161,7 @@
     extern __shared__ __attribute__((aligned(16))) char smem[];
     const int gp = P.gx0, id = (int)blockIdx.x;
     if (id < gp) f16s_body<G, 2, 4, 2, 2, 1, false, true, 0, 0, kDist, 1, 4, -1>(P, smem, id, gp);
-    else f16s_vfc_body<G>(V.xv, V.a, V.b1, V.w2, V.b2, V.inv_scale, V.value, P.batch, id - gp);
+    else f16s_vfc_body<G>(V.xv, V.a, V.b1, V.w2, V.b2, V.inv_scale, V.value, f16s_count(P.cnt, P.batch), id - gp, V.rows, P.batch);
 }
 
 constexpr int kDfStem = 0, kDfL0 = 8, kDfL1 = 16, kDfL2 = 24, kDfL3 = 32, kDfP = 40, kDfV = 48, kDfQ = 56, kDfB5 = 64, kDfPF = 72, kDfFin = 73, kDfErr = 74, kDfWords = 75;
@@ -1328,8 +1347,11 @@
 #endif
 template <class G>
 __global__ __launch_bounds__(512, 1) void af_policy_fc_f16s(const char* __restrict__ xp, const uint4* __restrict__ a ,
-                                                            const float* __restrict__ bf, float inv_scale, float* __restrict__ policy, int batch) {
+                                                            const float* __restrict__ bf, float inv_scale, float* __restrict__ policy, const int cap,
+                                                            const int* __restrict__ rows, const int* __restrict__ cnt) {
     extern __shared__ __attribute__((aligned(16))) char psm[];
+    const int batch = f16s_count(cnt, cap);
+    if ((int)blockIdx.x * kPfPos >= batch) return;
     constexpr int NPIX = G::NPIX, HXP = Hx<G>::HXP, NLT = Hx<G>::NLT, MT = NLT / 4, RD = 16 / MT, NCH = HXP / 32, LW = 32 * NLT;
     constexpr int LWP = LW + 1;
     static_assert(NLT % 4 == 0 && LWP * 32 * 4 <= (int)kPfLds, "logit tiles");
@@ -1438,10 +1460,11 @@
 #pragma unroll
     for (int off = 8; off >= 1; off >>= 1) sum += __shfl_xor(sum, off);
     if (p < kPfPos && b0 + p < batch) {
+        const size_t prow = f16s_row(rows, b0 + p, cap);
 #pragma unroll
         for (int q = 0; q < NV; ++q) {
             const int j = sub + 16 * q;
-            if (j < NPIX) policy[(size_t)(b0 + p) * NPIX + j] = v[q] / sum;
+            if (j < NPIX) policy[prow * NPIX + j] = v[q] / sum;
         }
     }
     PF_T(4);
@@ -1870,13 +1893,20 @@
     return p;
 }
 
+bool f16s_plan_rows(const f16s_net* n, int max_rows, int bits, bool heads, const int* rows_dev, const int* count_dev, F16sPlan* out) {
+    *out = f16s_plan(n, max_rows, bits, heads);
+    if (n->S != 11 || bits != 0 || out->form != kF16sPaired || out->tile_split || !rows_dev || !count_dev) return false;
+    out->rows = rows_dev; out->count = count_dev;
+    return true;
+}
+
 static F16sArgs layer_args(const f16s_net* n, const F16sPlan& p, int li, const char* in, const char* in2, char* out) {
     F16sArgs a = {};
     a.in = in; a.in2 = in2; a.out = out;
     a.w = n->w[li]; a.bias = n->bias[li]; a.inv_scale = n->inv_scale[li];
     a.pw = n->pw[li]; a.pbuf = n->pbuf[li / 2]; a.inv_scale_p = n->inv_scale_p[li];
     a.inv_scale2 = a.inv_scale_h = 1.0f;
-    a.batch = p.batch; a.stash = n->stash;
+    a.batch = p.batch; a.cnt = p.count; a.stash = n->stash;
     a.abl = (p.bits & 0xf0ff) | (li << 8);
     static const int mask = [] { const char* e = getenv("AF_F16S_ABL_LAYERS"); return e ? (int)strtol(e, nullptr, 0) : 0x3ff; }();
     if (!((mask >> li) & 1)) a.abl &= ~kF16sProfilingBits;
@@ -1923,10 +1953,11 @@
     }
     return with_geo(n, [&](auto g) { return launch_one<decltype(g), LI>(n, p, st, a); });
 }
-static int launch_policy_fc(const f16s_net* n, hipStream_t st, int batch, float* policy) {
+static int launch_policy_fc(const f16s_net* n, hipStream_t st, const F16sPlan& p, float* policy) {
+    const int batch = p.batch;
     return with_geo(n, [&](auto g) {
         hipLaunchKernelGGL(af_policy_fc_f16s<decltype(g)>, dim3((batch + kPfPos - 1) / kPfPos), dim3(512), kPfLds, st, n->hx[1], n->hfw[1], n->hfb[1],
-                           n->hf_inv[1], policy, batch);
+                           n->hf_inv[1], policy, batch, p.rows, p.count);
         return 0;
     });
 }
@@ -1937,7 +1968,8 @@
     with_geo(n, [&](auto g) {
         using G = decltype(g);
         if (p.valu_stem) hipLaunchKernelGGL(af_stem_f16s<G>, dim3(std::min(batch, 2048)), dim3(256), 0, st, planes, n->stem_w, n->stem_b, n->f0, batch);
-        else hipLaunchKernelGGL(af_stem_mfma_f16s<G>, dim3(std::min(batch, 1024)), dim3(256), 0, st, planes, n->stem_wm, n->stem_b, n->stem_inv_scale, n->f0, batch);
+        else hipLaunchKernelGGL(af_stem_mfma_f16s<G>, dim3(std::min(batch, 1024)), dim3(256), 0, st, planes, n->stem_wm, n->stem_b, n->stem_inv_scale, n->f0, batch,
+                                p.rows, p.count);
         return 0;
     });
     int rc = launch_layer<0>(n, p, st, n->f0, nullptr, n->g[0]);
@@ -1973,7 +2005,7 @@
         if (!rc) rc = launch_layer<8>(n, p, st, n->o[3], nullptr, n->g[4]);
         if (!rc) rc = launch_layer<9>(n, p, st, n->g[4], n->o[3], nullptr, o5, WP, PP);
     }
-    if (!rc && p.heads) launch_policy_fc(n, st, p.batch, policy);
+    if (!rc && p.heads) launch_policy_fc(n, st, p, policy);
     return rc;
 }
 
@@ -1999,7 +2031,7 @@
     }
     FS_HIP_OK(hipGetLastError());
     F16sArgs Q = layer_args(n, p, 7, n->g[3], n->o[1], n->o[3]);
-    const VfcArgs F = {n->hx[0], n->hfw[0], n->hfb[0], n->v2w, n->v2b, n->hf_inv[0], value};
+    const VfcArgs F = {n->hx[0], n->hfw[0], n->hfb[0], n->v2w, n->v2b, n->hf_inv[0], value, p.rows};
     constexpr size_t lds7 = Lds<G, kDist>::kScrOff + (size_t)2 * 1 * 4 * 4096;
     if (p.tile_split) {
         if (dyn_lds<af_small_l7v_f16s<G>>(bit, (int)lds7)) return -2;
@@ -2011,7 +2043,7 @@
     }
     FS_HIP_OK(hipGetLastError());
     const int rc = launch_block<G, 8>(st, block_args<8>(n, p, n->o[3]), n->ncu);
-    if (!rc) launch_policy_fc(n, st, batch, policy);
+    if (!rc) launch_policy_fc(n, st, p, policy);
     FS_HIP_OK(hipGetLastError());
     return rc;
 }
@@ -2031,7 +2063,7 @@
     S.V = role(block_args<4>(n, p, n->o[1]), kDfL3, 4, kDfV);
     S.Q = role(layer_args(n, p, 7, n->g[3], n->o[1], n->o[3]), kDfP, 2, kDfQ);
     S.B5 = role(block_args<8>(n, p, n->o[3]), kDfQ, 2, kDfB5);
-    S.F = VfcArgs{n->hx[0], n->hfw[0], n->hfb[0], n->v2w, n->v2b, n->hf_inv[0], value};
+    S.F = VfcArgs{n->hx[0], n->hfw[0], n->hfb[0], n->v2w, n->v2b, n->hf_inv[0], value, nullptr};
     constexpr size_t ldsC = Lds<G, kDist>::kScrOff + (size_t)2 * 1 * 4 * 4096;
     constexpr size_t ldsV = Lds<G, 2>::kScrOff + (size_t)2 * 2 * 4096 * 2 + 36864;
     constexpr size_t ldsB = Lds<G, 2>::kScrOff + Lay<G>::kSlotL + 36864;
diff --git a/alphafive_amd/csrc/af_engine.hip b/alphafive_amd/csrc/af_engine.hip
--- a/alphafive_amd/csrc/af_engine.hip
+++ b/alphafive_amd/csrc/af_engine.hip
@@ -1317,6 +1317,7 @@
     std::vector<int32_t> pack_host;
     std::vector<u64> h_ct;
     unsigned long long* stamps = nullptr;
+    int32_t* live = nullptr;
     bool memo = false;
     bool memo_budget_fixed = false;
     size_t memo_entries = 0;
@@ -1361,6 +1362,28 @@
     for (int k = 0; k < KW; ++k)
         if (((key[k] | key[KW + k]) & ~P.boardmask[k]) || (key[k] & key[KW + k])) return false;
     return true;
+}
+
+__global__ __launch_bounds__(1024) void af_live_scan(const int32_t* __restrict__ pending, const int G, int32_t* __restrict__ live) {
+    __shared__ int s_w[2][16];
+    const int t = threadIdx.x, lane = t & 63, wv = t >> 6;
+    int base = 0;
+    int nxt = t < G ? pending[t] : 0;
+    for (int g0 = 0, it = 0; g0 < G; g0 += 1024, ++it) {
+        const int g = g0 + t;
+        const bool on = nxt != 0;
+        if (g + 1024 < G) nxt = pending[g + 1024];
+        const unsigned long long m = __ballot(on);
+        const int rank = __popcll(m & ((1ull << lane) - 1ull));
+        if (lane == 0) s_w[it & 1][wv] = __popcll(m);
+        __syncthreads();
+        int before = 0, total = 0;
+#pragma unroll
+        for (int w = 0; w < 16; ++w) { const int c = s_w[it & 1][w]; total += c; if (w < wv) before += c; }
+        if (on) live[1 + base + before + rank] = g;
+        base += total;
+    }
+    if (t == 0) live[0] = base;
 }
 
 #define WITH_KW(kw, ...) do { if ((kw) == 2) { constexpr int KW_ = 2; __VA_ARGS__; } else { constexpr int KW_ = 4; __VA_ARGS__; } } while (0)
@@ -1467,6 +1490,7 @@
     }
 #undef A
     if (rc == AF_OK) rc = dalloc(e, &e->stamps, (size_t)AF_STAMP_SLOTS);
+    if (rc == AF_OK) rc = dalloc(e, &e->live, 1 + G);
     if (rc != AF_OK) { af_engine_destroy(e); return rc; }
     std::vector<int32_t> ph(G, mode == AF_MODE_SELFPLAY ? PH_MOVE_START : PH_IDLE), rl(G, -1);
     std::vector<double> tau(G, cfg->init_temp);
@@ -1496,7 +1520,15 @@
     hipStream_t st = (hipStream_t)stream;
     WITH_FLAG(e->memo, MEMO_, WITH_KW(e->KW, WITH_FLAG(e->P.w64, W64_,
         hipLaunchKernelGGL((af_tick_kernel<KW_, W64_, MEMO_>), dim3(e->P.G), dim3(64), 0, st, e->P, policy_dev, value_dev, planes_dev))));
+    hipLaunchKernelGGL(af_live_scan, dim3(1), dim3(1024), 0, st, e->P.pending, e->P.G, e->live);
     HIP_OK(hipGetLastError());
+    return AF_OK;
+}
+
+int af_engine_live_rows(af_engine* e, const int32_t** count_dev, const int32_t** rows_dev) {
+    if (!e || !count_dev || !rows_dev) return AF_ERR_ARG;
+    *count_dev = e->live;
+    *rows_dev = e->live + 1;
     return AF_OK;
 }
 
diff --git a/alphafive_amd/csrc/af_net.hip b/alphafive_amd/csrc/af_net.hip
--- a/alphafive_amd/csrc/af_net.hip
+++ b/alphafive_amd/csrc/af_net.hip
@@ -880,6 +880,16 @@
     return forward_range(n, (hipStream_t)stream, planes, 0, batch, policy, value);
 }
 
+int af_net_forward_rows(af_net* n, void* stream, const float* planes, const int32_t* rows, const int32_t* count, int32_t max_rows,
+                        float* policy, float* value) {
+    if (!n || !planes || !rows || !count || !policy || !value || max_rows < 1 || max_rows > n->max_batch) return AF_NET_ERR_ARG;
+    if (!n->ready) return AF_NET_ERR_STATE;
+    F16sPlan plan;
+    if (g_wino == 5 && n->f16s && g_fhead && f16s_plan_rows(n->f16s, max_rows, g_f16s_abl, true, rows, count, &plan))
+        return f16s_forward(n->f16s, plan, (hipStream_t)stream, planes, value, policy) ? AF_NET_ERR_HIP : AF_NET_OK;
+    return forward_range(n, (hipStream_t)stream, planes, 0, max_rows, policy, value);
+}
+
 int af_net_tune(int32_t key, int32_t value) {
     if (key == 0) { if (value != 1 && value != 5) return AF_NET_ERR_ARG; g_wino = value; return AF_NET_OK; }
     if (key == 5) { g_phead = value; return AF_NET_OK; }
diff --git a/alphafive_amd/engine.py b/alphafive_amd/engine.py
--- a/alphafive_amd/engine.py
+++ b/alphafive_amd/engine.py
@@ -89,6 +89,8 @@
         L.af_match_step.argtypes = [vp, vp]
         L.af_match_progress_async.argtypes = [vp, vp, vp]
         L.af_match_results.argtypes = [vp, vp, i32p, i32p, i32p]
+        if hasattr(L, "af_engine_live_rows"):
+            L.af_engine_live_rows.argtypes = [vp, C.POINTER(vp), C.POINTER(vp)]
         L.af_engine_tree_dump.argtypes = [vp, C.c_int32, C.c_int32, u64p, i32p, i32p, f32p, f32p, u8p]
         L.af_engine_load_tree.argtypes = [vp, C.c_int32, C.c_int32, u64p, i32p, i32p, f32p, f32p, u8p]
         L.af_state_to_key.argtypes = [C.c_char_p, C.c_int32, u64p]
@@ -158,6 +160,15 @@
 
     def tick(self, policy_ptr, value_ptr, planes_ptr, stream=None):
         _check(lib().af_engine_tick(self._h, stream, policy_ptr, value_ptr, planes_ptr), "af_engine_tick")
+
+    def live_rows(self):
+        if getattr(self, "_live", None) is None:
+            if not hasattr(lib(), "af_engine_live_rows"):
+                raise EngineError("libaf_hip.so has no af_engine_live_rows (rebuild: python -m alphafive_amd.build)")
+            cnt, rows = C.c_void_p(), C.c_void_p()
+            _check(lib().af_engine_live_rows(self._h, C.byref(cnt), C.byref(rows)), "af_engine_live_rows")
+            self._live = (cnt.value, rows.value)
+        return self._live
 
     def status(self, stream=None):
         rc = lib().af_engine_status(self._h, stream, _p(self._status, C.c_int32))
@@ -354,7 +365,7 @@
 class SelfPlayEngine:
 
     def __init__(self, cfg, num_games, pv_device, device=0, seed=0, first_game_id=0, training=True, node_cap=0,
-                 value_f64=False, weights_version=None, eval_memo=None):
+                 value_f64=False, weights_version=None, eval_memo=None, live_rows=True):
         import torch
         if not torch.cuda.is_available():
             raise EngineError("SelfPlayEngine needs a HIP device (torch.cuda.is_available() is False)")
@@ -373,6 +384,7 @@
         self._weights_version = self._resolve_weights_version(weights_version)
         if hasattr(pv_device, "bind_outputs"):
             pv_device.bind_outputs(self.policy, self.value)
+        self.live_rows = bool(live_rows) and hasattr(pv_device, "forward_rows") and hasattr(pv_device, "bind_outputs")
         self._memo_version = None
         if eval_memo:
             if self._weights_version is None:
@@ -401,7 +413,15 @@
         self.engine.tick(self.policy.data_ptr(), self.value.data_ptr(), self.planes.data_ptr(), stream)
         if stamp_base is not None:
             self.engine.stamp(stamp_base + 1, stream)
-        p, v = self.pv_device(self.planes)
+        if self.live_rows:
+            count_ptr, rows_ptr = self.engine.live_rows()
+            self.pv_device.bind_outputs(self.policy, self.value)
+            p, v = self.pv_device.forward_rows(self.planes, rows_ptr, count_ptr)
+            if p.data_ptr() != self.policy.data_ptr() or v.data_ptr() != self.value.data_ptr():
+                raise EngineError("forward_rows did not write into the engine's policy / value tensors (its handle is sized for "
+                                  "a larger batch than this engine's); use SelfPlayEngine(..., live_rows=False)")
+        else:
+            p, v = self.pv_device(self.planes)
         if p.data_ptr() != self.policy.data_ptr():
             self.policy.copy_(p.reshape(self.G, self.C))
         if v.data_ptr() != self.value.data_ptr():
diff --git a/alphafive_amd/net_hip.py b/alphafive_amd/net_hip.py
--- a/alphafive_amd/net_hip.py
+++ b/alphafive_amd/net_hip.py
@@ -27,6 +27,7 @@
         L.af_net_set_variable.argtypes = [vp, C.c_char_p, C.POINTER(C.c_float), C.c_int64]
         L.af_net_finalize.argtypes = [vp]
         L.af_net_forward.argtypes = [vp, vp, vp, C.c_int32, vp, vp]
+        L.af_net_forward_rows.argtypes = [vp, vp, vp, vp, vp, C.c_int32, vp, vp]
         L.af_net_update_device.argtypes = [vp, vp, C.POINTER(C.c_char_p), C.POINTER(vp), C.POINTER(C.c_int64), C.c_int32]
         L.af_net_debug_weights.argtypes = [vp, C.c_int32, vp, C.c_int64]
         L.af_net_debug_weights.restype = C.c_int64
@@ -116,6 +117,14 @@
                "af_net_forward")
         return self.policy[:B], self.value[:B]
 
+    def forward_rows(self, planes, rows_ptr, count_ptr):
+        B = planes.shape[0]
+        assert B <= self.max_batch and planes.is_contiguous() and planes.dtype == torch.float32
+        stream = torch.cuda.current_stream(self.device).cuda_stream
+        _check(lib().af_net_forward_rows(self._h, stream, planes.data_ptr(), rows_ptr, count_ptr, B, self.policy.data_ptr(),
+                                         self.value.data_ptr()), "af_net_forward_rows")
+        return self.policy[:B], self.value[:B]
+
     def small_forward_error(self):
         return int(lib().af_net_small_forward_error(self._h))
 
@@ -136,8 +145,7 @@
     lib()
     state = {"net": None, "out": None, "version": None}
 
-    def pv(planes):
-        B = planes.shape[0]
+    def net_for(B):
         if state["net"] is None or state["net"].max_batch < B:
             if state["net"] is not None:
                 state["net"].close()
@@ -158,7 +166,13 @@
             else:
                 state["net"].load(resnet.variables)
             state["version"] = version
-        return state["net"](planes)
+        return state["net"]
+
+    def pv(planes):
+        return net_for(planes.shape[0])(planes)
+
+    def forward_rows(planes, rows_ptr, count_ptr):
+        return net_for(planes.shape[0]).forward_rows(planes, rows_ptr, count_ptr)
 
     def bind_outputs(policy, value):
         state["out"] = (policy, value)
@@ -171,6 +185,7 @@
             state["net"] = None
 
     pv.bind_outputs = bind_outputs
+    pv.forward_rows = forward_rows
     pv.close = close
     pv.weights_version = lambda: getattr(resnet, "version", None)
     return pv
diff --git a/include/af_engine.h b/include/af_engine.h
--- a/include/af_engine.h
+++ b/include/af_engine.h
@@ -109,6 +109,8 @@
 int af_match_progress_async(af_match* m, void* stream, uint64_t* out_pinned);
 int af_match_results(af_match* m, void* stream, int32_t* result, int32_t* lengths, int32_t* moves);
 
+int af_engine_live_rows(af_engine* e, const int32_t** count_dev, const int32_t** rows_dev);
+
 int af_engine_tree_dump(af_engine* e, int32_t game, int32_t cap, uint64_t* keys, int32_t* sum_n, int32_t* n,
                         float* w, float* p, uint8_t* f32);
 
diff --git a/include/af_net.h b/include/af_net.h
--- a/include/af_net.h
+++ b/include/af_net.h
@@ -26,6 +26,9 @@
 
 int af_net_forward(af_net* n, void* stream, const float* planes_dev, int32_t batch, float* policy_dev, float* value_dev);
 
+int af_net_forward_rows(af_net* n, void* stream, const float* planes_dev, const int32_t* rows_dev, const int32_t* count_dev,
+                        int32_t max_rows, float* policy_dev, float* value_dev);
+
 int af_net_tune(int32_t key, int32_t value);
 
 int af_net_debug_activation(af_net* n, int32_t which, int32_t batch, float* host_out);
```

Result: no change. 6061 (median of 3 runs) (+0.2%).
